# w111liang222/lidar-slam-detection

Hardware: AMD Instinct MI355X
Metric: registered points/sec (120k-pt scan vs 1e7-pt map, full iterate-to-converge) (higher is better)
Workload: dtype f32 per-point geometry / f64 transforms and reductions

## Files before the change

include/lio_hip.h:

```cpp
#ifndef LIO_HIP_H_
#define LIO_HIP_H_

#include <stdint.h>

#ifdef __cplusplus
extern "C" {
#endif

#define LIO_OK 0
#define LIO_E_INVALID (-1)
#define LIO_E_CAPACITY (-2)
#define LIO_E_DEVICE (-3)
#define LIO_E_STATE (-4)

typedef struct lio_map lio_map;
typedef struct lio_scan lio_scan;
typedef struct lio_engine lio_engine;

const char* lio_last_error(void);
const char* lio_last_warning(void);
int lio_device_count(void);
#define LIO_ABI_VERSION 24
int lio_abi_version(void);
void* lio_pinned_alloc(uint64_t bytes);
void lio_pinned_free(void* p);
uint64_t lio_map_bytes(const lio_map*);

lio_map* lio_map_create(int device, float resolution, uint64_t max_points, uint64_t max_voxels, int stencil);
void lio_map_destroy(lio_map*);
int lio_map_set_stencil(lio_map*, int stencil);
int lio_map_insert(lio_map*, const float* world_xyzi, uint64_t n, double travel);
int lio_map_insert_device(lio_map*, const void* d_world_xyzi, uint64_t n, double travel);
int lio_map_clear(lio_map*);
int lio_map_set_lru(lio_map*, uint64_t capacity_voxels, double max_distance);
int lio_map_lru_stats(lio_map*, uint64_t* n_evicted, uint64_t* n_interleaved);
int lio_map_lru_exact_stats(lio_map*, uint64_t* n_recreated, uint64_t* n_batches_not_followed);
int lio_map_set_tie_mode(lio_map*, int mode);
int lio_map_tie_stats(lio_map*, uint64_t* n_boundary_ties, uint64_t* n_unresolved);
int lio_map_pool_stats(lio_map*, uint64_t* pool_top, uint64_t* pool_cap);
int lio_map_stats(lio_map*, uint64_t* n_points, uint64_t* n_voxels);
uint64_t lio_map_knn_candidates(lio_map*);
uint64_t lio_map_knn_touched(lio_map*);
uint64_t lio_map_knn_unique(lio_map*);
int64_t lio_map_dump(lio_map*, float* out_xyzi, uint64_t cap_points);
int lio_map_knn(lio_map*, const float* world_xyzi, uint32_t n, float* out_pts, int32_t* out_cnt);

lio_scan* lio_scan_create(int device, uint32_t max_raw, uint32_t max_ds);
void lio_scan_destroy(lio_scan*);
int lio_scan_reset(lio_scan*);
int lio_scan_upload(lio_scan*, const float* body_xyzi, uint32_t n_raw);
int lio_scan_set_device(lio_scan*, const void* d_body_xyzi, uint32_t n_raw);
int lio_scan_undistort_delta(lio_scan*, const uint32_t* stamp_us, int stamps_on_device, const float delta_pose[16], double scan_period);
int lio_scan_download_raw(lio_scan*, float* out_xyzi, uint32_t cap);
int lio_scan_undistort_poses(lio_scan*, const uint32_t* stamp_us, int stamps_on_device, uint64_t header_stamp_us, const uint64_t* pose_stamp_us,
                             const double* pose_T, uint32_t n_poses);
int lio_scan_undistort_imu(lio_scan*, const uint32_t* stamp_us, int stamps_on_device, const double* poses, uint32_t n_poses, const double* end_pos3,
                           const double* end_rot_xyzw, const double* ril_xyzw, const double* til3, double blind, int filter_num, int undistort);
int lio_scan_voxel_downsample(lio_scan*, float leaf, int sync, uint32_t* n_ds);
int lio_scan_voxel_downsample_batch(lio_scan** scans, int n, float leaf, uint32_t* n_ds);
int lio_scan_set_ds(lio_scan*, const float* ds_body_xyzi, uint32_t n_ds);
int lio_scan_num_ds(lio_scan*);
int lio_scan_download_ds(lio_scan*, float* out_xyzi, uint32_t cap);
int lio_scan_download_world(lio_scan*, float* out_xyzi, uint32_t cap);
const void* lio_scan_ds_device(lio_scan*, uint32_t* n);
int lio_scan_download_match(lio_scan*, uint8_t* selected, float* normvec, int32_t* nn_cnt, float* nn_pts);

typedef struct lio_kernel_times {
    double knn_us, linearize_us, finalize_us;
    uint32_t knn_launches, linearize_launches, finalize_launches;
    uint32_t pad;
} lio_kernel_times;
int lio_scan_enable_kernel_timing(lio_scan*, int on);
int lio_scan_kernel_times(lio_scan*, lio_kernel_times* out, int reset);

typedef struct lio_normal_eq {
    double JtJ[36];
    double Jtr[6];
    double nnT[9];
    double eigvec[9];
    double eigval[3];
    double contri[3];
    double strong[3];
    double sum_abs_res;
    uint32_t n_eff;
    uint32_t n_ds;
    uint32_t n_knn_candidates_lo, n_knn_candidates_hi;
    uint32_t n_tie;
    uint32_t seq;
} lio_normal_eq;

int lio_p2plane_linearize(lio_map*, lio_scan*, const double pose_wi[7], const double ext_il[7], int redo_knn,
                          lio_normal_eq* out);
int lio_scan_set_degeneracy_mode(lio_scan*, int mode);
int lio_p2plane_degeneracy(lio_scan*, const double V[9], double contri[3], double strong[3]);
int lio_p2plane_rows(lio_scan*, const double pose_wi[7], const double ext_il[7], double* h_x6, double* h, uint32_t cap_rows);
int lio_map_incremental(lio_map*, lio_scan*, const double pose_wi[7], const double ext_il[7], float map_leaf,
                        int ekf_inited, double travel);
int lio_map_seed(lio_map*, lio_scan*, const double pose_wi[7], const double ext_il[7], double travel);

lio_engine* lio_engine_create(int device, float resolution, int stencil, uint64_t max_points, uint64_t max_voxels,
                              uint32_t max_raw, uint32_t max_ds);
lio_engine* lio_engine_create_shared(lio_map* shared_map, uint32_t max_raw, uint32_t max_ds);
void lio_engine_destroy(lio_engine*);
lio_map* lio_engine_map(lio_engine*);
lio_scan* lio_engine_scan(lio_engine*);
// ... 40 lines not shown
int lio_engine_set_device_loop(lio_engine*, int on);

int lio_fastlio_ins_enqueue(lio_engine*, double stamp, const double vel_imu[3]);
int lio_fastlio_set_wheelspeed(lio_engine*, int enable);
int lio_fastlio_pcl_enqueue(lio_engine*, const float* xyzi, const uint32_t* stamp_us, uint32_t n, double header_stamp);
int lio_fastlio_pcl_stage(lio_engine*, uint32_t n, float** xyzi, uint32_t** stamp_us);
int lio_fastlio_pcl_commit(lio_engine*, uint32_t n, double header_stamp);
int lio_fastlio_pcl_enqueue_device(lio_engine*, const void* d_xyzi, const void* d_stamp_us, uint32_t n, double header_stamp);
int lio_fastlio_main(lio_engine*);
int lio_fastlio_odometry(lio_engine*, double odom_s[16], double odom_e[16]);
int lio_fastlio_state(lio_engine*, double out[20]);
int lio_fastlio_start_state(lio_engine*, double s26[26]);
int lio_fastlio_download_undistorted(lio_engine*, float* out_xyzi, uint32_t cap, uint32_t* n);
typedef int (*lio_meas_fn)(void* ctx, const double* s26, int converge, int* n, double* rows6, double* h, int cap);
int lio_eskf_update_cb(const double s26[26], const double P[529], double R, int max_iter, lio_meas_fn fn, void* ctx, int cap, double s26_out[26],
                       double P_out[529]);
int lio_eskf_update_ws_cb(const double s26[26], const double P[529], double R, int max_iter, lio_meas_fn fn, void* ctx, int cap, const double* ins_vel,
                          int degenerate, double s26_out[26], double P_out[529]);
int lio_state_predict(const double s26[26], const double P[529], double dt, const double Q[12], const double acc[3], const double gyro[3],
                      double s26_out[26], double P_out[529]);
typedef int (*lio_sums_fn)(void* ctx, const double* s26, int converge, double* acc29);
typedef void (*lio_degeneracy_fn)(void* ctx, const double* V9, double* cs6);
int lio_eskf_update_sums_cb(const double s26[26], const double P[529], double R, int max_iter, int degenerate_detect_en, lio_sums_fn fn,
                            lio_degeneracy_fn dfn, void* ctx, double s26_out[26], double P_out[529], lio_pass_log* logs, int cap_logs, int* status);

typedef void (*lio_reduce_fn)(void* ctx, double* buf, int n);
int lio_engine_set_reduce_hook(lio_engine*, lio_reduce_fn fn, void* ctx);
typedef struct lio_comm lio_comm;
int lio_comm_unique_id(uint8_t id[128]);
lio_comm* lio_comm_init(int device, int rank, int world, const uint8_t id[128]);
void lio_comm_destroy(lio_comm*);
int lio_comm_rank(const lio_comm*);
int lio_comm_world(const lio_comm*);
int lio_allgather_normal_eq(lio_comm*, const double* d_local32, double* d_gathered, double* d_sum32, void* stream);
int lio_allgather_records(lio_comm*, const double* d_local, double* d_gathered, uint32_t n_records, void* stream);
int lio_comm_stats(lio_comm*, uint64_t* n_collectives, double* total_us);
int lio_engine_set_joint(lio_engine* e, lio_engine** others, int n_others, lio_comm* comm);
int lio_engine_joint_register(lio_engine* e, const float* raw_body_xyzi, uint32_t n_raw, double lidar_beg_time, double state26[26], double cov[529]);
int lio_engine_joint_register_device(lio_engine* e, const void* d_raw_body_xyzi, uint32_t n_raw, double lidar_beg_time, double state26[26], double cov[529]);
#define LIO_JOB_KEEP_CACHE 1u
#define LIO_JOB_IDLE 2u
#define LIO_JOB_HOST_RAW 4u
#define LIO_JOB_FLAGS_KNOWN 7u
typedef struct lio_scan_job {
    const void* d_raw;
    uint32_t n_raw;
    uint32_t flags;
    double lidar_beg_time;
    const double* state_in;
    const double* cov_in;
    double* state_out;
    int32_t rc;
    int32_t n_ds, n_pass, n_knn_pass;
} lio_scan_job;
int lio_engines_process_batch(lio_engine** engines, int n_engines, lio_scan_job* jobs, int n_jobs);
typedef struct lio_batch lio_batch;
typedef struct lio_batch_result {
    double state[26];
    int32_t status;
    int32_t n_pass, n_knn_pass, n_ds, n_eff, degenerate, radix_passes, err;
    int32_t loop_i, loop_t, loop_converge, pad;
    uint32_t seq, pad2;
} lio_batch_result;
lio_batch* lio_batch_create(lio_map* shared_map, int n_slots, int n_groups, uint32_t max_raw, uint32_t max_ds);
lio_batch* lio_batch_create_joint(lio_map** sub_maps, int n_sub_maps, lio_comm* comm, int n_slots, int n_groups, uint32_t max_raw, uint32_t max_ds);
typedef int (*lio_gather_fn)(void* ctx, const double* d_local, double* d_gathered, uint32_t n_records, void* stream);
int lio_batch_set_gather_hook(lio_batch*, lio_gather_fn fn, void* ctx, int rank, int world);
int lio_batch_exchange_stats(lio_batch*, uint32_t* chunk_points, uint64_t* jobs_rerun, uint64_t* bytes_per_rank_and_round);
lio_batch* lio_batch_create_sequences(int device, float resolution, int stencil, uint64_t max_points, uint64_t max_voxels, int n_slots, int n_groups,
                                      uint32_t max_raw, uint32_t max_ds);
int lio_batch_sequences_step(lio_batch*, lio_scan_job* jobs, int n_jobs, double* cov_out);
int lio_batch_fastlio_main(lio_batch*, int* rc_out);
void lio_batch_destroy(lio_batch*);
int lio_batch_process(lio_batch*, lio_scan_job* jobs, int n_jobs);
typedef struct lio_batch_times {
    double downsample_us, knn_us, linearize_us, step_us;
    uint32_t downsample_launches, knn_launches, linearize_launches, step_launches;
    double insert_us;
    uint32_t insert_launches, pad;
} lio_batch_times;
int lio_batch_enable_kernel_timing(lio_batch*, int on);
int lio_batch_kernel_times(lio_batch*, lio_batch_times* out, int reset);
lio_engine* lio_batch_engine(lio_batch*, int group, int slot);
int lio_engine_set_static_map(lio_engine*, int on);

typedef struct lio_ndt lio_ndt;
lio_ndt* lio_ndt_create(int device, float resolution, int search_method, uint64_t max_points, uint64_t max_voxels, uint32_t max_source_points);
void lio_ndt_destroy(lio_ndt*);
int lio_ndt_set_target(lio_ndt*, const float* xyzi, uint64_t n);
int lio_ndt_set_target_device(lio_ndt*, const void* d_xyzi, uint64_t n);
int lio_ndt_num_voxels(lio_ndt*);
int lio_ndt_voxel_at(lio_ndt*, const float p[3], float mean[3], float cinv[9]);
int lio_ndt_linearize(lio_ndt*, lio_scan* source, const double T[16], int update_corr, int with_derivatives, double H[36], double b[6],
                      double* err, uint32_t* n_corr);
int lio_ndt_fitness_score(lio_ndt*, lio_scan* source, const double T[16], double max_range, double* score, uint32_t* n_inliers);
int lio_ndt_overlap_score(lio_ndt*, lio_scan* source, const double relpose[16], double max_range, double xy_range, double min_z, double* score,
                          double* inlier_ratio);
typedef struct lio_ndt_times {
    double cost_us;
    uint64_t launches, update_launches, pairs, source_points;
} lio_ndt_times;
int lio_ndt_enable_kernel_timing(lio_ndt*, int on);
int lio_ndt_kernel_times(lio_ndt*, lio_ndt_times* out, int reset);
typedef struct lio_ndt_params {
    int32_t max_iterations;
    int32_t lm_max_iterations;
    double rotation_epsilon_deg;
    double transformation_epsilon;
    double lm_init_lambda_factor;
    double max_process_time_ms;
} lio_ndt_params;
void lio_ndt_default_params(lio_ndt_params*);
int lio_ndt_align(lio_ndt*, lio_scan* source, const double guess[16], const lio_ndt_params* params, double out[16], int* iterations,
                  int* converged);

typedef struct lio_align_job {
    lio_ndt* target;
    lio_scan* source;
    const double* guess;
    double out[16];
    int32_t iterations, converged, evaluations, rc;
} lio_align_job;
int lio_ndt_align_batch(lio_ndt*, lio_align_job* jobs, int n_jobs, const lio_ndt_params* params);

typedef struct lio_gicp lio_gicp;
lio_gicp* lio_gicp_create(int device, float grid_resolution, uint32_t max_points, int k_correspondences);
void lio_gicp_destroy(lio_gicp*);
int lio_gicp_set_target(lio_gicp*, const float* xyzi, uint32_t n);
int lio_gicp_set_source(lio_gicp*, const float* xyzi, uint32_t n);
int lio_gicp_set_target_device(lio_gicp*, const void* d_xyzi, uint32_t n);
int lio_gicp_set_source_device(lio_gicp*, const void* d_xyzi, uint32_t n);
int lio_gicp_set_voxel_mode(lio_gicp*, double voxel_resolution, int search_method);
int lio_gicp_voxel_at(lio_gicp*, const float p[3], double mean[3], double cov6[6]);
int lio_gicp_download(lio_gicp*, int which, float* xyzi, double* cov6, uint32_t cap);
int lio_gicp_correspondences(lio_gicp*, int32_t* corr, uint32_t cap);
int lio_gicp_neighbours(lio_gicp*, int which, int32_t* idx, uint32_t cap_points);
int lio_gicp_mahalanobis(lio_gicp*, double* maha6, uint32_t cap);
int lio_gicp_linearize(lio_gicp*, const double T[16], double max_corr_dist, int update_corr, int with_derivatives, double H[36], double b[6], double* err,
                       uint32_t* n_corr);
int lio_gicp_align(lio_gicp*, const double guess[16], const lio_ndt_params* params, double max_corr_dist, double out[16], int* iterations, int* converged);
int lio_gicp_fitness_score(lio_gicp*, const double T[16], double max_range, double* score, uint32_t* nr);

typedef struct lio_pose_estimator lio_pose_estimator;
typedef struct lio_gps_observation {
    double T[16];
    double precision;
    int32_t dimension;
} lio_gps_observation;
lio_pose_estimator* lio_pose_estimator_create(const float imu_ext[16], uint64_t stamp_us, const float pos[3], const float quat_wxyz[4],
                                              double cool_time_duration);
void lio_pose_estimator_destroy(lio_pose_estimator*);
int lio_pose_estimator_predict(lio_pose_estimator*, uint64_t stamp_us, const float acc[3], const float gyro[3]);
int lio_pose_estimator_match(lio_pose_estimator*, lio_ndt* target, lio_scan* source, const lio_ndt_params* params, float observation[7],
                             int* iterations);
int lio_pose_estimator_match_gps(lio_pose_estimator*, lio_ndt* target, lio_scan* source, const lio_ndt_params* params, const lio_gps_observation* gps,
                                 float observation[7], float observation_cov[49], int* iterations);
int lio_pose_estimator_guess(lio_pose_estimator*, const lio_gps_observation* gps, float init_guess[16]);
int lio_pose_estimator_observe(lio_pose_estimator*, const float init_guess[16], const float aligned[16], int converged, const lio_gps_observation* gps,
                               float observation[7], float observation_cov[49]);
int lio_pose_estimator_match_gps_only(lio_pose_estimator*, const lio_gps_observation* gps, float observation[7], float observation_cov[49]);
int lio_pose_estimator_get_timed_pose(lio_pose_estimator*, uint64_t stamp_us, const double acc_g[3], const double gyro_dps[3], double pose[16]);
int lio_pose_estimator_predict_nostate(lio_pose_estimator*, uint64_t stamp_us, double pose[16]);
int lio_pose_estimator_correct(lio_pose_estimator*, uint64_t stamp_us, const float observation[7]);
uint64_t lio_pose_estimator_get_dt(lio_pose_estimator*);
int lio_pose_estimator_get(lio_pose_estimator*, float mean23[23], float cov529[529]);
int lio_pose_estimator_set(lio_pose_estimator*, const float mean23[23], const float cov529[529]);
// ... 532 lines not shown
```

lidar-slam-detection_amd/csrc/batch.hip:

```cpp
#include <sched.h>
#include <stdlib.h>

#include <chrono>
#include <deque>
#include <vector>

#include "eskf.h"
#include "lio_common.h"

using namespace lio;

int engine_resume_update(lio_engine* e, const double* x_now26, const double* x_prop26, const double* P_prop, int i, int converge, int t);
void engine_count_passes(lio_engine* e, int* n_pass, int* n_knn);
int engine_joint_register_device(lio_engine* e, const void* d_raw, uint32_t n_raw, double lidar_beg_time, double state26[26], double cov[529]);
struct lio_comm;
extern "C" int lio_comm_world(const lio_comm*);
extern "C" {
int engine_seq_prepare(lio_engine* e, uint32_t n_raw, double lidar_beg_time, int* ekf_inited);
void engine_seq_params(lio_engine* e, double* laser_cov, int* maximum_iter, int* degenerate_detect_en, float* leaf_surf, float* leaf_map, int* static_map,
                       double* travel, double last_pos_lid[3]);
int engine_seq_finish(lio_engine* e, const double x26[26], const double P529[529], int n_ds, int n_pass, int n_knn, int n_eff, int degenerate, int inserted,
                      uint32_t n_add, uint32_t map_err, uint32_t bound);
int engine_seq_resume(lio_engine* e, const double* x_now26, const double* x_prop26, const double* P_prop, int i, int converge, int t);
int engine_seq_has_lru(lio_engine* e);
int engine_fastlio_front(lio_engine* e, const void** d_raw, uint32_t* n_raw, double* beg, double state26[26], double cov529[529]);
void engine_fastlio_back(lio_engine* e);
}

namespace {

struct Group {
    hipStream_t stream = nullptr;
    std::vector<lio_engine*> eng;
    std::vector<lio_engine*> sub_eng;
    double* d_local32 = nullptr;
    double* d_gathered = nullptr;
    char* d_ds_send = nullptr;
    char* d_ds_all = nullptr;
    int ds_world = 0;
    MapRef* d_rowmaps = nullptr;
    std::vector<MapRef> rowmap_rows;
    char* d_block = nullptr;
    char* h_block = nullptr;
    size_t block_bytes = 0;
    SlotDesc* d_desc = nullptr;
    SlotDesc* h_desc = nullptr;
    EskfDev* d_ctrl = nullptr;
    EskfDev* h_ctrl = nullptr;
    hipGraphExec_t exec[5] = {nullptr, nullptr, nullptr, nullptr, nullptr};
    const void* graph_table = nullptr;
    int graph_stencil = 0;
    lio_batch_result* h_res = nullptr;
    lio_batch_result* h_res_dev = nullptr;
    std::vector<int> job_of_slot;
    float4* d_rawbuf = nullptr;
    MapRef* d_maps = nullptr;
    MapRef* h_maps = nullptr;
    SeqDev* d_seq = nullptr;
    SeqDev* h_seq = nullptr;
    std::vector<int> seq_path;
    int any_lru = 0;
    int n_active = 0;
    int launched_passes = 4;
    uint32_t seq = 0;
    uint32_t max_n_raw = 0;
    BatchTimer* bt = nullptr;
};

}

struct lio_batch {
    lio_map* map = nullptr;
    int device = 0;
    int n_slots = 0;
    uint32_t max_raw = 0, max_ds = 0;
    int pred_passes = 4;
    bool broken = false;
    int use_graph = 1;
    int count_touched = 0;
    std::vector<lio_map*> maps;
    lio_comm* comm = nullptr;
    int world = 1;
    int rank = 0;
    int split_ds = 1;
    uint32_t ds_cap = 0;
    uint32_t ds_seen_max = 0;
    bool ds_cap_full = false;
    uint64_t n_ds_cut = 0;
    int (*gather_hook)(void*, const double*, double*, uint32_t, void*) = nullptr;
    void* gather_ctx = nullptr;
    bool joint = false;
    bool sequences = false;
    std::vector<lio_scan_job> fl_jobs;
    std::vector<double> fl_state, fl_cov;
    std::vector<Group> groups;
    double t_submit = 0, t_wait = 0, t_collect = 0;
    uint64_t n_rounds = 0;
};

static void fill_mapref(MapRef& r, const lio_map* m);

namespace {

const MapRef* joint_rowmaps(lio_batch* b, Group& g) {
    const int M = (int)b->maps.size(), B = b->n_slots;
    if (M < 2) return nullptr;
    for (int m = 1; m < M; m++)
        if (b->maps[m]->stencil_id != b->maps[0]->stencil_id || b->maps[m]->stencil.n != b->maps[0]->stencil.n) return nullptr;
    std::vector<MapRef> now((size_t)M);
    for (int m = 0; m < M; m++) {
        memset(&now[m], 0, sizeof(MapRef));
        fill_mapref(now[m], b->maps[m]);
    }
    bool fresh = g.d_rowmaps != nullptr && (int)g.rowmap_rows.size() == M;
    for (int m = 0; m < M && fresh; m++) fresh = memcmp(&g.rowmap_rows[m], &now[m], sizeof(MapRef)) == 0;
    if (fresh) return g.d_rowmaps;
    std::vector<MapRef> rows((size_t)M * B);
    for (int m = 0; m < M; m++)
        for (int s = 0; s < B; s++) rows[(size_t)m * B + s] = now[m];
    if (!g.d_rowmaps && hipMalloc(reinterpret_cast<void**>(&g.d_rowmaps), sizeof(MapRef) * rows.size()) != hipSuccess) { g.d_rowmaps = nullptr; return nullptr; }
    if (hipMemcpyAsync(g.d_rowmaps, rows.data(), sizeof(MapRef) * rows.size(), hipMemcpyHostToDevice, g.stream) != hipSuccess) return nullptr;
    if (hipStreamSynchronize(g.stream) != hipSuccess) return nullptr;
    g.rowmap_rows = now;
    return g.d_rowmaps;
}

void fill_desc(SlotDesc& d, lio_scan* sc, EskfDev* d_ctrl, lio_batch_result* d_res) {
    d.max_ds = sc->max_ds;
    d.partial_blocks = sc->partial_blocks;
    d.sd = sc->dev;
    d.keys_a = sc->keys_a; d.keys_b = sc->keys_b; d.vals_a = sc->vals_a; d.vals_b = sc->vals_b;
// ... 60 lines not shown
    return dst;
}

int submit(lio_batch* b, Group& g, lio_scan_job* jobs, int first, int n, int passes) {
    const int B = b->n_slots;
    g.seq++;
    g.n_active = 0;
    g.max_n_raw = 0;
    g.launched_passes = passes;
    for (int s = 0; s < B; s++) {
        SlotDesc& d = g.h_desc[s];
        d.active = 0;
        g.job_of_slot[s] = -1;
        if (s >= n) continue;
        lio_scan_job& job = jobs[first + s];
        g.job_of_slot[s] = first + s;
        job.rc = LIO_E_INVALID;
        job.n_ds = job.n_pass = job.n_knn_pass = 0;
        if (job.flags & ~LIO_JOB_FLAGS_KNOWN) { set_error("lio_scan_job.flags = 0x%x: unknown bits (a job array that was not zero-initialised?)", job.flags); continue; }
        if (job.flags & LIO_JOB_IDLE) { job.rc = 0; g.job_of_slot[s] = -1; continue; }
        if (!job.state_in || !job.cov_in || (!job.d_raw && job.n_raw)) continue;
        if (job.n_raw > b->max_raw) { set_error("scan of %u points exceeds max_raw %u", job.n_raw, b->max_raw); job.rc = LIO_E_CAPACITY; continue; }
        if (job.n_raw == 0) { job.rc = 2; continue; }
        d.raw = static_cast<const float4*>(job.d_raw);
        if (job.flags & LIO_JOB_HOST_RAW) {
            int src = LIO_OK;
            d.raw = stage_host_raw(b, g, s, job, &src);
            if (src != LIO_OK) { job.rc = src; continue; }
        }
        d.n_raw = job.n_raw;
        d.nblocks = (job.n_raw + 2047u) / 2048u;
        d.active = 1;
        d.seq = g.seq;
        d.min_ds = 5;
        d.reset_cache = (job.flags & LIO_JOB_KEEP_CACHE) ? 0u : 1u;
        fill_ctrl(g.h_ctrl[s], job.state_in, job.cov_in, 0.001 , 4, 1, b->joint ? 1 : 0);
        g.h_res[s].seq = g.seq - 1;
        g.n_active++;
        if (job.n_raw > g.max_n_raw) g.max_n_raw = job.n_raw;
    }
    const int M = (int)b->maps.size();
    for (int m = 1; m < M; m++)
        for (int s = 0; s < B; s++) {
            SlotDesc& d = g.h_desc[(size_t)m * B + s];
            const SlotDesc& p = g.h_desc[s];
            d.raw = p.raw; d.n_raw = p.n_raw; d.nblocks = p.nblocks; d.active = p.active; d.seq = p.seq; d.min_ds = p.min_ds; d.reset_cache = p.reset_cache;
        }
    if (g.n_active == 0) return LIO_OK;
    const bool timed = g.bt && g.bt->on;
    const MapRef* rowmaps = b->joint ? joint_rowmaps(b, g) : nullptr;
    auto enqueue = [&](BatchTimer* bt) -> int {
        LIO_HIP_TRY(hipMemcpyAsync(g.d_block, g.h_block, g.block_bytes, hipMemcpyHostToDevice, g.stream));
        const uint32_t ds_bound = b->max_raw < b->max_ds ? b->max_raw : b->max_ds;
        int rc = LIO_OK;
        if (b->joint && b->world > 1 && b->split_ds) {
            const int per = (B + b->world - 1) / b->world;
            const int s0 = std::min(B, b->rank * per), s1 = std::min(B, s0 + per);
            if (g.ds_world != b->world) {
                if (g.d_ds_send) hipFree(g.d_ds_send);
                if (g.d_ds_all) hipFree(g.d_ds_all);
                g.d_ds_send = g.d_ds_all = nullptr;
                g.ds_world = 0;
                const size_t chunk = (size_t)per * ds_exchange_slot_bytes(ds_bound);
                LIO_HIP_TRY(hipMalloc(reinterpret_cast<void**>(&g.d_ds_send), chunk));
                LIO_HIP_TRY(hipMalloc(reinterpret_cast<void**>(&g.d_ds_all), chunk * (size_t)b->world));
                g.ds_world = b->world;
            }
            if (bt) bt->begin(0);
            if (s1 > s0) rc = vg_downsample_batch(g.stream, g.d_desc + s0, s1 - s0, b->max_raw, b->max_ds, 0.5f, passes);
            if (bt) bt->end(0);
            if (rc != LIO_OK) return rc;
            if (b->ds_cap == 0) {
                const char* k = getenv("LIO_JOINT_DS_CAP");
                const uint32_t want = k ? (uint32_t)strtoul(k, nullptr, 10) : ((ds_bound / 4u + 1023u) & ~1023u);
                b->ds_cap = std::min(ds_bound, std::max(k ? 1u : 4096u, want));
            }
            const uint32_t cap = b->ds_cap_full ? ds_bound : b->ds_cap;
            rc = p2plane_batch_exchange_ds(b->comm, b->world, b->gather_hook, b->gather_ctx, g.stream, g.d_desc, B, per, s0, s1, cap, g.d_ds_send, g.d_ds_all);
            if (rc == LIO_OK && s0 > 0) rc = scan_begin_rows(g.stream, g.d_desc, s0);
            if (rc == LIO_OK && s1 < B) rc = scan_begin_rows(g.stream, g.d_desc + s1, B - s1);
            if (rc != LIO_OK) return rc;
        } else {
            if (bt) bt->begin(0);
            rc = vg_downsample_batch(g.stream, g.d_desc, B, b->max_raw, b->max_ds, 0.5f, passes);
            if (bt) bt->end(0);
            if (rc != LIO_OK) return rc;
        }
        if (b->joint) {
            rc = p2plane_batch_share(g.stream, g.d_desc, B, M, ds_bound);
            if (rc == LIO_OK) rc = scan_begin_rows(g.stream, g.d_desc + B, B * (M - 1));
            if (rc != LIO_OK) return rc;
            return p2plane_batch_update_joint(b->maps.data(), M, b->comm, b->world, b->gather_hook, b->gather_ctx, g.stream, g.d_desc, B, ds_bound, 5, g.d_local32, g.d_gathered, bt,
                                              rowmaps);
        }
        return p2plane_batch_update(b->map, g.stream, g.d_desc, B, ds_bound, 5, bt, bt ? b->count_touched : 0);
    };
    if (!b->use_graph || timed || b->joint) return enqueue(timed ? g.bt : nullptr);
    if (g.graph_table != b->map->table || g.graph_stencil != b->map->stencil.n) {
        for (int k = 0; k < 5; k++)
            if (g.exec[k]) { hipGraphExecDestroy(g.exec[k]); g.exec[k] = nullptr; }
        g.graph_table = b->map->table;
        g.graph_stencil = b->map->stencil.n;
    }
    if (!g.exec[passes]) {
        hipGraph_t graph = nullptr;
        LIO_HIP_TRY(hipStreamBeginCapture(g.stream, hipStreamCaptureModeThreadLocal));
        const int rc = enqueue(nullptr);
        const hipError_t e2 = hipStreamEndCapture(g.stream, &graph);
        if (rc != LIO_OK) { if (graph) hipGraphDestroy(graph); return rc; }
        LIO_HIP_TRY(e2);
        LIO_HIP_TRY(hipGraphInstantiate(&g.exec[passes], graph, nullptr, nullptr, 0));
        hipGraphDestroy(graph);
    }
    LIO_HIP_TRY(hipGraphLaunch(g.exec[passes], g.stream));
    return LIO_OK;
}

int wait_group(Group& g, int B) {
    for (int s = 0; s < B; s++) {
        if (!g.h_desc[s].active) continue;
        volatile uint32_t* seq = &g.h_res[s].seq;
        for (uint64_t spin = 0; *seq != g.seq; spin++) {
            __builtin_ia32_pause();
            if (spin > 2000 && (spin & 31) == 0) sched_yield();
            if (spin > 40000000ull) {
                LIO_HIP_TRY(hipStreamSynchronize(g.stream));
                if (*seq != g.seq) { set_error("batch slot %d did not report (seq %u, expected %u)", s, *seq, g.seq); return LIO_E_DEVICE; }
                break;
            }
        }
    }
    __atomic_thread_fence(__ATOMIC_ACQUIRE);
    return LIO_OK;
}

}


extern "C" {

static lio_batch* batch_create_impl(lio_map** maps, int n_maps, lio_comm* comm, int n_slots, int n_groups, uint32_t max_raw, uint32_t max_ds) {
    lio_map* map = n_maps > 0 && maps ? maps[0] : nullptr;
    if (!map || n_maps > 64 || n_slots < 1 || n_slots > 256 || n_groups < 1 || n_groups > 8 || max_raw == 0 || max_ds == 0) { set_error("lio_batch_create: bad argument"); return nullptr; }
    for (int m = 1; m < n_maps; m++)
        if (!maps[m] || maps[m]->device != map->device) { set_error("lio_batch_create_joint: the sub-maps of a batch live on one device"); return nullptr; }
    if (hipSetDevice(map->device) != hipSuccess) { set_error("lio_batch_create: no HIP device %d", map->device); return nullptr; }
    lio_batch* b = new lio_batch();
    b->map = map;
    b->device = map->device;
    b->n_slots = n_slots;
    b->max_raw = max_raw;
    b->max_ds = max_ds;
    b->maps.assign(maps, maps + n_maps);
    b->comm = comm;
    b->world = comm ? lio_comm_world(comm) : 1;
    b->rank = comm ? lio_comm_rank(comm) : 0;
    { const char* k = getenv("LIO_JOINT_SPLIT_DS"); b->split_ds = (k && k[0] == '0') ? 0 : 1; }
    b->joint = n_maps > 1 || comm != nullptr;
    b->groups.resize(n_groups);
    { const char* k = getenv("LIO_BATCH_GRAPH"); b->use_graph = (k && k[0] == '0') ? 0 : 1; }
    bool ok = true;
    const int M = n_maps;
    for (Group& g : b->groups) ok = ok && hipStreamCreateWithFlags(&g.stream, hipStreamNonBlocking) == hipSuccess;
    for (Group& g : b->groups) {
        g.job_of_slot.assign(n_slots, -1);
        const size_t desc_bytes = sizeof(SlotDesc) * (size_t)n_slots * (size_t)M;
        g.block_bytes = desc_bytes + sizeof(EskfDev) * (size_t)n_slots;
        ok = ok && hipMalloc(reinterpret_cast<void**>(&g.d_block), g.block_bytes) == hipSuccess;
        ok = ok && hipHostMalloc(reinterpret_cast<void**>(&g.h_block), g.block_bytes, hipHostMallocDefault) == hipSuccess;
        if (ok) {
            g.d_desc = reinterpret_cast<SlotDesc*>(g.d_block);
            g.h_desc = reinterpret_cast<SlotDesc*>(g.h_block);
            g.d_ctrl = reinterpret_cast<EskfDev*>(g.d_block + desc_bytes);
            g.h_ctrl = reinterpret_cast<EskfDev*>(g.h_block + desc_bytes);
        }
        ok = ok && hipHostMalloc(reinterpret_cast<void**>(&g.h_res), sizeof(lio_batch_result) * n_slots, hipHostMallocMapped) == hipSuccess;
        ok = ok && hipHostGetDevicePointer(reinterpret_cast<void**>(&g.h_res_dev), g.h_res, 0) == hipSuccess;
        if (b->joint) {
            ok = ok && hipMalloc(reinterpret_cast<void**>(&g.d_local32), sizeof(double) * 32 * n_slots) == hipSuccess;
            ok = ok && hipMalloc(reinterpret_cast<void**>(&g.d_gathered), sizeof(double) * 32 * n_slots * (size_t)b->world) == hipSuccess;
        }
        if (!ok) break;
        memset(g.h_block, 0, g.block_bytes);
        memset(g.h_res, 0, sizeof(lio_batch_result) * n_slots);
        ok = hipMemset(g.d_block, 0, g.block_bytes) == hipSuccess;
        for (int s = 0; s < n_slots && ok; s++) {
            lio_engine* e = lio_engine_create_shared(map, max_raw, max_ds);
            if (!e) { ok = false; break; }
            lio_engine_set_flags(e, 1, 0, 0.0, -10.0);
            g.eng.push_back(e);
            fill_desc(g.h_desc[s], lio_engine_scan(e), &g.d_ctrl[s], &g.h_res_dev[s]);
        }
        for (int m = 1; m < M && ok; m++)
            for (int s = 0; s < n_slots && ok; s++) {
                lio_engine* e = lio_engine_create_shared(maps[m], max_raw, max_ds);
                if (!e) { ok = false; break; }
                lio_engine_set_flags(e, 1, 0, 0.0, -10.0);
                g.sub_eng.push_back(e);
                fill_desc(g.h_desc[(size_t)m * n_slots + s], lio_engine_scan(e), &g.d_ctrl[s], nullptr);
            }
        for (int s = 0; s < n_slots && ok && b->joint; s++) {
            std::vector<lio_engine*> others;
            for (int m = 1; m < M; m++) others.push_back(g.sub_eng[(size_t)(m - 1) * n_slots + s]);
            ok = lio_engine_set_joint(g.eng[s], others.empty() ? nullptr : others.data(), (int)others.size(), comm) == LIO_OK;
        }
    }
    if (!ok) {
        set_error("lio_batch_create: device setup failed: %s", hipGetErrorString(hipGetLastError()));
        lio_batch_destroy(b);
        return nullptr;
    }
    {
        const char* q = getenv("GPU_MAX_HW_QUEUES");
        if (n_groups > 1 && (!q || atoi(q) < 8))
            set_warning("lio_batch_create: GPU_MAX_HW_QUEUES=%s -- with fewer than 8 hardware queues the %d rounds in flight mostly serialise (~20 %% slower); "
                        "export GPU_MAX_HW_QUEUES=8 before the process's first HIP call", q ? q : "(unset: 4)", n_groups);
    }
    return b;
}

lio_batch* lio_batch_create(lio_map* map, int n_slots, int n_groups, uint32_t max_raw, uint32_t max_ds) {
    return batch_create_impl(&map, map ? 1 : 0, nullptr, n_slots, n_groups, max_raw, max_ds);
}

lio_batch* lio_batch_create_joint(lio_map** sub_maps, int n_sub_maps, lio_comm* comm, int n_slots, int n_groups, uint32_t max_raw, uint32_t max_ds) {
    return batch_create_impl(sub_maps, n_sub_maps, comm, n_slots, n_groups, max_raw, max_ds);
}

int lio_batch_set_gather_hook(lio_batch* b, lio_gather_fn fn, void* ctx, int rank, int world) {
    if (!b || !fn || world < 1 || rank < 0 || rank >= world) return LIO_E_INVALID;
    if (!b->joint || b->comm) { set_error("lio_batch_set_gather_hook: for a batch made by lio_batch_create_joint without a communicator"); return LIO_E_STATE; }
    hipSetDevice(b->map->device);
    for (auto& g : b->groups) {
        LIO_HIP_TRY(hipStreamSynchronize(g.stream));
        if (g.d_gathered) hipFree(g.d_gathered);
        g.d_gathered = nullptr;
        LIO_HIP_TRY(hipMalloc(reinterpret_cast<void**>(&g.d_gathered), sizeof(double) * 32 * b->n_slots * (size_t)world));
    }
    b->gather_hook = fn;
    b->gather_ctx = ctx;
    b->world = world;
    b->rank = rank;
    return LIO_OK;
}

int lio_batch_exchange_stats(lio_batch* b, uint32_t* chunk_points, uint64_t* jobs_rerun, uint64_t* bytes_per_rank_and_round) {
    if (!b) return LIO_E_INVALID;
    const bool on = b->joint && b->world > 1 && b->split_ds;
    if (chunk_points) *chunk_points = on ? b->ds_cap : 0u;
    if (jobs_rerun) *jobs_rerun = b->n_ds_cut;
    if (bytes_per_rank_and_round) {
        const int per = (b->n_slots + b->world - 1) / b->world;
        *bytes_per_rank_and_round = on && b->ds_cap ? (uint64_t)per * ds_exchange_slot_bytes(b->ds_cap) : 0u;
    }
    return LIO_OK;
}

void lio_batch_destroy(lio_batch* b) {
    if (!b) return;
    hipSetDevice(b->device);
    if (getenv("LIO_BATCH_PROFILE") && b->n_rounds)
        fprintf(stderr, "lio_batch: %llu rounds of %d slots; host per round: submit %.1f us, wait %.1f us, collect %.1f us\n", (unsigned long long)b->n_rounds,
                b->n_slots, 1e6 * b->t_submit / b->n_rounds, 1e6 * b->t_wait / b->n_rounds, 1e6 * b->t_collect / b->n_rounds);
    for (Group& g : b->groups) {
        if (g.stream) hipStreamSynchronize(g.stream);
        group_free(g);
    }
    delete b;
}

int lio_batch_enable_kernel_timing(lio_batch* b, int on) {
    if (!b) return LIO_E_INVALID;
    hipSetDevice(b->device);
    for (Group& g : b->groups) {
        if (!g.bt) { g.bt = new BatchTimer(); g.bt->stream = g.stream; }
        if (on && !g.bt->created) {
            for (int c = 0; c < BatchTimer::kClasses; c++)
                for (int i = 0; i < BatchTimer::kPool; i++) {
                    LIO_HIP_TRY(hipEventCreate(&g.bt->ev[c][i][0]));
                    LIO_HIP_TRY(hipEventCreate(&g.bt->ev[c][i][1]));
                }
            g.bt->created = true;
        }
        g.bt->on = on != 0;
    }
    b->count_touched = (on & 2) ? 1 : 0;
    if (b->count_touched && b->map) { const int rc = map_enable_touch_bits(b->map); if (rc != LIO_OK) return rc; }
    return LIO_OK;
}

int lio_batch_kernel_times(lio_batch* b, lio_batch_times* out, int reset) {
    if (!b || !out) return LIO_E_INVALID;
    memset(out, 0, sizeof(*out));
    for (Group& g : b->groups) {
        if (!g.bt) continue;
        out->downsample_us += g.bt->us[0]; out->knn_us += g.bt->us[1]; out->linearize_us += g.bt->us[2]; out->step_us += g.bt->us[3];
        out->downsample_launches += g.bt->launches[0]; out->knn_launches += g.bt->launches[1]; out->linearize_launches += g.bt->launches[2];
        out->step_launches += g.bt->launches[3];
        out->insert_us += g.bt->us[4];
        out->insert_launches += g.bt->launches[4];
        if (reset)
            for (int c = 0; c < BatchTimer::kClasses; c++) { g.bt->us[c] = 0; g.bt->launches[c] = 0; }
    }
    return LIO_OK;
}

lio_engine* lio_batch_engine(lio_batch* b, int group, int slot) {
    if (!b || group < 0 || group >= (int)b->groups.size() || slot < 0 || slot >= b->n_slots) return nullptr;
    return b->groups[group].eng[slot];
}

int lio_batch_process(lio_batch* b, lio_scan_job* jobs, int n_jobs) {
    if (!b || (!jobs && n_jobs) || n_jobs < 0) return LIO_E_INVALID;
    if (b->sequences) { set_error("lio_batch_process: a sequence batch is driven by lio_batch_sequences_step"); return LIO_E_STATE; }
    hipSetDevice(b->device);
    const int B = b->n_slots;
    int next = 0, first_err = 0;
    std::deque<int> inflight;
    std::vector<int> retry;
    auto note = [&](int rc) { if (rc < 0 && !first_err) first_err = rc; };
    auto collect = [&](Group& g) {
        int need_max = 1;
        for (int s = 0; s < B; s++) {
            const int j = g.job_of_slot[s];
            if (j < 0) continue;
            if (!g.h_desc[s].active) { note(jobs[j].rc); continue; }
            lio_scan_job& job = jobs[j];
            const lio_batch_result& r = g.h_res[s];
            if (r.radix_passes > need_max) need_max = r.radix_passes;
            if (r.radix_passes > g.launched_passes) { retry.push_back(j); continue; }
            lio_engine* e = g.eng[s];
            lio_scan* sc = lio_engine_scan(e);
            sc->have_ds = r.n_ds;
            sc->n_raw = g.h_desc[s].n_raw;
            job.n_ds = r.n_ds;
            job.n_pass = r.n_pass;
            job.n_knn_pass = r.n_knn_pass;
            if (r.err & 4) {
                hipMemsetAsync(&sc->dev->err, 0, 4, g.stream);
                b->n_ds_cut++;
                retry.push_back(j);
                continue;
            }
            if (r.err & 1) {
                set_error("downsampled scan exceeds max_ds %u", b->max_ds);
                hipMemsetAsync(&sc->dev->err, 0, 4, g.stream);
                job.rc = LIO_E_CAPACITY;
                note(job.rc);
                continue;
            }
            if ((uint32_t)r.n_ds > b->ds_seen_max) b->ds_seen_max = (uint32_t)r.n_ds;
            if (r.status == EK_SKIPPED) { job.rc = 2; continue; }
            if (r.status == EK_NEEDS_HOST && b->joint && b->gather_hook) {
                set_error("lio_batch (gather hook mode): a scan needs the host-driven joint path, which only exists over a lio_comm");
                job.rc = LIO_E_STATE;
                note(job.rc);
                continue;
            }
            if (r.status == EK_NEEDS_HOST && b->joint) {
                if (!(job.flags & LIO_JOB_KEEP_CACHE)) {
                    scan_forget_cache(sc);
                    for (int m = 1; m < (int)b->maps.size(); m++) scan_forget_cache(lio_engine_scan(g.sub_eng[(size_t)(m - 1) * B + s]));
                }
                double st26[26], cov[529];
                memcpy(st26, job.state_in, sizeof(st26));
                memcpy(cov, job.cov_in, sizeof(cov));
                const void* d_cloud = (job.flags & LIO_JOB_HOST_RAW) ? static_cast<const void*>(g.d_rawbuf + (size_t)s * b->max_raw) : job.d_raw;
                const int rc = engine_joint_register_device(e, d_cloud, job.n_raw, job.lidar_beg_time, st26, cov);
                if (rc < 0) { job.rc = rc; note(rc); continue; }
                engine_count_passes(e, &job.n_pass, &job.n_knn_pass);
                if (job.state_out) memcpy(job.state_out, st26, sizeof(st26));
                job.rc = rc;
                continue;
            }
            if (r.status == EK_NEEDS_HOST) {
                const int rc = engine_resume_update(e, r.state, job.state_in, job.cov_in, r.loop_i, r.loop_converge, r.loop_t);
                if (rc != LIO_OK) { job.rc = rc; note(rc); continue; }
                int np = 0, nk = 0;
                engine_count_passes(e, &np, &nk);
                job.n_pass += np;
                job.n_knn_pass += nk;
                if (job.state_out) lio_engine_get_state(e, job.state_out);
                job.rc = 3;
                continue;
            }
// ... 497 lines not shown
```

lidar-slam-detection_amd/csrc/knn.hip:

```cpp
#include "hashgrid.h"
#include "knn_dev.h"
#include "lio_common.h"
#include "refsel.h"

namespace lio {

#ifndef LIO_KNN_G
#define LIO_KNN_G 16
#endif
#ifndef LIO_KNN_U
#define LIO_KNN_U 4
#endif
#ifndef LIO_KNN_WAVES
#define LIO_KNN_WAVES 6
#endif
#ifndef LIO_KNN_PRUNE
#define LIO_KNN_PRUNE 1
#endif
#ifndef LIO_KNN_STAT
#define LIO_KNN_STAT 1
#endif
#ifndef LIO_KNN_WAVES_BATCH
#define LIO_KNN_WAVES_BATCH 7
#endif
#ifdef LIO_KNN_MAXWAVES
#define LIO_KNN_OCC __attribute__((amdgpu_waves_per_eu(LIO_KNN_MAXWAVES, LIO_KNN_MAXWAVES)))
#else
#define LIO_KNN_OCC
#endif
constexpr int kG = LIO_KNN_G;
constexpr int kU = LIO_KNN_U;
constexpr int kGPB = 256 / kG;

template <int CTRL>
__device__ inline uint32_t dpp_row(uint32_t v) {
    return (uint32_t)__builtin_amdgcn_update_dpp(0, (int)v, CTRL, 0xF, 0xF, true);
}
__device__ inline uint32_t group_min32(uint32_t v) {
    if constexpr (kG == 8) {
        v = min(v, dpp_row<0xB1>(v));
        v = min(v, dpp_row<0x4E>(v));
        v = min(v, dpp_row<0x141>(v));
    } else if constexpr (kG == 16) {
        v = min(v, dpp_row<0x128>(v));
        v = min(v, dpp_row<0x124>(v));
        v = min(v, dpp_row<0x122>(v));
        v = min(v, dpp_row<0x121>(v));
    } else {
#pragma unroll
        for (int off = kG / 2; off > 0; off >>= 1) v = min(v, __shfl_xor(v, off, kG));
    }
    return v;
}
__device__ inline uint32_t group_ballot(bool p, int lane) {
    const unsigned long long b = __ballot(p);
    if constexpr (kG == 16 || kG == 8) {
        const uint32_t half = (lane & 32) ? (uint32_t)(b >> 32) : (uint32_t)b;
        return (half >> (lane & (32 - kG) & 31)) & ((1u << kG) - 1u);
    } else {
        return (uint32_t)((b >> (lane & ~(kG - 1))) & ((1ull << kG) - 1ull));
    }
}
__device__ inline uint32_t group_max32(uint32_t v) {
    if constexpr (kG == 8) {
        v = max(v, dpp_row<0xB1>(v));
        v = max(v, dpp_row<0x4E>(v));
        v = max(v, dpp_row<0x141>(v));
    } else if constexpr (kG == 16) {
        v = max(v, dpp_row<0x128>(v));
        v = max(v, dpp_row<0x124>(v));
        v = max(v, dpp_row<0x122>(v));
        v = max(v, dpp_row<0x121>(v));
    } else {
#pragma unroll
        for (int off = kG / 2; off > 0; off >>= 1) v = max(v, __shfl_xor(v, off, kG));
    }
    return v;
}
__device__ inline uint32_t group_sum32(uint32_t v) {
    if constexpr (kG == 8) {
        v += dpp_row<0xB1>(v);
        v += dpp_row<0x4E>(v);
        v += dpp_row<0x141>(v);
    } else if constexpr (kG == 16) {
// ... 132 lines not shown
    for (int k = 0; k < KM; k++) {
        uint32_t ptr = 0, cnt = 0;
        if (want[k] != kEmptyKey) {
            uint4 r = raw[k];
            for (uint32_t probe = 0; probe <= (mask >> 6); probe++) {
                const unsigned long long kk = ((unsigned long long)r.y << 32) | r.x;
                if (kk == want[k]) { ptr = r.z; cnt = r.w; break; }
                if (kk == kEmptyKey) break;
                brick_next(bp[k]);
                r = *reinterpret_cast<const uint4*>(&table[brick_slot(bp[k], mask)]);
            }
        }
        const bool hit = cnt > 0;
        const uint32_t m = group_ballot(hit, lane);
        if (hit) {
            const uint32_t at = nhit + __popc(m & below);
            g.v_ptr[at] = ptr;
            g.v_cnt[at] = cnt;
        }
        nhit += __popc(m);
        total += cnt;
    }
    if (gl < kU) { g.v_ptr[nhit + gl] = 0; g.v_cnt[nhit + gl] = 0; }
    nhit_out = nhit;
    return total;
}

__device__ inline void group_lds_sync() {
    __builtin_amdgcn_fence(__ATOMIC_RELEASE, "wavefront");
    __builtin_amdgcn_wave_barrier();
    __builtin_amdgcn_fence(__ATOMIC_ACQUIRE, "wavefront");
}

__device__ inline uint32_t med3_u32(uint32_t a, uint32_t b, uint32_t c) {
    uint32_t r;
    asm("v_med3_u32 %0, %1, %2, %3" : "=v"(r) : "v"(a), "v"(b), "v"(c));
    return r;
}
#ifndef LIO_KNN_BOUND
#define LIO_KNN_BOUND 5
#endif
__device__ inline uint32_t fifth_bound(uint32_t d0, uint32_t d2, uint32_t d4) {
    uint32_t t = group_min32(d4);
#if LIO_KNN_BOUND == 2
    (void)d0;
    const uint32_t m1 = group_min32(d2);
    return min(t, group_min32(d2 == m1 ? 0xFFFFFFFFu : d2));
#endif
    (void)d2;
    uint32_t v = d0, m = 0xFFFFFFFFu;
#pragma unroll
    for (int r = 0; r < 5; r++) {
        m = group_min32(v);
        if (v == m) v = 0xFFFFFFFFu;
    }
    return min(t, m);
}

struct Cand {
    float d2;
    uint32_t id;
};

__device__ __noinline__ bool cand_tie_less(const Cand& a, const Cand& b, const float4* __restrict__ pool) {
    if (a.id == b.id) return false;
    if (a.id == kNoIdx || b.id == kNoIdx) return a.id < b.id;
    const float4 pa = pool[a.id], pb = pool[b.id];
    if (pa.x != pb.x) return pa.x < pb.x;
    if (pa.y != pb.y) return pa.y < pb.y;
    if (pa.z != pb.z) return pa.z < pb.z;
    return a.id < b.id;
}
__device__ inline bool cand_less(const Cand& a, const Cand& b, const float4* __restrict__ pool) {
    if (a.d2 != b.d2) return a.d2 < b.d2;
    return cand_tie_less(a, b, pool);
}


template <int KM, int MODE, bool COUNT = false, class PoseFill>
__device__ __forceinline__ void knn_body(const Slot* __restrict__ table, uint32_t mask, const float4* __restrict__ pool,
                                         float inv_res, const StencilArgs& st, PoseFill fill, const float4* __restrict__ queries,
                                         uint32_t n_host, const ScanDev* __restrict__ sd, float4* __restrict__ world_out,
                                         float4* __restrict__ nn_pts, uint32_t nn_stride, int32_t* __restrict__ nn_cnt,
                                         MapDev* md, uint32_t* __restrict__ n_tie, uint32_t* __restrict__ tie_list) {
    __shared__ GroupLds lds[kGPB];
    const int tid = threadIdx.x;
    const int grp = tid / kG, gl = tid % kG;
    const int lane = tid & 63;
    GroupLds& g = lds[grp];
    const uint32_t n = sd ? sd->n_ds : n_host;
    const unsigned long long gmask = ((1ull << kG) - 1ull) << (lane - gl);
    __shared__ uint32_t stat_s[256 / 64];
    if (tid < 256 / 64) stat_s[tid] = 0;
    uint32_t touched = 0;
    uint32_t fresh = 0;
    uint32_t* const bits = COUNT ? md->touch_bits : nullptr;
    const float res = 1.0f / inv_res;
    const uint32_t b1_bits = __float_as_uint(0.0625f * res * res), b2_bits = __float_as_uint(0.25f * res * res);
    (void)b1_bits; (void)b2_bits;

    const uint32_t nblk = (n + kGPB - 1) / kGPB;
    const uint32_t per_xcd = (nblk + 7u) >> 3;
    const uint32_t wg_per_xcd = gridDim.x >> 3;
    constexpr uint32_t kAhead = 64 / kGPB;
    __shared__ float4 pw_s[64];
    __shared__ PoseArgs pose_s;
    if constexpr (MODE == 0) fill(pose_s);
    uint32_t ahead = kAhead;
    for (uint32_t j = blockIdx.x >> 3; j < per_xcd; j += wg_per_xcd) {
        const uint32_t q0 = ((blockIdx.x & 7u) * per_xcd + j) * kGPB;
        const uint32_t q = q0 + grp;
        const bool active = q < n;
        float4 pw = make_float4(0.f, 0.f, 0.f, 0.f);
        if constexpr (MODE == 0) {
            if (ahead == kAhead) {
                __syncthreads();
                if (tid < 64) {
                    const uint32_t j2 = j + (uint32_t)(tid / kGPB) * wg_per_xcd;
                    const uint32_t q2 = ((blockIdx.x & 7u) * per_xcd + j2) * kGPB + (uint32_t)(tid % kGPB);
                    if (j2 < per_xcd && q2 < n) {
                        float4 w2;
                        body_to_world(pose_s, queries[q2], w2);
                        world_out[q2] = w2;
                        uint32_t t2 = (uint32_t)tid;
                        asm volatile("" : "+v"(t2));
                        pw_s[t2] = w2;
                    }
                }
                __syncthreads();
                ahead = 0;
            }
            if (active) pw = pw_s[ahead * kGPB + grp];
            ahead++;
        } else {
            if (active) pw = queries[q];
        }
        int kx = 0, ky = 0, kz = 0;
        pos2grid(pw.x, pw.y, pw.z, inv_res, kx, ky, kz);
        uint32_t nhit = 0;
        constexpr bool kPrune = LIO_KNN_PRUNE && KM * kG <= 32;
        uint32_t n0 = 0, n01 = 0, total;
        const uint32_t limit = 0xFFFFFFFFu;
        if constexpr (kPrune) total = probe_stencil_bucketed<KM>(table, mask, st, active, pw, res, kx, ky, kz, gl, lane, gmask, g, nhit, n0, n01, limit);
        else total = probe_stencil<KM>(table, mask, st, active, kx, ky, kz, gl, lane, gmask, g, nhit);
        if constexpr (LIO_KNN_STAT || COUNT) {
            const uint32_t gs = group_sum32(total);
            const uint32_t ws = (uint32_t)__builtin_amdgcn_readlane((int)gs, 0) + (uint32_t)__builtin_amdgcn_readlane((int)gs, 16) +
                                (uint32_t)__builtin_amdgcn_readlane((int)gs, 32) + (uint32_t)__builtin_amdgcn_readlane((int)gs, 48);
            if (lane == 0) stat_s[tid >> 6] += ws;
        }
        group_lds_sync();
        uint32_t d0 = 0xFFFFFFFFu, d1 = 0xFFFFFFFFu, dd2 = 0xFFFFFFFFu, d3 = 0xFFFFFFFFu, d4 = 0xFFFFFFFFu;
        uint32_t i0d = 0xFFFFFFFFu, i1d = 0xFFFFFFFFu, i2d = 0xFFFFFFFFu, i3d = 0xFFFFFFFFu, i4d = 0xFFFFFFFFu;
        uint32_t inrange = 0;
        bool drop_tie = false;
        uint32_t bound5 = 0xFFFFFFFFu;
        const uint32_t ptr_first = g.v_ptr[0];
        bool need_bound = true;
#ifndef LIO_KNN_HOME_FIRST
#define LIO_KNN_HOME_FIRST 0
#endif
        int phase = (kPrune && LIO_KNN_HOME_FIRST) ? 0 : 2;
        for (uint32_t s0 = 0; s0 < nhit; s0 += (phase >= 1 ? kU : 0u), phase = (phase < 2 ? phase + 1 : 2)) {
            uint32_t ptr4[kU], cnt4[kU];
            uint32_t cmax = 0;
            bool ins = false;
            if constexpr (kPrune) {
                if (s0 > 0 || phase == 1) {
                    if (need_bound) bound5 = fifth_bound(d0, dd2, d4);
                    const uint32_t floor_bits = s0 < n0 ? 0u : (s0 < n01 ? b1_bits : b2_bits);
                    if (bound5 < floor_bits) break;
                    const uint32_t r0 = s0 + gl, r1 = r0 + kG, r2 = r1 + kG, r3 = r2 + kG;
                    const bool mine = (r0 < nhit && g.v_dmin[r0] <= bound5) || (r1 < nhit && g.v_dmin[r1] <= bound5) ||
                                      (kG < 16 && ((r2 < nhit && g.v_dmin[r2] <= bound5) || (r3 < nhit && g.v_dmin[r3] <= bound5)));
                    if (!group_ballot(mine, lane)) break;
                }
            }
#pragma unroll
            for (int u = 0; u < kU; u += 4) {
                const uint4 vp = *reinterpret_cast<const uint4*>(&g.v_ptr[s0 + u]);
                uint4 vc = *reinterpret_cast<const uint4*>(&g.v_cnt[s0 + u]);
                if constexpr (kPrune) {
                    const uint4 vd = *reinterpret_cast<const uint4*>(&g.v_dmin[s0 + u]);
                    if (vd.x > bound5) vc.x = 0;
                    if (vd.y > bound5) vc.y = 0;
                    if (vd.z > bound5) vc.z = 0;
                    if (vd.w > bound5) vc.w = 0;
                    if (LIO_KNN_HOME_FIRST && u == 0) {
                        if (phase == 0) { vc.y = 0; vc.z = 0; vc.w = 0; }
                        else if (phase == 1) vc.x = 0;
                    }
                }
                ptr4[u] = vp.x; ptr4[u + 1] = vp.y; ptr4[u + 2] = vp.z; ptr4[u + 3] = vp.w;
                cnt4[u] = vc.x; cnt4[u + 1] = vc.y; cnt4[u + 2] = vc.z; cnt4[u + 3] = vc.w;
                cmax = max(cmax, max(max(vc.x, vc.y), max(vc.z, vc.w)));
                if constexpr (COUNT) { if (gl == 0) touched += (vc.x + vc.y) + (vc.z + vc.w); }
            }
            for (uint32_t i0 = gl; i0 < cmax + gl; i0 += kG) {
                float4 p[kU];
#pragma unroll
                for (int u = 0; u < kU; u++) p[u] = pool[i0 < cnt4[u] ? ptr4[u] + i0 : ptr_first];
#pragma unroll
// ... 27 lines not shown
                        dd2 = med3_u32(d1, dd2, kd);
                        d1 = med3_u32(d0, d1, kd);
                        d0 = min(d0, kd);
                    }
                }
            }
            if constexpr (kPrune) need_bound = group_ballot(ins, lane) != 0;
        }
        inrange = group_sum32(inrange);
        uint32_t win = 0xFFFFFFFFu, prev_d = 0xFFFFFFFFu;
        bool tie = false;
        int pops = 0;
#pragma unroll
        for (int r = 0; r < 6; r++) {
            const uint32_t bd = group_min32(d0);
            const uint32_t bi = group_min32(d0 == bd ? i0d : 0xFFFFFFFFu);
            const bool some = bi != 0xFFFFFFFFu;
            if (r > 0 && some && bd == prev_d) tie = true;
            prev_d = some ? bd : 0xFFFFFFFFu;
            if (gl == r) win = bi;
            if (some && d0 == bd && i0d == bi) {
                d0 = d1; d1 = dd2; dd2 = d3; d3 = d4; d4 = 0xFFFFFFFFu;
                i0d = i1d; i1d = i2d; i2d = i3d; i3d = i4d; i4d = 0xFFFFFFFFu;
                pops++;
            }
        }
        if (group_ballot(pops >= 5 && drop_tie, lane)) tie = true;
        if (active && inrange > 0) {
            if (gl < 5) {
                uint32_t g2 = (uint32_t)gl;
                asm volatile("" : "+v"(g2));
                nn_pts[g2 * nn_stride + q] = (win != 0xFFFFFFFFu) ? pool[win] : make_float4(0.f, 0.f, 0.f, 0.f);
            }
            if (gl == 0) {
                nn_cnt[q] = inrange < 5 ? (int32_t)inrange : 5;
                if (tie) tie_list[atomicAdd(n_tie, 1u)] = q;
            }
        }
        group_lds_sync();
    }
    __shared__ unsigned long long vred[256 / 64];
    if constexpr (LIO_KNN_STAT || COUNT) {
        __syncthreads();
        uint32_t te = threadIdx.x;
        asm volatile("" : "+v"(te));
        if (te < 256 / 64) vred[te] = stat_s[te];
        __syncthreads();
        if (tid == 0) {
            const unsigned long long v = (vred[0] + vred[1]) + (vred[2] + vred[3]);
            if (v) atomicAdd(&md->knn_cand[(blockIdx.x & 63) * 16], v);
        }
    }
    if constexpr (COUNT) {
        __syncthreads();
        unsigned long long tsum = touched;
#pragma unroll
        for (int off = 32; off > 0; off >>= 1) tsum += __shfl_xor(tsum, off);
        if (lane == 0) vred[tid >> 6] = tsum;
        __syncthreads();
        if (tid == 0) {
            const unsigned long long v = (vred[0] + vred[1]) + (vred[2] + vred[3]);
            if (v) atomicAdd(&md->knn_cand[(blockIdx.x & 63) * 16 + 1], v);
        }
        __syncthreads();
        unsigned long long fsum = fresh;
#pragma unroll
        for (int off = 32; off > 0; off >>= 1) fsum += __shfl_xor(fsum, off);
        if (lane == 0) vred[tid >> 6] = fsum;
        __syncthreads();
        if (tid == 0) {
            const unsigned long long v = (vred[0] + vred[1]) + (vred[2] + vred[3]);
            if (v) atomicAdd(&md->knn_cand[(blockIdx.x & 63) * 16 + 2], v);
        }
    }
}

template <int KM, int MODE>
__global__ void __launch_bounds__(256, LIO_KNN_WAVES) knn_kernel(const Slot* __restrict__ table, uint32_t mask, const float4* __restrict__ pool,
                                                  float inv_res, StencilArgs st, PoseArgs pose, const float4* __restrict__ queries,
                                                  uint32_t n_host, const ScanDev* __restrict__ sd, float4* __restrict__ world_out,
                                                  float4* __restrict__ nn_pts, uint32_t nn_stride, int32_t* __restrict__ nn_cnt,
                                                  MapDev* md, uint32_t* __restrict__ n_tie, uint32_t* __restrict__ tie_list) {
    knn_body<KM, MODE>(table, mask, pool, inv_res, st, [&](PoseArgs& P) { if (threadIdx.x == 0) P = pose; }, queries, n_host, sd, world_out, nn_pts, nn_stride, nn_cnt, md,
                       n_tie, tie_list);
}
template <int KM, bool COUNT>
__global__ void LIO_KNN_OCC __launch_bounds__(256, COUNT ? LIO_KNN_WAVES : LIO_KNN_WAVES_BATCH) knn_batch_kernel(const Slot* __restrict__ table, uint32_t mask, const float4* __restrict__ pool,
                                                                       float inv_res, StencilArgs st, const SlotDesc* __restrict__ slots, MapDev* md) {
    const SlotDesc& d = slots[blockIdx.y];
    if (!d.active) return;
    const SlotGateLite sg = slot_gate_lite(d);
    if ((sg.status != EK_RUNNING) | (sg.converge == 0) | (sg.n_ds < d.min_ds)) return;
    const double* __restrict__ x = d.ctrl->x;
    knn_body<KM, 0, COUNT>(table, mask, pool, inv_res, st, [x](PoseArgs& P) { pose_fill_from_state(P, x); }, d.ds_body, sg.n_ds, nullptr, d.ds_world, d.nn_pts,
                                  d.max_ds, d.nn_cnt, md, &d.sd->n_tie, d.tie_list);
}

constexpr int kSelCap = 2560;
struct SelLds {
    uint32_t a_d[kSelCap], a_id[kSelCap], a_seq[kSelCap];
    refsel::Rec list[kSelCap];
    refsel::Rec fin[5 * kMaxStencil + 8];
    uint32_t v_ptr[kMaxStencil], v_cnt[kMaxStencil];
    uint32_t v_first[kMaxStencil + 1];
    uint32_t seg_m[kMaxStencil], seg_base[kMaxStencil + 1], seg_keep[kMaxStencil];
    uint32_t wsum[4];
    uint32_t out_d[8], out_id[8];
    int size;
};

template <int MODE>
__device__ __forceinline__ void refsel_query(const Slot* __restrict__ table, uint32_t mask, const float4* __restrict__ pool, const uint32_t* __restrict__ seq,
                                          float inv_res, const StencilArgs& st, const PoseArgs& pose, const float4* __restrict__ queries, uint32_t q,
                                          float4* __restrict__ nn_pts, uint32_t nn_stride, MapDev* md, SelLds& S, bool keep_order) {
    const int tid = threadIdx.x, lane = tid & 63, wave = tid >> 6;
    float4 pw;
    {
        const float4 pq = queries[q];
        if (MODE == 0) body_to_world(pose, pq, pw);
        else pw = pq;
    }
    int kx = 0, ky = 0, kz = 0;
    pos2grid(pw.x, pw.y, pw.z, inv_res, kx, ky, kz);
    if (tid < st.n) {
        uint32_t ptr = 0, cnt = 0;
        grid_find(table, mask, kx + st.off[tid][0], ky + st.off[tid][1], kz + st.off[tid][2], ptr, cnt);
        S.v_ptr[tid] = ptr;
        S.v_cnt[tid] = cnt;
        S.seg_m[tid] = 0;
    }
    __syncthreads();
    if (tid == 0) {
        uint32_t acc = 0;
        for (int v = 0; v < st.n; v++) { S.v_first[v] = acc; acc += S.v_cnt[v]; }
        S.v_first[st.n] = acc;
    }
    __syncthreads();
    if (tid == 0) S.size = 0;
    bool overflow = false;
    int g0 = 0;
    while (g0 < st.n) {
        int g1 = g0;
        uint32_t total = 0;
        while (g1 < st.n && total + S.v_cnt[g1] <= (uint32_t)kSelCap) { total += S.v_cnt[g1]; g1++; }
        if (g1 == g0) { overflow = true; break; }
        const uint32_t f0 = S.v_first[g0];
        uint32_t m_all = 0;
        for (uint32_t base = 0; base < total; base += 256) {
            const uint32_t f = f0 + base + (uint32_t)tid;
            const bool have = base + (uint32_t)tid < total;
            int v = g0;
            if (have)
                while (v + 1 < g1 && S.v_first[v + 1] <= f) v++;
            const uint32_t idx = have ? S.v_ptr[v] + (f - S.v_first[v]) : 0u;
            const float4 p = pool[idx];
            const float dx = p.x - pw.x, dy = p.y - pw.y, dz = p.z - pw.z;
            const float d2 = dx * dx + (dy * dy + dz * dz);
            const bool in = have && d2 < 5.0f;
            const unsigned long long bal = __ballot(in);
            if (lane == 0) S.wsum[wave] = (uint32_t)__popcll(bal);
            __syncthreads();
            uint32_t at = m_all + (uint32_t)__popcll(bal & ((1ull << lane) - 1ull));
            for (int w = 0; w < wave; w++) at += S.wsum[w];
            const uint32_t tot = (S.wsum[0] + S.wsum[1]) + (S.wsum[2] + S.wsum[3]);
            if (in) {
                S.a_d[at] = __float_as_uint(d2);
                S.a_id[at] = idx;
                S.a_seq[at] = seq[idx];
                atomicAdd(&S.seg_m[v], 1u);
            }
            m_all += tot;
            __syncthreads();
        }
        if (tid == 0) {
            uint32_t acc = 0;
            for (int v = g0; v < g1; v++) { S.seg_base[v] = acc; acc += S.seg_m[v]; }
            S.seg_base[g1] = acc;
        }
// ... 127 lines not shown
        uint32_t win = kNoIdx;
        float d_fifth = -1.f, d_sixth = -2.f;
        for (int r = 0; r < 6; r++) {
            Cand best = e[0];
            for (int off = kG / 2; off > 0; off >>= 1) {
                Cand o;
                o.d2 = __shfl_xor(best.d2, off, kG);
                o.id = __shfl_xor(best.id, off, kG);
                if (cand_less(o, best, pool)) best = o;
            }
            if (r < 5 && gl == r) win = best.id;
            if (best.id != kNoIdx) {
                if (r == 4) d_fifth = best.d2;
                if (r == 5) d_sixth = best.d2;
            }
            if (best.id != kNoIdx && e[0].id == best.id) {
                for (int k = 0; k < 5; k++) e[k] = e[k + 1];
                e[5] = {INFINITY, kNoIdx};
            }
        }
        if (active && gl < 5 && win != kNoIdx) nn_pts[(size_t)gl * nn_stride + q] = pool[win];
        if (tie_mode != 0 && active && gl == 0 && d_fifth == d_sixth) tie_list[w] = q | 0x80000000u;
        __syncthreads();
    }
}

template <int KM, int MODE>
__global__ void __launch_bounds__(256) knn_exact_kernel(const Slot* __restrict__ table, uint32_t mask, const float4* __restrict__ pool,
                                                        float inv_res, StencilArgs st, PoseArgs pose, const float4* __restrict__ queries,
                                                        float4* __restrict__ nn_pts, uint32_t nn_stride, const uint32_t* __restrict__ n_tie,
                                                        uint32_t* __restrict__ tie_list, int tie_mode) {
    knn_exact_body<KM, MODE>(table, mask, pool, inv_res, st, pose, queries, nn_pts, nn_stride, n_tie, tie_list, tie_mode);
}
template <int MODE>
__device__ __forceinline__ void knn_refsel_body(const Slot* __restrict__ table, uint32_t mask, const float4* __restrict__ pool, const uint32_t* __restrict__ seq,
                                                float inv_res, const StencilArgs& st, const PoseArgs& pose, const float4* __restrict__ queries,
                                                float4* __restrict__ nn_pts, uint32_t nn_stride, const uint32_t* __restrict__ n_tie,
                                                const uint32_t* __restrict__ tie_list, MapDev* md, int tie_mode, uint32_t n_all) {
    __shared__ SelLds sel;
    const bool all = tie_mode == 2;
    const uint32_t n = all ? n_all : *n_tie;
    for (uint32_t w = blockIdx.x; w < n; w += gridDim.x) {
        const uint32_t ent = all ? (w | 0x80000000u) : tie_list[w];
        if (!(ent >> 31)) continue;
        refsel_query<MODE>(table, mask, pool, seq, inv_res, st, pose, queries, ent & 0x7FFFFFFFu, nn_pts, nn_stride, md, sel, all);
    }
}
template <int MODE>
__global__ void __launch_bounds__(256) knn_refsel_kernel(const Slot* __restrict__ table, uint32_t mask, const float4* __restrict__ pool, const uint32_t* __restrict__ seq,
                                                         float inv_res, StencilArgs st, PoseArgs pose, const float4* __restrict__ queries, float4* __restrict__ nn_pts,
                                                         uint32_t nn_stride, const uint32_t* __restrict__ n_tie, const uint32_t* __restrict__ tie_list, MapDev* md,
                                                         int tie_mode, uint32_t n_all) {
    knn_refsel_body<MODE>(table, mask, pool, seq, inv_res, st, pose, queries, nn_pts, nn_stride, n_tie, tie_list, md, tie_mode, n_all);
}
__global__ void __launch_bounds__(256) knn_refsel_batch_kernel(const Slot* __restrict__ table, uint32_t mask, const float4* __restrict__ pool,
                                                               const uint32_t* __restrict__ seq, float inv_res, StencilArgs st, const SlotDesc* __restrict__ slots,
                                                               MapDev* md, int tie_mode) {
    const SlotDesc& d = slots[blockIdx.y];
    if (!d.active || (d.sd->n_tie == 0 && tie_mode != 2)) return;
    const SlotGate sg = slot_gate(d);
    if ((sg.status != EK_RUNNING) | (sg.converge == 0) | (sg.n_ds < d.min_ds)) return;
    knn_refsel_body<0>(table, mask, pool, seq, inv_res, st, sg.pose, d.ds_body, d.nn_pts, d.max_ds, &d.sd->n_tie, d.tie_list, md, tie_mode, sg.n_ds);
}
__global__ void __launch_bounds__(256) knn_refsel_seq_kernel(const MapRef* __restrict__ maps, StencilArgs st, int stencil_id, const SlotDesc* __restrict__ slots) {
    const SlotDesc& d = slots[blockIdx.y];
    if (!d.active) return;
    const MapRef& r = maps[blockIdx.y];
    if (r.stencil_id != stencil_id || r.tie_mode == 0 || !r.pool_seq || (d.sd->n_tie == 0 && r.tie_mode != 2)) return;
    const SlotGate sg = slot_gate(d);
    if ((sg.status != EK_RUNNING) | (sg.converge == 0) | (sg.n_ds < d.min_ds)) return;
    knn_refsel_body<0>(r.table, r.mask, r.pool, r.pool_seq, r.inv_res, st, sg.pose, d.ds_body, d.nn_pts, d.max_ds, &d.sd->n_tie, d.tie_list, r.md, r.tie_mode, sg.n_ds);
}
template <int KM>
__global__ void __launch_bounds__(256) knn_exact_batch_kernel(const Slot* __restrict__ table, uint32_t mask, const float4* __restrict__ pool,
                                                              float inv_res, StencilArgs st, const SlotDesc* __restrict__ slots, int tie_mode) {
    const SlotDesc& d = slots[blockIdx.y];
    if (!d.active || d.sd->n_tie == 0) return;
    const SlotGate sg = slot_gate(d);
    if ((sg.status != EK_RUNNING) | (sg.converge == 0) | (sg.n_ds < d.min_ds)) return;
    const PoseArgs& pose = sg.pose;
    knn_exact_body<KM, 0>(table, mask, pool, inv_res, st, pose, d.ds_body, d.nn_pts, d.max_ds, &d.sd->n_tie, d.tie_list, tie_mode);
}

int knn_batch_launch(lio_map* m, hipStream_t st, const SlotDesc* d_slots, int n_slots, uint32_t grid_x, int count_touched) {
    static const uint32_t forced = [] { const char* e = getenv("LIO_KNN_GRID"); const int v = e ? atoi(e) : 0; return v >= 8 ? (uint32_t)v : 0u; }();
    uint32_t cap = forced ? forced : (12288u / (uint32_t)(n_slots > 0 ? n_slots : 1));
    if (cap > 2048u) cap = 2048u;
    if (cap < 128u) cap = 128u;
    if (grid_x > cap) grid_x = cap;
    if (grid_x == 0) grid_x = 8;
    const dim3 grid((grid_x + 7u) & ~7u, (uint32_t)n_slots);
    const dim3 gridx(n_slots > 8 ? 8 : 64, (uint32_t)n_slots);
    const int tmode = m->pool_seq ? m->tie_mode : 0;
    const int km = (m->stencil.n + kG - 1) / kG;
    if (count_touched && m->touch_bits) LIO_HIP_TRY(hipMemsetAsync(m->touch_bits, 0, (size_t)((m->pool_cap + 31) / 32) * 4, st));
#define KNNB_LAUNCH(KM)                                                                                                                              \
    do {                                                                                                                                             \
        if (count_touched) hipLaunchKernelGGL((knn_batch_kernel<KM, true>), grid, 256, 0, st, m->table, m->table_mask, m->pool, m->inv_res, m->stencil, d_slots, m->dev); \
        else hipLaunchKernelGGL((knn_batch_kernel<KM, false>), grid, 256, 0, st, m->table, m->table_mask, m->pool, m->inv_res, m->stencil, d_slots, m->dev); \
        hipLaunchKernelGGL((knn_exact_batch_kernel<KM>), gridx, 256, 0, st, m->table, m->table_mask, m->pool, m->inv_res, m->stencil, d_slots, tmode); \
    } while (0)
    if (km <= 1) KNNB_LAUNCH(1);
    else if (km <= 2) KNNB_LAUNCH(2);
    else if (km <= 3) KNNB_LAUNCH(3);
    else KNNB_LAUNCH((kMaxStencil + kG - 1) / kG);
#undef KNNB_LAUNCH
    if (tmode != 0)
        hipLaunchKernelGGL(knn_refsel_batch_kernel, dim3(tmode == 2 ? 256 : 4, (uint32_t)n_slots), 256, 0, st, m->table, m->table_mask, m->pool, m->pool_seq, m->inv_res,
                           m->stencil, d_slots, m->dev, tmode);
    LIO_HIP_TRY(hipGetLastError());
    return LIO_OK;
}

template <int KM>
__global__ void __launch_bounds__(256, KM <= 3 ? LIO_KNN_WAVES_BATCH : LIO_KNN_WAVES) knn_seq_kernel(const MapRef* __restrict__ maps, StencilArgs st, int stencil_id,
                                                                     const SlotDesc* __restrict__ slots) {
    const SlotDesc& d = slots[blockIdx.y];
    if (!d.active) return;
    const MapRef& r = maps[blockIdx.y];
    if (r.stencil_id != stencil_id) return;
    const SlotGateLite sg = slot_gate_lite(d);
    if ((sg.status != EK_RUNNING) | (sg.converge == 0) | (sg.n_ds < d.min_ds)) return;
    const double* __restrict__ x = d.ctrl->x;
    knn_body<KM, 0, false>(r.table, r.mask, r.pool, r.inv_res, st, [x](PoseArgs& P) { pose_fill_from_state(P, x); }, d.ds_body, sg.n_ds, nullptr, d.ds_world, d.nn_pts,
                                  d.max_ds, d.nn_cnt, r.md, &d.sd->n_tie, d.tie_list);
}
template <int KM>
__global__ void __launch_bounds__(256) knn_exact_seq_kernel(const MapRef* __restrict__ maps, StencilArgs st, int stencil_id, const SlotDesc* __restrict__ slots) {
    const SlotDesc& d = slots[blockIdx.y];
    if (!d.active) return;
    const MapRef& r = maps[blockIdx.y];
    if (r.stencil_id != stencil_id || d.sd->n_tie == 0) return;
    const SlotGate sg = slot_gate(d);
    if ((sg.status != EK_RUNNING) | (sg.converge == 0) | (sg.n_ds < d.min_ds)) return;
    const PoseArgs& pose = sg.pose;
    knn_exact_body<KM, 0>(r.table, r.mask, r.pool, r.inv_res, st, pose, d.ds_body, d.nn_pts, d.max_ds, &d.sd->n_tie, d.tie_list, r.pool_seq ? r.tie_mode : 0);
}

int knn_seq_launch(hipStream_t st, const MapRef* d_maps, const SlotDesc* d_slots, int n_slots, uint32_t grid_x, const StencilArgs* stencils, const int* stencil_ids,
                   int n_stencils) {
    static const uint32_t forced = [] { const char* e = getenv("LIO_KNN_GRID"); const int v = e ? atoi(e) : 0; return v >= 8 ? (uint32_t)v : 0u; }();
    uint32_t cap = forced ? forced : (12288u / (uint32_t)(n_slots > 0 ? n_slots : 1));
    if (cap > 2048u) cap = 2048u;
    if (cap < 128u) cap = 128u;
    if (grid_x > cap) grid_x = cap;
    if (grid_x == 0) grid_x = 8;
    const dim3 grid((grid_x + 7u) & ~7u, (uint32_t)n_slots);
    const dim3 gridx(n_slots > 8 ? 8 : 64, (uint32_t)n_slots);
    for (int k = 0; k < n_stencils; k++) {
        const StencilArgs& sa = stencils[k];
        const int km = (sa.n + kG - 1) / kG;
#define KNNS_LAUNCH(KM)                                                                                                  \
    do {                                                                                                                 \
        hipLaunchKernelGGL((knn_seq_kernel<KM>), grid, 256, 0, st, d_maps, sa, stencil_ids[k], d_slots);                 \
        hipLaunchKernelGGL((knn_exact_seq_kernel<KM>), gridx, 256, 0, st, d_maps, sa, stencil_ids[k], d_slots);          \
    } while (0)
        if (km <= 1) KNNS_LAUNCH(1);
        else if (km <= 2) KNNS_LAUNCH(2);
        else if (km <= 3) KNNS_LAUNCH(3);
        else KNNS_LAUNCH((kMaxStencil + kG - 1) / kG);
#undef KNNS_LAUNCH
        hipLaunchKernelGGL(knn_refsel_seq_kernel, dim3(4, (uint32_t)n_slots), 256, 0, st, d_maps, sa, stencil_ids[k], d_slots);
    }
    LIO_HIP_TRY(hipGetLastError());
    return LIO_OK;
}

template <int MODE>
static int launch_knn(lio_map* m, hipStream_t st, const PoseArgs& pose, const float4* q, uint32_t n_host, const ScanDev* sd,
                      float4* world_out, float4* nn_pts, uint32_t nn_stride, int32_t* nn_cnt, uint32_t n_bound, uint32_t* n_tie,
                      uint32_t* tie_list) {
    uint32_t blocks = (n_bound + kGPB - 1) / kGPB;
    if (blocks > 16384) blocks = 16384;
    if (blocks == 0) return LIO_OK;
    blocks = (blocks + 7u) & ~7u;
#define KNN_LAUNCH(KM)                                                                                                                  \
    hipLaunchKernelGGL((knn_kernel<KM, MODE>), blocks, 256, 0, st, m->table, m->table_mask, m->pool, m->inv_res, m->stencil, pose, q, n_host, \
                       sd, world_out, nn_pts, nn_stride, nn_cnt, m->dev, n_tie, tie_list)
    const int km = (m->stencil.n + kG - 1) / kG;
    if (km <= 1) KNN_LAUNCH(1);
    else if (km <= 2) KNN_LAUNCH(2);
    else if (km <= 3) KNN_LAUNCH(3);
    else KNN_LAUNCH((kMaxStencil + kG - 1) / kG);
#undef KNN_LAUNCH
    LIO_HIP_TRY(hipGetLastError());
    return LIO_OK;
}

template <int MODE>
static int launch_knn_exact(lio_map* m, hipStream_t st, const PoseArgs& pose, const float4* q, float4* nn_pts, uint32_t nn_stride,
                            uint32_t n_tie_host, const uint32_t* n_tie, uint32_t* tie_list, uint32_t n_all = 0) {
    const int tmode = m->pool_seq ? m->tie_mode : 0;
    if (tmode == 2 && n_all) {
        hipLaunchKernelGGL((knn_refsel_kernel<MODE>), n_all < 4096u ? n_all : 4096u, 256, 0, st, m->table, m->table_mask, m->pool, m->pool_seq, m->inv_res, m->stencil, pose,
                           q, nn_pts, nn_stride, n_tie, tie_list, m->dev, tmode, n_all);
        LIO_HIP_TRY(hipGetLastError());
        return LIO_OK;
    }
    uint32_t blocks = (n_tie_host + kGPB - 1) / kGPB;
    if (blocks == 0) return LIO_OK;
    if (blocks > 4096) blocks = 4096;
#define KNNX_LAUNCH(KM)                                                                                                                      \
    hipLaunchKernelGGL((knn_exact_kernel<KM, MODE>), blocks, 256, 0, st, m->table, m->table_mask, m->pool, m->inv_res, m->stencil, pose, q, nn_pts, \
                       nn_stride, n_tie, tie_list, tmode)
    const int km = (m->stencil.n + kG - 1) / kG;
    if (km <= 1) KNNX_LAUNCH(1);
    else if (km <= 2) KNNX_LAUNCH(2);
    else if (km <= 3) KNNX_LAUNCH(3);
// ... 42 lines not shown
```

lidar-slam-detection_amd/csrc/lio_common.h:

```cpp
#pragma once
#include <hip/hip_runtime.h>
#include <stdint.h>
#include <stdio.h>
#include <string.h>

#include "../../include/lio_hip.h"
#include "eskf_dev.h"

struct LruEntry;

namespace lio {

#if defined(__HIP_DEVICE_COMPILE__)
#define LIO_PIN4(r) asm volatile("" : "+v"((r).x), "+v"((r).y), "+v"((r).z), "+v"((r).w))
#define LIO_PIN1(r) asm volatile("" : "+v"(r))
#else
#define LIO_PIN4(r) ((void)(r))
#define LIO_PIN1(r) ((void)(r))
#endif
__host__ __device__ __forceinline__ void pin_loaded(float4& r) { LIO_PIN4(r); }
__host__ __device__ __forceinline__ void pin_loaded(uint4& r) { LIO_PIN4(r); }
__host__ __device__ __forceinline__ void pin_loaded(uint32_t& r) { LIO_PIN1(r); }
__host__ __device__ __forceinline__ void pin_loaded(float& r) { LIO_PIN1(r); }

// ... 206 lines not shown
    lio::StencilArgs stencil;
    int stencil_id;
    int own_stream;
    uint64_t n_batches;
    uint64_t bytes;
};

namespace lio {
struct KernelTimer;
namespace ground {
const float4* inliers_view(lio_ground* g, uint32_t* n);
}
}
struct lio_scan {
    lio::KernelTimer* kt;
    int force_degeneracy;
    int device;
    hipStream_t stream;
    uint32_t max_raw, max_ds;
    uint32_t n_raw;
    const float4* raw;
    float4* raw_own;
    float4* ds_body;
    float4* ds_world;
    float4* nn_pts;
    int32_t* nn_cnt;
    uint8_t* selected;
    float4* normvec;
    uint32_t *keys_a, *keys_b, *vals_a, *vals_b;
    uint32_t* hist;
    uint32_t* blockcnt;
    uint32_t* hpos;
    uint32_t* longlist;
    uint32_t* tie_list;
    float4* sorted;
    double* partial;
    uint32_t partial_blocks;
    lio::ScanDev* dev;
    lio::ScanDev* host_dev;
    lio_normal_eq* d_result;
    uint32_t* host_nds;
    int pred_passes;
    lio::SlotDesc* d_batch_desc = nullptr;
    lio::SlotDesc* h_batch_desc = nullptr;
    uint32_t batch_desc_cap = 0;
    uint32_t* host_nds_dev;
    lio_normal_eq* h_result;
    lio_normal_eq* h_result_dev;
    uint32_t seq_expected;
    int have_ds;
    uint32_t resize_min;
    uint64_t bytes;
};

namespace lio {
constexpr int kMaxImuPoses = 128;
struct ImuPoseDev {
    double off;
    double acc[3], gyr[3], vel[3], pos[3], R[9];
};
struct UndistortArgs {
    double pos_e[3], rot_e[4], ril[4], til[3];
    double blind2;
    int n_poses, filter_num, undistort;
};
struct DeltaArgs {
    float t[3];
    float aa[3];
    double scan_period;
};
constexpr int kMaxPoseList = 64;
struct PoseListArgs {
    int n_poses;
    unsigned long long limit[kMaxPoseList];
    DeltaArgs d[kMaxPoseList];
};
int undistort_poses_launch(hipStream_t stream, const float4* d_in, const uint32_t* d_stamp_us, uint32_t n, float4* d_out, const PoseListArgs& args,
                           uint32_t* d_tile_max);
int undistort_delta_launch(hipStream_t stream, const float4* d_in, const uint32_t* d_stamp_us, uint32_t n, float4* d_out, const DeltaArgs& args);
int undistort_launch(hipStream_t stream, const float4* d_in, const uint32_t* d_stamp_us, uint32_t n, float4* d_out, const ImuPoseDev* d_poses,
                     const UndistortArgs& args, unsigned long long* d_block_min );

int vg_downsample(lio_scan* s, float leaf, int passes );
int vg_downsample_batch(hipStream_t st, const SlotDesc* d_slots, int n_slots, uint32_t max_raw, uint32_t max_ds, float leaf, int passes);
int knn_batch_launch(lio_map* m, hipStream_t st, const SlotDesc* d_slots, int n_slots, uint32_t grid_x, int count_touched);
struct BatchTimer {
    static constexpr int kClasses = 5;
    static constexpr int kPool = 256;
    hipEvent_t ev[kClasses][kPool][2];
    int used[kClasses] = {0, 0, 0, 0, 0};
    double us[kClasses] = {0, 0, 0, 0, 0};
    uint32_t launches[kClasses] = {0, 0, 0, 0, 0};
    bool on = false, created = false;
    hipStream_t stream = nullptr;
    void begin(int c) { if (on && used[c] < kPool) hipEventRecord(ev[c][used[c]][0], stream); }
    void end(int c) { if (on && used[c] < kPool) { hipEventRecord(ev[c][used[c]][1], stream); used[c]++; } }
    void resolve() {
        for (int c = 0; c < kClasses; c++) {
            for (int i = 0; i < used[c]; i++) {
                float ms = 0.f;
                if (hipEventElapsedTime(&ms, ev[c][i][0], ev[c][i][1]) == hipSuccess) { us[c] += (double)ms * 1000.0; launches[c]++; }
            }
            used[c] = 0;
        }
    }
};
int p2plane_batch_update(lio_map* m, hipStream_t st, const SlotDesc* d_slots, int n_slots, uint32_t ds_bound, int n_passes, BatchTimer* bt, int count_touched);
int knn_seq_launch(hipStream_t st, const MapRef* d_maps, const SlotDesc* d_slots, int n_slots, uint32_t grid_x, const StencilArgs* stencils, const int* stencil_ids,
                   int n_stencils);
int p2plane_seq_update(hipStream_t st, const MapRef* d_maps, const SlotDesc* d_slots, int n_slots, uint32_t ds_bound, int n_passes, const StencilArgs* stencils,
                       const int* stencil_ids, int n_stencils, BatchTimer* bt);
int p2plane_seq_insert(hipStream_t st, const MapRef* d_maps, const SlotDesc* d_slots, SeqDev* d_seq, int n_slots, uint32_t ds_bound, int any_lru);
int map_insert_seq(hipStream_t st, const MapRef* d_maps, const SeqDev* d_seq, int n_slots, uint32_t bound, int any_lru);
int map_rebuild(lio_map* m, hipStream_t stream);
}
struct lio_comm;
namespace lio {
int p2plane_batch_share(hipStream_t st, const SlotDesc* d_descs, int n_slots, int n_maps, uint32_t ds_bound);
int p2plane_batch_update_joint(lio_map** maps, int n_maps, ::lio_comm* comm, int world, int (*gather_hook)(void*, const double*, double*, uint32_t, void*), void* gather_ctx, hipStream_t st, const SlotDesc* d_descs, int n_slots, uint32_t ds_bound,
                               int n_passes, double* d_local32, double* d_gathered, BatchTimer* bt, const MapRef* d_rowmaps = nullptr);
int scan_begin_rows(hipStream_t st, const SlotDesc* d_descs, int n_rows);
size_t ds_exchange_slot_bytes(uint32_t cap);
int p2plane_batch_exchange_ds(::lio_comm* comm, int world, int (*gather_hook)(void*, const double*, double*, uint32_t, void*), void* gather_ctx, hipStream_t st,
                              const SlotDesc* d_descs, int n_slots, int per, int s0, int s1, uint32_t cap, char* d_send, char* d_all);
int scan_begin(lio_scan* s);
int scan_set_nds(lio_scan* s, uint32_t n);
void kt_begin(lio_scan* s, int which);
void kt_end(lio_scan* s, int which);
int map_enable_touch_bits(lio_map* m);
lio_map* map_create_mode(int device, float resolution, uint64_t max_points, uint64_t max_voxels, int stencil, int key_mode);
int map_insert_dev(lio_map* m, hipStream_t stream, const float4* d_pts, uint64_t n, const uint32_t* d_n, double travel);
int map_knn_plane(lio_map* m, lio_scan* s, const PoseArgs& pose, int redo_knn);
int knn_batch(lio_map* m, const float4* d_q, uint32_t n, float4* d_out, int32_t* d_cnt, uint32_t* d_tie);
int map_knn_exact(lio_map* m, lio_scan* s, const PoseArgs& pose, uint32_t n_tie_host);
int p2plane_reduce(lio_map* m, lio_scan* s, const PoseArgs& pose, int redo_knn);
int p2plane_degeneracy(lio_scan* s);
int incremental_classify(lio_map* m, lio_scan* s, const PoseArgs& pose, float map_leaf, int ekf_inited, int seed_all);
PoseArgs make_pose(const double pose_wi[7], const double ext_il[7]);
}

extern "C" {
int p2plane_linearize_begin(lio_map* m, lio_scan* s, const double pose_wi[7], const double ext_il[7], int redo_knn);
int p2plane_linearize_end(lio_map* m, lio_scan* s, const double pose_wi[7], const double ext_il[7], int redo_knn, lio_normal_eq* out);
int scan_share_ds(lio_scan* dst, lio_scan* src, uint32_t n);
int scan_forget_cache(lio_scan* s);
int map_clear(lio_map* m);
int map_incremental_async(lio_map* m, lio_scan* s, const double pose_wi[7], const double ext_il[7], float map_leaf, int ekf_inited, double travel);
int map_settle(lio_map* m);
int map_settle_if_done(lio_map* m);
}
```

lidar-slam-detection_amd/csrc/p2plane.hip:

```cpp
#include "knn_dev.h"
#include "lio_common.h"

namespace lio {


__device__ inline void body_to_world_d(const PoseArgs& P, const float4 pb, double pi[3], float4& pw) {
    const double vx = (double)pb.x, vy = (double)pb.y, vz = (double)pb.z;
    double ux = P.ql[1] * vz - P.ql[2] * vy, uy = P.ql[2] * vx - P.ql[0] * vz, uz = P.ql[0] * vy - P.ql[1] * vx;
    ux += ux; uy += uy; uz += uz;
    double cx = P.ql[1] * uz - P.ql[2] * uy, cy = P.ql[2] * ux - P.ql[0] * uz, cz = P.ql[0] * uy - P.ql[1] * ux;
    pi[0] = ((vx + P.ql[3] * ux) + cx) + P.tl[0];
    pi[1] = ((vy + P.ql[3] * uy) + cy) + P.tl[1];
    pi[2] = ((vz + P.ql[3] * uz) + cz) + P.tl[2];
    ux = P.qw[1] * pi[2] - P.qw[2] * pi[1]; uy = P.qw[2] * pi[0] - P.qw[0] * pi[2]; uz = P.qw[0] * pi[1] - P.qw[1] * pi[0];
    ux += ux; uy += uy; uz += uz;
    cx = P.qw[1] * uz - P.qw[2] * uy; cy = P.qw[2] * ux - P.qw[0] * uz; cz = P.qw[0] * uy - P.qw[1] * ux;
    pw.x = (float)(((pi[0] + P.qw[3] * ux) + cx) + P.tw[0]);
    pw.y = (float)(((pi[1] + P.qw[3] * uy) + cy) + P.tw[1]);
    pw.z = (float)(((pi[2] + P.qw[3] * uz) + cz) + P.tw[2]);
    pw.w = pb.w;
}

__device__ inline bool esti_plane_dev(const float4 pt[5], float threshold, float pabcd[4]) {
    float A[5][3], b[5];
// ... 326 lines not shown
        if (c < kAcc && l == 0) acc[c] = s;
    }
    __syncthreads();
    if (tid < 64) {
        if (tid < 36) {
            int a = tid / 6, c = tid % 6;
            if (a > c) { const int u = a; a = c; c = u; }
            const int t = a * 6 - a * (a - 1) / 2 + (c - a);
            out->JtJ[tid] = acc[t];
        } else if (tid < 42) {
            out->Jtr[tid - 36] = acc[21 + (tid - 36)];
        } else if (tid < 51) {
            const int k = tid - 42;
            int a = k / 3, c = k % 3;
            if (a > c) { const int u = a; a = c; c = u; }
            out->nnT[k] = acc[a * 6 - a * (a - 1) / 2 + (c - a)];
        } else if (tid < 54) {
            out->contri[tid - 51] = 0.0;
        } else if (tid < 57) {
            out->strong[tid - 54] = 0.0;
        } else if (tid == 57) {
            out->sum_abs_res = acc[27];
            out->n_eff = (uint32_t)(acc[28] + 0.5);
            out->n_ds = n;
            out->n_tie = sd->n_tie;
            sd->n_tie_done = sd->n_tie;
            sd->n_tie = 0;
        } else if (tid == 58) {
            unsigned long long kc = 0ull;
            if (md)
                for (int k = 0; k < 64; k++) kc += md->knn_cand[k * 16];
            out->n_knn_candidates_lo = (uint32_t)kc;
            out->n_knn_candidates_hi = (uint32_t)(kc >> 32);
        }
        __threadfence_system();
    }
    __syncthreads();
    if (tid == 0) {
        const uint32_t seq = sd->seq + 1u;
        sd->seq = seq;
        *reinterpret_cast<volatile uint32_t*>(&out->seq) = seq;
    }
}

__global__ void __launch_bounds__(256) degeneracy_kernel(const ScanDev* __restrict__ sd, const uint8_t* __restrict__ selected,
                                                         const float4* __restrict__ normvec, lio_normal_eq* __restrict__ out) {
    const uint32_t n = sd->n_ds;
    if (blockIdx.x * 256u >= n) return;
    __shared__ double red[4][6];
    __shared__ double V[9];
    const int tid = threadIdx.x, wave = tid >> 6, lane = tid & 63;
    if (tid < 9) V[tid] = out->eigvec[tid];
    __syncthreads();
    double s[6] = {0, 0, 0, 0, 0, 0};
    const uint32_t i = blockIdx.x * 256u + tid;
    if (i < n && selected[i]) {
        const float4 nv = normvec[i];
        double f0 = (double)nv.x, f1 = (double)nv.y, f2 = (double)nv.z;
        const double nn = sqrt(f0 * f0 + f1 * f1 + f2 * f2);
        if (nn > 0) { f0 /= nn; f1 /= nn; f2 /= nn; }
#pragma unroll
        for (int e = 0; e < 3; e++) {
            const float dotp = (float)fabs(f0 * V[0 * 3 + e] + f1 * V[1 * 3 + e] + f2 * V[2 * 3 + e]);
            if (dotp > 0.1736f) s[e] += (double)dotp;
            if (dotp > 0.7070f) s[3 + e] += (double)dotp;
        }
    }
#pragma unroll
    for (int e = 0; e < 6; e++) {
        const double v = wave_sum(s[e]);
        if (lane == 0) red[wave][e] = v;
    }
    __syncthreads();
    if (tid < 6) {
        const double v = (red[0][tid] + red[1][tid]) + (red[2][tid] + red[3][tid]);
        if (v != 0.0) atomicAdd(tid < 3 ? &out->contri[tid] : &out->strong[tid - 3], v);
    }
}

constexpr int kStepThreads = 1024;

template <bool JOINT>
__global__ void __launch_bounds__(kStepThreads) step_batch(const SlotDesc* __restrict__ slots, const double* __restrict__ gathered, int world,
                                                           uint32_t n_slots) {
    const SlotDesc& d = slots[blockIdx.x];
    if (!d.active) return;
    EskfDev& cg = *d.ctrl;
    if (cg.status != EK_RUNNING) return;
    __shared__ __attribute__((aligned(16))) EskfDev c;
    __shared__ EkWork w;
    __shared__ double acc[kAcc];
    __shared__ double red6[kStepThreads / 64][6];
    const int tid = threadIdx.x;
    constexpr int kCoreWords = (int)(offsetof(EskfDev, log) / 8);
    EK_STAMP(0);
    const uint32_t n = d.sd->n_ds;
    const bool skip = (d.sd->err & 1u) || n < d.min_ds;
    const uint32_t nb = (n + kLinThreads - 1) / kLinThreads;
    {
        const double* src = reinterpret_cast<const double*>(&cg);
        double* dst = reinterpret_cast<double*>(&c);
        double v0 = 0, v1 = 0;
        const int k0 = tid, k1 = tid + kStepThreads;
        if (k0 < kCoreWords) v0 = src[k0];
        if (k1 < kCoreWords) v1 = src[k1];
        static_assert(kCoreWords <= 2 * kStepThreads, "filter core: two words per thread");
        double s = 0.0;
        const int comp = tid >> 5, l = tid & 31;
        if constexpr (JOINT) {
            if (!skip && tid < kAcc) {
                s = gathered[(size_t)blockIdx.x * 32 + tid];
                for (int r = 1; r < world; r++) s += gathered[((size_t)r * n_slots + blockIdx.x) * 32 + tid];
            }
        } else {
            if (!skip && comp < kAcc) s = fold_partials(d.partial, (uint32_t)l, nb, comp);
        }
        if (k0 < kCoreWords) dst[k0] = v0;
        if (k1 < kCoreWords) dst[k1] = v1;
        if constexpr (JOINT) {
            if (!skip && tid < kAcc) acc[tid] = s;
        } else if (!skip) {
#pragma unroll
            for (int off = 16; off > 0; off >>= 1) s += __shfl_xor(s, off);
            if (comp < kAcc && l == 0) acc[comp] = s;
        }
    }
    __syncthreads();
    EK_STAMP(1);
    if (tid == 0) d.sd->n_tie = 0;
    const int log0 = c.n_log;
    if (skip) {
        if (tid == 0) c.status = EK_SKIPPED;
    } else if (tid < 64) {
        ek_measure_head(c, w, acc, c.converge);
        EK_STAMP(20);
        if constexpr (JOINT) {
            if (w.flag[1]) {
                if (tid == 0) { c.status = EK_NEEDS_HOST; c.n_pass--; if (c.converge) c.n_knn--; w.flag[0] = 0; w.flag[5] = 1; }
                EK_SYNC();
            } else {
                ek_measure_tail(c, w);
            }
        } else {
            if (!w.flag[1]) ek_measure_tail(c, w);
            EK_STAMP(21);
        }
    } else if (tid < 128) {
        ek_step_prep(c, w);
    }
    __syncthreads();
    EK_STAMP(2);
    if (!JOINT && !skip && w.flag[1]) {
        double s6[6] = {0, 0, 0, 0, 0, 0};
        for (uint32_t i = tid; i < n; i += kStepThreads) {
            if (!d.selected[i]) continue;
            const float4 nv = d.normvec[i];
            double f0 = (double)nv.x, f1 = (double)nv.y, f2 = (double)nv.z;
            const double nn = sqrt(f0 * f0 + f1 * f1 + f2 * f2);
            if (nn > 0) { f0 /= nn; f1 /= nn; f2 /= nn; }
#pragma unroll
            for (int e = 0; e < 3; e++) {
                const float dotp = (float)fabs(f0 * w.eigvec[0 * 3 + e] + f1 * w.eigvec[1 * 3 + e] + f2 * w.eigvec[2 * 3 + e]);
                if (dotp > 0.1736f) s6[e] += (double)dotp;
                if (dotp > 0.7070f) s6[3 + e] += (double)dotp;
            }
        }
#pragma unroll
        for (int e = 0; e < 6; e++) {
            const double v = wave_sum(s6[e]);
            if ((tid & 63) == 0) red6[tid >> 6][e] = v;
        }
        __syncthreads();
        if (tid < 6) {
            double v = 0.0;
            for (int k = 0; k < kStepThreads / 64; k++) v += red6[k][tid];
            w.cs[tid] = v;
        }
        __syncthreads();
        if (tid < 64) ek_measure_tail(c, w);
    }
    if (tid >= 64) return;
    EK_STAMP(3);
    if (!skip && c.status == EK_RUNNING && w.flag[0]) ek_step_solve(c, w);
    EK_SYNC();
    EK_STAMP(5);
    {
        const double* src = reinterpret_cast<const double*>(&c);
        double* dst = reinterpret_cast<double*>(&cg);
        for (int k = tid; k < kCoreWords; k += 64) dst[k] = src[k];
        constexpr int kLogWords = (int)(sizeof(EkPassLog) / 8);
        const int log1 = c.n_log < kEkMaxPass ? c.n_log : kEkMaxPass;
        for (int e = log0; e < log1 + (c.status == EK_NEEDS_HOST ? 1 : 0) && e < kEkMaxPass; e++) {
            const double* ls = reinterpret_cast<const double*>(&c.log[e]);
            double* ld = reinterpret_cast<double*>(&cg.log[e]);
            for (int k = tid; k < kLogWords; k += 64) ld[k] = ls[k];
        }
    }
    EK_STAMP(6);
    if (c.status != EK_RUNNING) {
        lio_batch_result* r = d.result;
        if (tid < 26) r->state[tid] = c.x[tid];
        if (tid == 32) {
            r->status = c.status; r->n_pass = c.n_pass; r->n_knn_pass = c.n_knn; r->n_ds = (int32_t)n;
            r->n_eff = c.n_eff_last; r->degenerate = c.is_degenerate; r->radix_passes = (int32_t)((d.sd->nbits + 7u) >> 3); r->err = (int32_t)d.sd->err;
            r->loop_i = c.i; r->loop_t = c.t; r->loop_converge = c.converge; r->pad = 0;
        }
        __threadfence_system();
        EK_SYNC();
        if (tid == 0) *reinterpret_cast<volatile uint32_t*>(&r->seq) = d.seq;
    }
    EK_STAMP(7);
}

#ifdef LIO_STEP_TRACE
extern "C" int lio_debug_step_trace(unsigned long long* out64, int reset) {
    hipDeviceSynchronize();
    if (hipMemcpyFromSymbol(out64, HIP_SYMBOL(g_ek_trace), 64 * sizeof(unsigned long long)) != hipSuccess) return -1;
    if (reset) { unsigned long long z[64] = {0}; hipMemcpyToSymbol(HIP_SYMBOL(g_ek_trace), z, sizeof(z)); }
    return 0;
}
#endif


__global__ void __launch_bounds__(256) share_ds_batch(const SlotDesc* __restrict__ descs, uint32_t n_slots) {
    const uint32_t slot = blockIdx.y % n_slots, m = 1u + blockIdx.y / n_slots;
    const SlotDesc& src = descs[slot];
    const SlotDesc& dst = descs[(size_t)m * n_slots + slot];
    if (!src.active) return;
    const uint32_t n = src.sd->n_ds;
    for (uint32_t i = blockIdx.x * blockDim.x + threadIdx.x; i < n; i += gridDim.x * blockDim.x) dst.ds_body[i] = src.ds_body[i];
    if (blockIdx.x == 0 && threadIdx.x == 0) {
        dst.sd->n_ds_prev = dst.sd->cache_n;
        dst.sd->n_ds = n;
        dst.sd->err = src.sd->err;
        dst.sd->n_tie = 0;
    }
}

int lio_allgather_records_internal(::lio_comm* c, const double* d_local, double* d_gathered, uint32_t n_records, hipStream_t st);
constexpr uint32_t kDsHdrBytes = 256;

__global__ void __launch_bounds__(256) pack_ds_batch(const SlotDesc* __restrict__ descs, uint32_t s0, char* __restrict__ send, size_t slot_bytes, uint32_t cap) {
    const SlotDesc& d = descs[s0 + blockIdx.y];
    char* chunk = send + (size_t)blockIdx.y * slot_bytes;
    uint32_t* hdr = reinterpret_cast<uint32_t*>(chunk);
    float4* pts = reinterpret_cast<float4*>(chunk + kDsHdrBytes);
    uint32_t n = d.active ? d.sd->n_ds : 0u;
    const bool cut = n > cap;
    if (cut) n = cap;
    if (blockIdx.x == 0 && threadIdx.x == 0) {
        hdr[0] = n;
        hdr[1] = d.active ? (d.sd->err | (cut ? 4u : 0u)) : 0u;
        hdr[2] = d.active ? d.sd->nbits : 0u;
        hdr[3] = d.active;
        if (cut) d.sd->err |= 4u;
    }
    for (uint32_t i = blockIdx.x * blockDim.x + threadIdx.x; i < n; i += gridDim.x * blockDim.x) pts[i] = d.ds_body[i];
}
__global__ void __launch_bounds__(256) unpack_ds_batch(const SlotDesc* __restrict__ descs, uint32_t s0, uint32_t s1, const char* __restrict__ all, size_t slot_bytes) {
    const uint32_t slot = blockIdx.y;
    if (slot >= s0 && slot < s1) return;
    const SlotDesc& d = descs[slot];
    if (!d.active) return;
    const char* chunk = all + (size_t)slot * slot_bytes;
    const uint32_t* hdr = reinterpret_cast<const uint32_t*>(chunk);
    const float4* pts = reinterpret_cast<const float4*>(chunk + kDsHdrBytes);
    const uint32_t n = hdr[0];
    for (uint32_t i = blockIdx.x * blockDim.x + threadIdx.x; i < n; i += gridDim.x * blockDim.x) d.ds_body[i] = pts[i];
    if (blockIdx.x == 0 && threadIdx.x == 0) {
        d.sd->n_ds_prev = d.sd->cache_n;
        d.sd->n_ds = n;
        d.sd->err = hdr[1];
        d.sd->nbits = hdr[2];
        d.sd->n_tie = 0;
    }
}

size_t ds_exchange_slot_bytes(uint32_t cap) { return ((size_t)kDsHdrBytes + (size_t)cap * sizeof(float4) + 255u) & ~(size_t)255u; }

int p2plane_batch_exchange_ds(::lio_comm* comm, int world, int (*gather_hook)(void*, const double*, double*, uint32_t, void*), void* gather_ctx, hipStream_t st,
                              const SlotDesc* d_descs, int n_slots, int per, int s0, int s1, uint32_t cap, char* d_send, char* d_all) {
// ... 16 lines not shown
    LIO_HIP_TRY(hipGetLastError());
    (void)world;
    return LIO_OK;
}

__global__ void __launch_bounds__(1024) joint_fold_batch(const SlotDesc* __restrict__ descs, uint32_t n_slots, int n_maps, double* __restrict__ local32) {
    const uint32_t slot = blockIdx.x;
    const SlotDesc& d0 = descs[slot];
    const int tid = threadIdx.x, comp = tid >> 5, l = tid & 31;
    double total = 0.0;
    bool run = d0.active != 0;
    if (run) {
        const EskfDev* c = d0.ctrl;
        const uint32_t n = d0.sd->n_ds;
        run = c->status == EK_RUNNING && !((d0.sd->err & 1u) || n < d0.min_ds);
        if (run) {
            const uint32_t nb = (n + kLinThreads - 1) / kLinThreads;
            for (int m = 0; m < n_maps; m++) {
                const SlotDesc& d = descs[(size_t)m * n_slots + slot];
                double s = 0.0;
                if (comp < kAcc) s = fold_partials(d.partial, (uint32_t)l, nb, comp);
#pragma unroll
                for (int off = 16; off > 0; off >>= 1) s += __shfl_xor(s, off);
                total = m == 0 ? s : total + s;
                if (m > 0 && tid == 0) d.sd->n_tie = 0;
            }
        }
    }
    if (comp < 32 && l == 0) local32[(size_t)slot * 32 + comp] = (run && comp < kAcc) ? total : 0.0;
}

int p2plane_batch_share(hipStream_t st, const SlotDesc* d_descs, int n_slots, int n_maps, uint32_t ds_bound) {
    if (n_maps <= 1) return LIO_OK;
    uint32_t bx = (ds_bound + 255u) / 256u;
    if (bx > 64u) bx = 64u;
    if (bx == 0) bx = 1;
    hipLaunchKernelGGL(share_ds_batch, dim3(bx, (uint32_t)(n_slots * (n_maps - 1))), 256, 0, st, d_descs, (uint32_t)n_slots);
    LIO_HIP_TRY(hipGetLastError());
    return LIO_OK;
}

int p2plane_batch_update_joint(lio_map** maps, int n_maps, ::lio_comm* comm, int world, int (*gather_hook)(void*, const double*, double*, uint32_t, void*),
                               void* gather_ctx, hipStream_t st, const SlotDesc* d_descs, int n_slots, uint32_t ds_bound,
                               int n_passes, double* d_local32, double* d_gathered, BatchTimer* bt, const MapRef* d_rowmaps) {
    uint32_t lin_blocks = (ds_bound + kLinThreads - 1) / kLinThreads;
    if (lin_blocks > kLinGridCap) lin_blocks = kLinGridCap;
    if (lin_blocks == 0) lin_blocks = 1;
    for (int p = 0; p < n_passes; p++) {
        if (d_rowmaps) {
            const int rows = n_maps * n_slots;
            const StencilArgs& sa = maps[0]->stencil;
            const int sid = maps[0]->stencil_id;
            if (bt) bt->begin(1);
            const int rc = knn_seq_launch(st, d_rowmaps, d_descs, rows, (ds_bound + 15) / 16, &sa, &sid, 1);
            if (bt) bt->end(1);
            if (rc != LIO_OK) return rc;
            if (bt) bt->begin(2);
            hipLaunchKernelGGL(linearize_batch, dim3(lin_blocks, (uint32_t)rows), kLinThreads, 0, st, d_descs);
            if (bt) bt->end(2);
        }
        for (int m = 0; m < n_maps && !d_rowmaps; m++) {
            const SlotDesc* row = d_descs + (size_t)m * n_slots;
            if (bt) bt->begin(1);
            const int rc = knn_batch_launch(maps[m], st, row, n_slots, (ds_bound + 15) / 16, 0);
            if (bt) bt->end(1);
            if (rc != LIO_OK) return rc;
            if (bt) bt->begin(2);
            hipLaunchKernelGGL(linearize_batch, dim3(lin_blocks, (uint32_t)n_slots), kLinThreads, 0, st, row);
            if (bt) bt->end(2);
        }
        if (bt) bt->begin(3);
        hipLaunchKernelGGL(joint_fold_batch, dim3((uint32_t)n_slots), 1024, 0, st, d_descs, (uint32_t)n_slots, n_maps, d_local32);
        LIO_HIP_TRY(hipGetLastError());
        const double* sums = d_local32;
        if (gather_hook && world > 1) {
            const int rc = gather_hook(gather_ctx, d_local32, d_gathered, (uint32_t)n_slots, st);
            if (rc != LIO_OK) { set_error("the gather hook returned %d", rc); return rc < 0 ? rc : LIO_E_DEVICE; }
            sums = d_gathered;
        } else if (comm && world > 1) {
            const int rc = lio_allgather_records_internal(comm, d_local32, d_gathered, (uint32_t)n_slots, st);
            if (rc != LIO_OK) return rc;
            sums = d_gathered;
        }
        hipLaunchKernelGGL((step_batch<true>), dim3((uint32_t)n_slots), kStepThreads, 0, st, d_descs, sums, world, (uint32_t)n_slots);
        if (bt) bt->end(3);
    }
    LIO_HIP_TRY(hipGetLastError());
    return LIO_OK;
}

int p2plane_batch_update(lio_map* m, hipStream_t st, const SlotDesc* d_slots, int n_slots, uint32_t ds_bound, int n_passes, BatchTimer* bt, int count_touched) {
    uint32_t lin_blocks = (ds_bound + kLinThreads - 1) / kLinThreads;
    if (lin_blocks > kLinGridCap) lin_blocks = kLinGridCap;
    if (lin_blocks == 0) lin_blocks = 1;
    for (int p = 0; p < n_passes; p++) {
        if (bt) bt->begin(1);
        const int rc = knn_batch_launch(m, st, d_slots, n_slots, (ds_bound + 15) / 16, count_touched);
        if (bt) bt->end(1);
        if (rc != LIO_OK) return rc;
        if (bt) bt->begin(2);
        hipLaunchKernelGGL(linearize_batch, dim3(lin_blocks, (uint32_t)n_slots), kLinThreads, 0, st, d_slots);
        if (bt) { bt->end(2); bt->begin(3); }
        hipLaunchKernelGGL((step_batch<false>), dim3((uint32_t)n_slots), kStepThreads, 0, st, d_slots, static_cast<const double*>(nullptr), 1, (uint32_t)n_slots);
        if (bt) bt->end(3);
    }
    LIO_HIP_TRY(hipGetLastError());
    return LIO_OK;
}

int p2plane_seq_update(hipStream_t st, const MapRef* d_maps, const SlotDesc* d_slots, int n_slots, uint32_t ds_bound, int n_passes, const StencilArgs* stencils,
                       const int* stencil_ids, int n_stencils, BatchTimer* bt) {
    uint32_t lin_blocks = (ds_bound + kLinThreads - 1) / kLinThreads;
    if (lin_blocks > kLinGridCap) lin_blocks = kLinGridCap;
    if (lin_blocks == 0) lin_blocks = 1;
    for (int p = 0; p < n_passes; p++) {
        if (bt) bt->begin(1);
        const int rc = knn_seq_launch(st, d_maps, d_slots, n_slots, (ds_bound + 15) / 16, stencils, stencil_ids, n_stencils);
        if (bt) bt->end(1);
        if (rc != LIO_OK) return rc;
        if (bt) bt->begin(2);
        hipLaunchKernelGGL(linearize_batch, dim3(lin_blocks, (uint32_t)n_slots), kLinThreads, 0, st, d_slots);
        if (bt) { bt->end(2); bt->begin(3); }
        hipLaunchKernelGGL((step_batch<false>), dim3((uint32_t)n_slots), kStepThreads, 0, st, d_slots, static_cast<const double*>(nullptr), 1, (uint32_t)n_slots);
        if (bt) bt->end(3);
    }
    LIO_HIP_TRY(hipGetLastError());
    return LIO_OK;
}

int p2plane_reduce(lio_map* m, lio_scan* s, const PoseArgs& pose, int redo_knn) {
    const uint32_t bound = s->have_ds > 0 ? (uint32_t)s->have_ds : (s->n_raw && s->n_raw < s->max_ds ? s->n_raw : s->max_ds);
    uint32_t blocks = (bound + kLinThreads - 1) / kLinThreads;
    if (blocks == 0) blocks = 1;
    if (blocks > s->partial_blocks) blocks = s->partial_blocks;
    kt_begin(s, 1);
    hipLaunchKernelGGL(linearize_kernel, blocks, kLinThreads, 0, s->stream, pose, redo_knn, s->dev, s->ds_body, s->ds_world, s->nn_pts,
                       s->max_ds, s->nn_cnt, s->selected, s->normvec, s->partial);
    hipLaunchKernelGGL(finalize_kernel, 1, kFinThreads, 0, s->stream, s->dev, s->partial, m ? m->dev : nullptr, s->h_result_dev);
    kt_end(s, 1);
    s->seq_expected++;
    LIO_HIP_TRY(hipGetLastError());
    return LIO_OK;
}

constexpr int kClsThreads = 256;

__device__ __forceinline__ void classify_body(const PoseArgs& pose, const ScanDev* __restrict__ sd, const float4* __restrict__ ds_body,
                                              float4* __restrict__ ds_world, const float4* __restrict__ nn_pts, uint32_t nn_stride,
                                              const int32_t* __restrict__ nn_cnt, float map_leaf, int ekf_inited, int seed_all,
                                              uint8_t* __restrict__ cls, uint32_t* __restrict__ blk_cnt ,
                                              uint32_t vb = 0xFFFFFFFFu, uint32_t stride = 0u) {
    if (vb == 0xFFFFFFFFu) { vb = blockIdx.x; stride = gridDim.x; }
    const uint32_t n = sd->n_ds;
    const uint32_t i = vb * kClsThreads + threadIdx.x;
    int c = 0;
    if (i < n) {
        double pi[3];
        float4 pw;
        body_to_world_d(pose, ds_body[i], pi, pw);
        ds_world[i] = pw;
        const int cnt = nn_cnt[i];
        c = 1;
        if (!seed_all && cnt > 0 && ekf_inited) {
            const double fs = (double)map_leaf;
            float4 mid;
            mid.x = (float)(floor((double)pw.x / fs) * fs + 0.5 * fs);
            mid.y = (float)(floor((double)pw.y / fs) * fs + 0.5 * fs);
            mid.z = (float)(floor((double)pw.z / fs) * fs + 0.5 * fs);
            const float dist = ((pw.x - mid.x) * (pw.x - mid.x) + (pw.y - mid.y) * (pw.y - mid.y)) + (pw.z - mid.z) * (pw.z - mid.z);
            const double half = 0.5 * fs;
            const float4 n0 = nn_pts[i];
            if (fabs((double)(n0.x - mid.x)) > half && fabs((double)(n0.y - mid.y)) > half && fabs((double)(n0.z - mid.z)) > half) {
                c = 2;
            } else if (cnt >= 5) {
#pragma unroll
                for (int k = 0; k < 5; k++) {
                    const float4 q = nn_pts[(size_t)k * nn_stride + i];
                    const float dq = ((q.x - mid.x) * (q.x - mid.x) + (q.y - mid.y) * (q.y - mid.y)) + (q.z - mid.z) * (q.z - mid.z);
                    if (dq < dist) c = 0;
                }
            }
        }
        cls[i] = (uint8_t)c;
    }
    __shared__ uint32_t wc[kClsThreads / 64][2];
    const unsigned long long m1 = __ballot(c == 1), m2 = __ballot(c == 2);
    if ((threadIdx.x & 63) == 0) { wc[threadIdx.x >> 6][0] = __popcll(m1); wc[threadIdx.x >> 6][1] = __popcll(m2); }
    __syncthreads();
    if (threadIdx.x < 2) {
        uint32_t t = 0;
        for (int w = 0; w < kClsThreads / 64; w++) t += wc[w][threadIdx.x];
        blk_cnt[threadIdx.x * stride + vb] = t;
    }
}

__device__ __forceinline__ void classify_scatter_body(const ScanDev* __restrict__ sd, const float4* __restrict__ ds_world,
                                                      const uint8_t* __restrict__ cls, const uint32_t* __restrict__ blk_cnt,
                                                      float4* __restrict__ stage, MapDev* md, uint32_t vb = 0xFFFFFFFFu, uint32_t nb = 0u,
                                                      uint32_t stride = 0u) {
    if (vb == 0xFFFFFFFFu) { vb = blockIdx.x; nb = gridDim.x; stride = gridDim.x; }
    const uint32_t n = sd->n_ds;
    const int tid = threadIdx.x, wave = tid >> 6, lane = tid & 63;
    __shared__ uint32_t red[kClsThreads / 64][3];
    uint32_t preA = 0, preB = 0, totA = 0;
    for (uint32_t b = tid; b < nb; b += kClsThreads) {
        const uint32_t a = blk_cnt[b], bb = blk_cnt[stride + b];
// ... 155 lines not shown
```

lidar-slam-detection_amd/csrc/voxelgrid.hip:

```cpp
#include "device_prims.h"

namespace lio {

constexpr int kThreads = 256;
constexpr int kItems = 8;
constexpr int kTile = kThreads * kItems;
constexpr int kWaves = kThreads / 64;

__device__ __forceinline__ void vg_bbox_atomic_body(const float4* __restrict__ in, uint32_t n, ScanDev* sd) {
    float mn0 = INFINITY, mn1 = INFINITY, mn2 = INFINITY, mx0 = -INFINITY, mx1 = -INFINITY, mx2 = -INFINITY;
    uint32_t cnt = 0;
    const uint32_t stride = gridDim.x * blockDim.x;
    for (uint32_t i = blockIdx.x * blockDim.x + threadIdx.x; i < n; i += 4u * stride) {
        float4 q[4];
#pragma unroll
        for (int k = 0; k < 4; k++) {
            const uint32_t j = i + (uint32_t)k * stride;
            q[k] = in[j < n ? j : i];
        }
#pragma unroll
        for (int k = 0; k < 4; k++) {
            const float4 p = q[k];
            if (i + (uint32_t)k * stride < n && isfinite(p.x) && isfinite(p.y) && isfinite(p.z)) {
                mn0 = fminf(mn0, p.x); mx0 = fmaxf(mx0, p.x);
// ... 804 lines not shown
    if (!d.active || bx >= d.nblocks) return;
    radix_hist_body(d.keys_a, d.keys_b, d.n_raw, pass, d.hist, d.nblocks, d.sd, bx);
}
__global__ void __launch_bounds__(kThreads) radix_scatter_kernel(uint32_t* __restrict__ ka, uint32_t* __restrict__ va,
                                                                 uint32_t* __restrict__ kb, uint32_t* __restrict__ vb, uint32_t n, int pass,
                                                                 const uint32_t* __restrict__ hist, uint32_t nblocks, const ScanDev* sd) {
    radix_scatter_body<false>(ka, va, kb, vb, n, pass, hist, nblocks, sd);
}
__global__ void __launch_bounds__(kThreads) radix_scatter_batch(const SlotDesc* __restrict__ slots, int pass) {
    uint32_t slot, bx;
    vg_slot_tile(gridDim.y, slot, bx);
    const SlotDesc& d = slots[slot];
    if (!d.active || bx >= d.nblocks) return;
    radix_scatter_body<true>(d.keys_a, d.vals_a, d.keys_b, d.vals_b, d.n_raw, pass, d.hist, d.nblocks, d.sd, bx);
}
__global__ void __launch_bounds__(256) radix_prefix_batch(const SlotDesc* __restrict__ slots, int pass) {
    const SlotDesc& d = slots[blockIdx.x];
    if (!d.active) return;
    if ((uint32_t)pass >= active_passes(d.sd)) return;
    const uint32_t nb = d.nblocks;
    uint32_t* col = d.hist + threadIdx.x;
    uint32_t run = 0;
    for (uint32_t b = 0; b < nb; b += 16) {
        uint32_t hv[16];
#pragma unroll
        for (int k = 0; k < 16; k++) hv[k] = col[(size_t)(b + k < nb ? b + k : b) * 256u];
#pragma unroll
        for (int k = 0; k < 16; k++)
            if (b + k < nb) {
                col[(size_t)(b + k) * 256u] = run;
                run += hv[k];
            }
    }
    col[(size_t)nb * 256u] = run;
}
__global__ void __launch_bounds__(kThreads) vg_count_heads_kernel(const uint32_t* __restrict__ ka, const uint32_t* __restrict__ kb, uint32_t n,
                                                                  const ScanDev* sd, uint32_t* __restrict__ blockcnt) {
    vg_count_heads_body(ka, kb, n, sd, blockcnt);
}
__global__ void __launch_bounds__(kThreads) vg_count_heads_batch(const SlotDesc* __restrict__ slots) {
    uint32_t slot, bx;
    vg_slot_tile(gridDim.y, slot, bx);
    const SlotDesc& d = slots[slot];
    if (!d.active || bx >= d.nblocks) return;
    vg_count_heads_body(d.keys_a, d.keys_b, d.n_raw, d.sd, d.blockcnt, bx);
}
__global__ void __launch_bounds__(kThreads) vg_heads_kernel(const float4* __restrict__ in, const uint32_t* __restrict__ ka,
                                                            const uint32_t* __restrict__ kb, const uint32_t* __restrict__ va,
                                                            const uint32_t* __restrict__ vb, uint32_t n, ScanDev* sd,
                                                            const uint32_t* __restrict__ blockcnt, uint32_t* __restrict__ hpos,
                                                            float4* __restrict__ sorted, float4* __restrict__ out, uint32_t* __restrict__ longlist,
                                                            uint32_t max_ds, uint32_t* __restrict__ host_nds, uint32_t launched_passes) {
    vg_heads_body(in, ka, kb, va, vb, n, sd, blockcnt, hpos, sorted, out, longlist, max_ds, host_nds, launched_passes, gridDim.x - 1);
}
__global__ void __launch_bounds__(kThreads) vg_heads_batch(const SlotDesc* __restrict__ slots, uint32_t launched_passes) {
    uint32_t slot, bx;
    vg_slot_tile(gridDim.y, slot, bx);
    const SlotDesc& d = slots[slot];
    if (!d.active || bx >= d.nblocks) return;
    vg_heads_body(d.raw, d.keys_a, d.keys_b, d.vals_a, d.vals_b, d.n_raw, d.sd, d.blockcnt, d.hpos, d.sorted, d.ds_body, d.longlist, d.max_ds, d.host_nds,
                  launched_passes, d.nblocks - 1, bx);
}
__global__ void __launch_bounds__(kThreads) vg_centroid_long_kernel(const float4* __restrict__ sorted, const uint32_t* __restrict__ hpos,
                                                                    const ScanDev* __restrict__ sd, float4* __restrict__ out,
                                                                    const uint32_t* __restrict__ longlist, uint32_t max_ds, uint32_t n_long_blocks) {
    vg_centroid_long_body<0>(sorted, hpos, sd, out, longlist, max_ds, n_long_blocks);
}
__global__ void __launch_bounds__(kThreads) vg_centroid_long_batch(const SlotDesc* __restrict__ slots) {
    const SlotDesc& d = slots[blockIdx.y];
    if (!d.active) return;
    vg_centroid_long_body<1>(d.sorted, d.hpos, d.sd, d.ds_body, d.longlist, d.max_ds, gridDim.x);
}
__global__ void __launch_bounds__(kThreads) vg_centroid_both_batch(const SlotDesc* __restrict__ slots) {
    const SlotDesc& d = slots[blockIdx.y];
    if (!d.active) return;
    vg_centroid_long_body<0>(d.sorted, d.hpos, d.sd, d.ds_body, d.longlist, d.max_ds, gridDim.x - kMonsterBlocksBatch);
}
__global__ void __launch_bounds__(kThreads) vg_centroid_monster_batch(const SlotDesc* __restrict__ slots) {
    const SlotDesc& d = slots[blockIdx.y];
    if (!d.active || d.sd->n_monster == 0) return;
    vg_centroid_long_body<2>(d.sorted, d.hpos, d.sd, d.ds_body, d.longlist, d.max_ds, 0u);
}
__global__ void scan_begin_kernel(ScanDev* sd, int32_t* __restrict__ nn_cnt, uint32_t min_ds) { scan_begin_body(sd, nn_cnt, min_ds, 0u); }
__global__ void scan_begin_batch(const SlotDesc* __restrict__ slots) {
    const SlotDesc& d = slots[blockIdx.y];
    if (!d.active) return;
    scan_begin_body(d.sd, d.nn_cnt, d.min_ds, d.reset_cache);
}

int vg_downsample(lio_scan* s, float leaf, int passes) {
    const uint32_t n = s->n_raw;
    const float inv = 1.0f / leaf;
    hipStream_t st = s->stream;
    const uint32_t nblocks = (n + kTile - 1) / kTile;
    if (n == 0) {
        hipLaunchKernelGGL(scan_set_nds_kernel, 1, 1, 0, st, s->dev, 0u);
        s->host_nds[0] = 0;
        s->host_nds[1] = 0;
        s->host_nds[2] = 0;
        return LIO_OK;
    }
    uint32_t* parts = reinterpret_cast<uint32_t*>(s->sorted);
    hipLaunchKernelGGL(vg_bbox_kernel, nblocks, kThreads, 0, st, s->raw, n, parts);
    hipLaunchKernelGGL(vg_keys_kernel, nblocks, kThreads, 0, st, s->raw, n, inv, s->dev, s->keys_a, s->hist, nblocks, parts);
    for (int pass = 0; pass < passes; pass++) {
        if (pass > 0) hipLaunchKernelGGL(radix_hist_kernel, nblocks, kThreads, 0, st, s->keys_a, s->keys_b, n, pass, s->hist, nblocks, s->dev);
        hipLaunchKernelGGL(radix_scatter_kernel, nblocks, kThreads, 0, st, s->keys_a, s->vals_a, s->keys_b, s->vals_b, n, pass, s->hist, nblocks,
                           s->dev);
    }
    hipLaunchKernelGGL(vg_count_heads_kernel, nblocks, kThreads, 0, st, s->keys_a, s->keys_b, n, s->dev, s->blockcnt);
    hipLaunchKernelGGL(vg_heads_kernel, nblocks, kThreads, 0, st, s->raw, s->keys_a, s->keys_b, s->vals_a, s->vals_b, n, s->dev, s->blockcnt,
                       s->hpos, s->sorted, s->ds_body, s->longlist, s->max_ds, s->host_nds_dev, (uint32_t)passes);
    hipLaunchKernelGGL(vg_centroid_long_kernel, 256 + kMonsterBlocks, kThreads, 0, st, s->sorted, s->hpos, s->dev, s->ds_body, s->longlist, s->max_ds, 256u);
    LIO_HIP_TRY(hipGetLastError());
    return LIO_OK;
}

int vg_downsample_batch(hipStream_t st, const SlotDesc* d_slots, int n_slots, uint32_t max_raw, uint32_t max_ds, float leaf, int passes) {
    const float inv = 1.0f / leaf;
    const uint32_t nblocks = (max_raw + kTile - 1) / kTile;
    if (nblocks == 0 || n_slots <= 0) return LIO_OK;
    const uint32_t B = (uint32_t)n_slots;
    hipLaunchKernelGGL(vg_bbox_batch, dim3(nblocks < 48 ? nblocks : 48, B), kThreads, 0, st, d_slots);
    hipLaunchKernelGGL(vg_keys_batch, dim3(nblocks, B), kThreads, 0, st, d_slots, inv);
    for (int pass = 0; pass < passes; pass++) {
        if (pass > 0) hipLaunchKernelGGL(radix_hist_batch, dim3(nblocks, B), kThreads, 0, st, d_slots, pass);
        hipLaunchKernelGGL(radix_prefix_batch, dim3(B), 256, 0, st, d_slots, pass);
        hipLaunchKernelGGL(radix_scatter_batch, dim3(nblocks, B), kThreads, 0, st, d_slots, pass);
    }
    hipLaunchKernelGGL(vg_count_heads_batch, dim3(nblocks, B), kThreads, 0, st, d_slots);
    hipLaunchKernelGGL(vg_heads_batch, dim3(nblocks, B), kThreads, 0, st, d_slots, (uint32_t)passes);
    static const bool split = []() { const char* e = getenv("LIO_VG_MONSTER_SPLIT"); return e && e[0] == '1'; }();
    if (split) {
        hipLaunchKernelGGL(vg_centroid_long_batch, dim3(64, B), kThreads, 0, st, d_slots);
        hipLaunchKernelGGL(vg_centroid_monster_batch, dim3(kMonsterBlocksBatch, B), kThreads, 0, st, d_slots);
    } else {
        hipLaunchKernelGGL(vg_centroid_both_batch, dim3(64 + kMonsterBlocksBatch, B), kThreads, 0, st, d_slots);
    }
    hipLaunchKernelGGL(scan_begin_batch, dim3(16, B), 256, 0, st, d_slots);
    LIO_HIP_TRY(hipGetLastError());
    return LIO_OK;
}

int scan_begin_rows(hipStream_t st, const SlotDesc* d_descs, int n_rows) {
    if (n_rows <= 0) return LIO_OK;
    hipLaunchKernelGGL(scan_begin_batch, dim3(16, (uint32_t)n_rows), 256, 0, st, d_descs);
    LIO_HIP_TRY(hipGetLastError());
    return LIO_OK;
}

int scan_begin(lio_scan* s) {
    hipLaunchKernelGGL(scan_begin_kernel, 64, 256, 0, s->stream, s->dev, s->nn_cnt, s->resize_min);
    LIO_HIP_TRY(hipGetLastError());
    return LIO_OK;
}

int scan_set_nds(lio_scan* s, uint32_t n) {
    hipLaunchKernelGGL(scan_set_nds_kernel, 1, 1, 0, s->stream, s->dev, n);
    LIO_HIP_TRY(hipGetLastError());
    return LIO_OK;
}

}
```

lidar-slam-detection_amd/python/lsd_amd/capi.py:

```python
import ctypes as C
import os

import numpy as np

_HERE = os.path.dirname(os.path.abspath(__file__))
os.environ.setdefault("GPU_MAX_HW_QUEUES", "8")
LIB_PATH = os.environ.get("LIO_HIP_LIB") or os.path.join(_HERE, "liblio_hip.so")

LIO_OK, LIO_E_INVALID, LIO_E_CAPACITY, LIO_E_DEVICE, LIO_E_STATE = 0, -1, -2, -3, -4
MAIN_FIRST_SCAN, MAIN_SEEDED, MAIN_SKIPPED, MAIN_UPDATED, MAIN_IMU_INIT, MAIN_IDLE = 0, 1, 2, 3, 4, 5

SYMBOLS = [
    "lio_last_warning",
    "lio_last_error", "lio_device_count", "lio_map_bytes",
    "lio_map_create", "lio_map_destroy", "lio_map_set_lru", "lio_map_lru_stats", "lio_map_lru_exact_stats", "lio_map_set_tie_mode", "lio_map_tie_stats", "lio_map_clear", "lio_map_pool_stats", "lio_map_set_stencil", "lio_map_insert", "lio_map_insert_device", "lio_map_stats",
    "lio_abi_version", "lio_pinned_alloc", "lio_pinned_free",
    "lio_map_dump", "lio_map_knn", "lio_map_knn_candidates", "lio_map_knn_touched", "lio_map_knn_unique",
    "lio_scan_create", "lio_scan_destroy", "lio_scan_reset", "lio_scan_upload", "lio_scan_set_device", "lio_scan_undistort_delta", "lio_scan_undistort_poses", "lio_scan_undistort_imu", "lio_scan_download_raw", "lio_scan_voxel_downsample", "lio_scan_voxel_downsample_batch", "lio_scan_set_ds",
    "lio_scan_num_ds", "lio_scan_download_ds", "lio_scan_download_world", "lio_scan_download_match",
    "lio_p2plane_linearize", "lio_scan_set_degeneracy_mode", "lio_p2plane_degeneracy", "lio_engine_set_reduce_hook", "lio_p2plane_rows", "lio_map_incremental", "lio_map_seed",
    "lio_engine_create", "lio_engine_create_shared", "lio_engine_destroy", "lio_engine_map", "lio_engine_scan", "lio_engine_set_state", "lio_engine_get_state",
    "lio_engine_set_cov", "lio_engine_get_cov", "lio_engine_set_flags", "lio_engine_travel", "lio_engine_is_degenerate",
    "lio_engine_update", "lio_engine_pass_log", "lio_engine_process_scan", "lio_engine_process_scan_device", "lio_engine_timings", "lio_engine_flush",
    "lio_engine_enable_timing", "lio_comm_unique_id", "lio_comm_init", "lio_comm_destroy", "lio_comm_rank", "lio_comm_world", "lio_allgather_normal_eq", "lio_comm_stats", "lio_engine_set_joint", "lio_engine_joint_register", "lio_engine_joint_register_device", "lio_allgather_records", "lio_engines_process_batch", "lio_batch_create", "lio_batch_create_joint", "lio_batch_create_sequences", "lio_batch_sequences_step", "lio_batch_fastlio_main", "lio_batch_set_gather_hook", "lio_batch_exchange_stats", "lio_batch_destroy", "lio_batch_process", "lio_batch_engine", "lio_batch_enable_kernel_timing", "lio_batch_kernel_times", "lio_engine_set_static_map", "lio_scan_enable_kernel_timing", "lio_scan_kernel_times",
    "lio_state_boxplus", "lio_state_boxminus",
    "lio_localmap_create", "lio_localmap_destroy", "lio_localmap_add_keyframe", "lio_localmap_num_keyframes", "lio_localmap_update",
    "lio_localmap_download",
    "lio_localmap_nearest", "lio_localmap_gather", "lio_localmap_z_mean", "lio_localmap_download_gather", "lio_localmap_gather_device", "lio_localmap_store_frame",
    "lio_localmap_frame", "lio_estimate_matcher_params", "lio_localmap_estimate_pose", "lio_scan_ds_device", "lio_gicp_set_target_device", "lio_gicp_set_source_device",
    "lio_cloud_create", "lio_cloud_destroy", "lio_cloud_clear", "lio_cloud_size", "lio_cloud_append_scan", "lio_cloud_append_host",
    "lio_cloud_voxel_downsample", "lio_cloud_download", "lio_cloud_scratch_bytes", "lio_cloud_last_times",
    "lio_knn_index_create", "lio_knn_index_destroy", "lio_knn_index_build", "lio_knn_index_query", "lio_knn_index_colour", "lio_knn_index_last_times",
    "lio_ground_default_params", "lio_ground_draw", "lio_ground_create", "lio_ground_destroy", "lio_ground_detect_scan", "lio_ground_detect_host",
    "lio_ground_download_indices", "lio_ground_download_normals", "lio_ground_download_inliers", "lio_ground_download_draws", "lio_ground_last_run",
    "lio_ground_last_times",
    "lio_bev_create", "lio_bev_destroy", "lio_bev_preprocess_host", "lio_bev_preprocess_cloud", "lio_bev_upload_pixels", "lio_bev_convert", "lio_bev_get_info",
    "lio_bev_download_pixel_coords", "lio_bev_download_kept", "lio_bev_download_pixels", "lio_bev_download_nodes", "lio_bev_download_equalised",
    "lio_bev_download_image", "lio_bev_grey_table", "lio_bev_last_times",
    "lio_keyframe_decide", "lio_keyframer_default_params", "lio_keyframer_create", "lio_keyframer_destroy", "lio_keyframer_reset", "lio_keyframer_push_host",
    "lio_keyframer_pending", "lio_keyframer_pop", "lio_radius_outlier_host", "lio_keyframe_filter_host", "lio_keyframer_fitness_host",
    "lio_keyframer_append_local_map_host", "lio_keyframer_download_local_map", "lio_keyframer_last_times",
    "lio_pose_estimator_create", "lio_pose_estimator_destroy", "lio_pose_estimator_predict", "lio_pose_estimator_match", "lio_pose_estimator_match_gps", "lio_pose_estimator_guess", "lio_pose_estimator_observe",
    "lio_pose_estimator_match_gps_only", "lio_pose_estimator_get_timed_pose", "lio_pose_estimator_predict_nostate",
    "lio_pose_estimator_correct", "lio_pose_estimator_get_dt", "lio_pose_estimator_get", "lio_pose_estimator_set", "lio_pose_estimator_matrix",
    "lio_fastlio_init", "lio_fastlio_is_init", "lio_fastlio_imu_enqueue", "lio_engine_set_device_loop", "lio_fastlio_ins_enqueue", "lio_fastlio_set_wheelspeed", "lio_fastlio_pcl_enqueue", "lio_fastlio_pcl_enqueue_device", "lio_fastlio_pcl_stage", "lio_fastlio_pcl_commit",
    "lio_fastlio_main", "lio_fastlio_odometry", "lio_fastlio_state", "lio_fastlio_start_state", "lio_fastlio_download_undistorted",
    "lio_state_predict", "lio_eskf_update_cb", "lio_eskf_update_ws_cb", "lio_eskf_update_sums_cb",
    "lio_ndt_create", "lio_ndt_destroy", "lio_ndt_set_target", "lio_ndt_set_target_device", "lio_ndt_num_voxels", "lio_ndt_fitness_score", "lio_ndt_overlap_score", "lio_ndt_voxel_at",
    "lio_ndt_linearize", "lio_ndt_default_params", "lio_ndt_align", "lio_ndt_align_batch", "lio_ndt_enable_kernel_timing", "lio_ndt_kernel_times",
    "lio_gicp_create", "lio_gicp_destroy", "lio_gicp_set_target", "lio_gicp_set_source", "lio_gicp_set_voxel_mode", "lio_gicp_voxel_at", "lio_gicp_download", "lio_gicp_correspondences", "lio_gicp_neighbours", "lio_gicp_mahalanobis", "lio_gicp_linearize", "lio_gicp_align", "lio_gicp_fitness_score",
    "lio_loop_default_params", "lio_loop_find_candidates", "lio_loop_information_matrix", "lio_loop_create", "lio_loop_destroy", "lio_loop_reset",
    "lio_loop_add_keyframe_host", "lio_loop_set_pose", "lio_loop_num_keyframes", "lio_loop_download_keyframe", "lio_loop_detect", "lio_loop_edges",
    "lio_loop_last_report", "lio_loop_last_times", "lio_loop_align_candidates", "lio_loop_align_fine", "lio_loop_pair_information",
    "lio_overlap_default_params", "lio_overlap_connection_count", "lio_overlap_find_candidates", "lio_overlap_create", "lio_overlap_destroy",
    "lio_overlap_gate_batch", "lio_overlap_align_pairs", "lio_overlap_accumulate", "lio_overlap_download_accum", "lio_overlap_detect",
    "lio_overlap_last_report", "lio_overlap_last_times",
    "lio_sc_create", "lio_sc_destroy", "lio_sc_reset", "lio_sc_num_frames", "lio_sc_add_frames_host", "lio_sc_download_frame", "lio_sc_describe_host", "lio_sc_set_active",
    "lio_sc_distance", "lio_sc_search", "lio_sc_global_search_host", "lio_sc_shift_to_yaw", "lio_sc_last_dropped", "lio_sc_last_times",
    "lio_sc_set_positions", "lio_sc_local_search", "lio_sc_last_local", "lio_update_origin",
    "lio_graph_default_params", "lio_graph_create", "lio_graph_destroy", "lio_graph_reset", "lio_graph_add_node", "lio_graph_set_fixed", "lio_graph_set_estimate",
    "lio_graph_num_nodes", "lio_graph_get_fixed", "lio_graph_add_edge", "lio_graph_remove_edge", "lio_graph_optimize", "lio_graph_estimates", "lio_graph_edges",
    "lio_graph_chi2", "lio_graph_linearize", "lio_graph_last_times", "lio_se3_from_mqt", "lio_se3_to_mqt", "lio_graph_edge_error",
    "lio_graph_add_prior", "lio_graph_set_kernel", "lio_graph_priors", "lio_graph_prior_error", "lio_graph_remove_gnss_outliers",
    "lio_graph_remove_node", "lio_graph_node_live", "lio_graph_edge_records", "lio_loop_retire",
    "lio_render_create", "lio_render_destroy", "lio_render_clear", "lio_render_set_cameras", "lio_render_set_active", "lio_render_frame", "lio_render_size",
    "lio_render_download", "lio_render_download_voxels", "lio_render_download_points", "lio_render_download_last_image", "lio_render_last_times",
    "lio_utm_create", "lio_utm_destroy", "lio_utm_zone", "lio_utm_forward", "lio_utm_inverse", "lio_utm_longitude0", "lio_grid_convergence",
    "lio_transform_from_rpyt", "lio_quat_of_transform", "lio_interpolate_transform", "lio_rtk_transform_utm", "lio_rtk_transform_origin",
    "lio_rtk_track_create", "lio_rtk_track_destroy", "lio_rtk_track_set_origin", "lio_rtk_track_origin", "lio_rtk_track_feed", "lio_rtk_track_size",
    "lio_rtk_track_interpolate",
    "lio_gnss_queue_create", "lio_gnss_queue_destroy", "lio_gnss_queue_set_origin", "lio_gnss_queue_push", "lio_gnss_queue_size", "lio_gnss_queue_stamps",
    "lio_gnss_queue_flush",
    "lio_scan_merge_create", "lio_scan_merge_destroy", "lio_scan_merge_set_transform", "lio_scan_merge_run_host", "lio_scan_merge_download",
    "lio_scan_merge_device", "lio_scan_merge_last_times",
    "lio_calib_subsample", "lio_se3f_exp", "lio_se3f_log", "lio_se3f_mul", "lio_se3f_inverse", "lio_se3f_matrix", "lio_se3f_from_matrix",
    "lio_calib_interpolate", "lio_dfo_default_params", "lio_dfo_direct_l", "lio_dfo_nelder_mead", "lio_calib_default_params",
    "lio_calib_ins_create", "lio_calib_ins_destroy", "lio_calib_ins_reset", "lio_calib_ins_add_scan", "lio_calib_ins_add_odom", "lio_calib_ins_counts",
    "lio_calib_ins_set_transform", "lio_calib_ins_scan_matrices", "lio_calib_ins_combined", "lio_calib_ins_error", "lio_calib_ins_error_terms",
    "lio_calib_ins_calibrate", "lio_calib_ins_progress", "lio_calib_ins_result", "lio_calib_ins_last_times",
]
ABI_VERSION = 22
ABI_REQUIRED = 23
RTK_INTERPOLATED, RTK_EXACT, RTK_NO_ORIGIN, RTK_TOO_FEW, RTK_EARLY, RTK_LATE = 0, 1, 2, 3, 4, 5


class NormalEq(C.Structure):
    _fields_ = [("JtJ", C.c_double * 36), ("Jtr", C.c_double * 6), ("nnT", C.c_double * 9), ("eigvec", C.c_double * 9),
                ("eigval", C.c_double * 3), ("contri", C.c_double * 3), ("strong", C.c_double * 3), ("sum_abs_res", C.c_double),
                ("n_eff", C.c_uint32), ("n_ds", C.c_uint32), ("n_knn_candidates_lo", C.c_uint32), ("n_knn_candidates_hi", C.c_uint32),
                ("n_tie", C.c_uint32), ("seq", C.c_uint32)]


class BatchTimes(C.Structure):
    _fields_ = [("downsample_us", C.c_double), ("knn_us", C.c_double), ("linearize_us", C.c_double), ("step_us", C.c_double),
                ("downsample_launches", C.c_uint32), ("knn_launches", C.c_uint32), ("linearize_launches", C.c_uint32), ("step_launches", C.c_uint32),
                ("insert_us", C.c_double), ("insert_launches", C.c_uint32), ("pad", C.c_uint32)]


class PassLog(C.Structure):
    _fields_ = [("knn", C.c_int32), ("n_eff", C.c_int32), ("valid", C.c_int32), ("degenerate", C.c_int32), ("sum_abs_res", C.c_double),
                ("JtJ", C.c_double * 36), ("Jtr", C.c_double * 6), ("dx", C.c_double * 23)]


SUMS_FN = C.CFUNCTYPE(C.c_int, C.c_void_p, C.POINTER(C.c_double), C.c_int, C.POINTER(C.c_double))
DEG_FN = C.CFUNCTYPE(None, C.c_void_p, C.POINTER(C.c_double), C.POINTER(C.c_double))
MEAS_FN = C.CFUNCTYPE(C.c_int, C.c_void_p, C.POINTER(C.c_double), C.c_int, C.POINTER(C.c_int), C.POINTER(C.c_double), C.POINTER(C.c_double), C.c_int)

# ... 200 lines not shown
    sig("lio_map_bytes", u64, vp)
    sig("lio_map_create", vp, cint, flt, u64, u64, cint)
    sig("lio_map_destroy", None, vp)
    sig("lio_map_set_stencil", cint, vp, cint)
    sig("lio_map_insert", cint, vp, f32p, u64, dbl)
    sig("lio_map_insert_device", cint, vp, vp, u64, dbl)
    sig("lio_map_stats", cint, vp, C.POINTER(u64), C.POINTER(u64))
    sig("lio_map_dump", C.c_int64, vp, f32p, u64)
    sig("lio_map_set_lru", cint, vp, u64, dbl)
    sig("lio_map_lru_stats", cint, vp, C.POINTER(u64), C.POINTER(u64))
    sig("lio_map_lru_exact_stats", cint, vp, C.POINTER(u64), C.POINTER(u64))
    sig("lio_map_clear", cint, vp)
    sig("lio_map_set_tie_mode", cint, vp, cint)
    sig("lio_map_tie_stats", cint, vp, C.POINTER(u64), C.POINTER(u64))
    sig("lio_map_pool_stats", cint, vp, C.POINTER(u64), C.POINTER(u64))
    sig("lio_map_knn_candidates", u64, vp)
    sig("lio_map_knn_touched", u64, vp)
    sig("lio_map_knn_unique", u64, vp)
    sig("lio_map_knn", cint, vp, f32p, u32, f32p, i32p)
    sig("lio_scan_create", vp, cint, u32, u32)
    sig("lio_scan_destroy", None, vp)
    sig("lio_scan_reset", cint, vp)
    sig("lio_scan_upload", cint, vp, f32p, u32)
    sig("lio_scan_set_device", cint, vp, vp, u32)
    sig("lio_scan_undistort_delta", cint, vp, vp, cint, f32p, C.c_double)
    sig("lio_scan_undistort_poses", cint, vp, vp, cint, u64, C.POINTER(u64), f64p, u32)
    sig("lio_scan_undistort_imu", cint, vp, vp, cint, f64p, u32, f64p, f64p, f64p, f64p, dbl, cint, cint)
    sig("lio_scan_download_raw", cint, vp, f32p, u32)
    sig("lio_scan_voxel_downsample", cint, vp, flt, cint, C.POINTER(u32))
    sig("lio_scan_voxel_downsample_batch", cint, C.POINTER(vp), cint, flt, C.POINTER(u32))
    sig("lio_scan_set_ds", cint, vp, f32p, u32)
    sig("lio_scan_num_ds", cint, vp)
    sig("lio_scan_download_ds", cint, vp, f32p, u32)
    sig("lio_scan_download_world", cint, vp, f32p, u32)
    sig("lio_scan_download_match", cint, vp, u8p, f32p, i32p, f32p)
    sig("lio_p2plane_linearize", cint, vp, vp, f64p, f64p, cint, C.POINTER(NormalEq))
    sig("lio_scan_set_degeneracy_mode", cint, vp, cint)
    sig("lio_p2plane_degeneracy", cint, vp, f64p, f64p, f64p)
    sig("lio_engine_set_reduce_hook", cint, vp, REDUCE_FN, vp)
    sig("lio_p2plane_rows", cint, vp, f64p, f64p, f64p, f64p, u32)
    sig("lio_map_incremental", cint, vp, vp, f64p, f64p, flt, cint, dbl)
    sig("lio_map_seed", cint, vp, vp, f64p, f64p, dbl)
    sig("lio_engine_create", vp, cint, flt, cint, u64, u64, u32, u32)
    sig("lio_engine_create_shared", vp, vp, u32, u32)
    sig("lio_engine_destroy", None, vp)
    sig("lio_engine_map", vp, vp)
    sig("lio_engine_scan", vp, vp)
    sig("lio_engine_set_state", cint, vp, f64p)
    sig("lio_engine_get_state", cint, vp, f64p)
    sig("lio_engine_set_cov", cint, vp, f64p)
    sig("lio_engine_get_cov", cint, vp, f64p)
    sig("lio_engine_set_flags", cint, vp, cint, cint, dbl, dbl)
    sig("lio_engine_travel", dbl, vp)
    sig("lio_engine_is_degenerate", cint, vp)
    sig("lio_engine_update", cint, vp)
    sig("lio_engine_pass_log", cint, vp, cint, C.POINTER(PassLog))
    sig("lio_engine_process_scan", cint, vp, f32p, u32, dbl)
    sig("lio_engine_process_scan_device", cint, vp, vp, u32, dbl)
    sig("lio_engine_timings", cint, vp, C.POINTER(Timings))
    sig("lio_engine_flush", cint, vp)
    sig("lio_engine_enable_timing", cint, vp, cint)
    sig("lio_engines_process_batch", cint, C.POINTER(vp), cint, C.POINTER(ScanJob), cint)
    sig("lio_comm_unique_id", cint, C.POINTER(C.c_uint8))
    sig("lio_comm_init", vp, cint, cint, cint, C.POINTER(C.c_uint8))
    sig("lio_comm_destroy", None, vp)
    sig("lio_comm_rank", cint, vp)
    sig("lio_comm_world", cint, vp)
    sig("lio_allgather_normal_eq", cint, vp, vp, vp, vp, vp)
    sig("lio_comm_stats", cint, vp, C.POINTER(u64), f64p)
    sig("lio_engine_set_joint", cint, vp, C.POINTER(vp), cint, vp)
    sig("lio_engine_joint_register", cint, vp, f32p, u32, dbl, f64p, f64p)
    sig("lio_engine_joint_register_device", cint, vp, vp, u32, dbl, f64p, f64p)
    sig("lio_allgather_records", cint, vp, vp, vp, u32, vp)
    sig("lio_batch_create_joint", vp, C.POINTER(vp), cint, vp, cint, cint, u32, u32)
    sig("lio_batch_set_gather_hook", cint, vp, GATHER_FN, vp, cint, cint)
    sig("lio_batch_exchange_stats", cint, vp, C.POINTER(C.c_uint32), C.POINTER(C.c_uint64), C.POINTER(C.c_uint64))
    sig("lio_batch_create", vp, vp, cint, cint, u32, u32)
    sig("lio_batch_create_sequences", vp, cint, C.c_float, cint, u64, u64, cint, cint, u32, u32)
    sig("lio_batch_sequences_step", cint, vp, C.POINTER(ScanJob), cint, C.POINTER(C.c_double))
    sig("lio_batch_fastlio_main", cint, vp, C.POINTER(cint))
    sig("lio_batch_destroy", None, vp)
    sig("lio_batch_process", cint, vp, C.POINTER(ScanJob), cint)
    sig("lio_batch_engine", vp, vp, cint, cint)
    sig("lio_batch_enable_kernel_timing", cint, vp, cint)
    sig("lio_batch_kernel_times", cint, vp, C.POINTER(BatchTimes), cint)
    sig("lio_engine_set_static_map", cint, vp, cint)
    sig("lio_localmap_create", vp, cint, u64, u32, u32)
    sig("lio_localmap_destroy", None, vp)
    sig("lio_localmap_add_keyframe", cint, vp, f32p, u32, f32p)
    sig("lio_localmap_num_keyframes", cint, vp)
    sig("lio_localmap_update", cint, vp, vp, f64p, dbl, dbl, dbl, flt, C.POINTER(cint), C.POINTER(u32))
    sig("lio_localmap_download", cint, vp, f32p, u32)
    sig("lio_localmap_nearest", cint, vp, f64p, u32, i32p, f32p)
    sig("lio_localmap_gather", cint, vp, i32p, u32, C.POINTER(u32), f64p)
    sig("lio_localmap_z_mean", cint, vp, vp, u32, f64p)
    sig("lio_localmap_download_gather", cint, vp, f32p, u32)
    sig("lio_localmap_gather_device", vp, vp, C.POINTER(u32))
    sig("lio_localmap_store_frame", cint, vp, cint, vp, u32)
    sig("lio_localmap_frame", vp, vp, cint, C.POINTER(u32))
    sig("lio_estimate_matcher_params", None, C.POINTER(NdtParams))
    sig("lio_localmap_estimate_pose", cint, vp, vp, vp, u32, f64p, C.POINTER(EstimateReport), f64p)
    sig("lio_scan_ds_device", vp, vp, C.POINTER(u32))
    sig("lio_cloud_create", vp, cint, u64)
    sig("lio_cloud_destroy", None, vp)
    sig("lio_cloud_clear", cint, vp)
    sig("lio_cloud_size", cint, vp, C.POINTER(u64))
    sig("lio_cloud_append_scan", cint, vp, vp, f64p, flt, cint, dbl, dbl)
    sig("lio_cloud_append_host", cint, vp, f32p, u64, f64p, flt, cint, dbl, dbl)
    sig("lio_cloud_voxel_downsample", cint, vp, flt, C.POINTER(u64))
    sig("lio_cloud_download", C.c_int64, vp, f32p, u64)
    sig("lio_cloud_scratch_bytes", cint, vp, C.POINTER(u64))
    sig("lio_cloud_last_times", cint, vp, f64p, f64p)
    sig("lio_knn_index_create", vp, cint)
    sig("lio_knn_index_destroy", None, vp)
    sig("lio_knn_index_build", cint, vp, f32p, C.POINTER(C.c_uint32), u64, C.POINTER(u64))
    sig("lio_knn_index_query", cint, vp, f32p, u64, cint, i32p, f32p)
    sig("lio_knn_index_colour", cint, vp, f32p, u64, cint, u8p)
    sig("lio_knn_index_last_times", cint, vp, f64p, f64p)
    gp, u32p = C.POINTER(GroundParams), C.POINTER(u32)
    sig("lio_ground_default_params", None, gp, cint)
    sig("lio_ground_draw", None, u32, u32, u32, u32p)
    sig("lio_ground_create", vp, cint)
    sig("lio_ground_destroy", None, vp)
    sig("lio_ground_detect_scan", cint, vp, vp, gp, cint, C.POINTER(cint), f32p, u32p, u32p, u32p)
    sig("lio_ground_detect_host", cint, vp, f32p, u64, gp, C.POINTER(cint), f32p, u32p, u32p, u32p)
    sig("lio_ground_download_indices", C.c_int64, vp, cint, u32p, u64)
    sig("lio_ground_download_normals", C.c_int64, vp, f32p, u64)
    sig("lio_ground_download_inliers", C.c_int64, vp, f32p, u64)
    sig("lio_ground_download_draws", C.c_int64, vp, u32p, u32p, f32p, u64)
    sig("lio_ground_last_run", cint, vp, C.POINTER(cint), C.POINTER(cint), C.POINTER(cint), C.POINTER(cint))
    sig("lio_ground_last_times", cint, vp, f64p, f64p)
    kp, kr, u64p = C.POINTER(KeyframerParams), C.POINTER(KeyframeReport), C.POINTER(u64)
    sig("lio_keyframe_decide", cint, f64p, f64p, dbl, dbl, C.POINTER(cint), C.POINTER(cint), f64p, f64p)
    sig("lio_keyframer_default_params", None, kp)
    sig("lio_keyframer_create", vp, cint, kp)
    sig("lio_keyframer_destroy", None, vp)
    sig("lio_keyframer_reset", cint, vp)
    sig("lio_keyframer_push_host", cint, vp, f32p, u32p, u32, u64, f64p, f64p, u64p, f64p, u32, kr)
    sig("lio_keyframer_pending", cint, vp)
    sig("lio_keyframer_pop", C.c_int64, vp, f32p, u64, f64p, u64p, f64p, u32p, u32p)
    sig("lio_radius_outlier_host", C.c_int64, vp, f32p, u64, dbl, cint, u32p, u64, u32p)
    sig("lio_keyframe_filter_host", C.c_int64, vp, f32p, u64, dbl, cint, dbl, u32p, u64, u32p, u32p)
    sig("lio_keyframer_fitness_host", cint, vp, f32p, u32, f64p, f64p, u32p)
    sig("lio_keyframer_append_local_map_host", cint, vp, f32p, u32, f64p)
    sig("lio_keyframer_download_local_map", C.c_int64, vp, f32p, u64)
    sig("lio_keyframer_last_times", cint, vp, f64p, f64p, f64p, f64p)
    u16p = C.POINTER(C.c_uint16)
    sig("lio_bev_create", vp, cint)
    sig("lio_bev_destroy", None, vp)
    sig("lio_bev_preprocess_host", cint, vp, f32p, u64, dbl)
    sig("lio_bev_preprocess_cloud", cint, vp, vp, dbl)
    sig("lio_bev_upload_pixels", cint, vp, u32p, f32p, f32p, u64, u32, u32)
    sig("lio_bev_convert", cint, vp, dbl, dbl)
    sig("lio_bev_get_info", cint, vp, C.POINTER(BevInfo))
    sig("lio_bev_download_pixel_coords", C.c_int64, vp, i32p, u64)
    sig("lio_bev_download_kept", C.c_int64, vp, u32p, u64)
    sig("lio_bev_download_pixels", C.c_int64, vp, u32p, f32p, f32p, u64)
    sig("lio_bev_download_nodes", C.c_int64, vp, u32p, i32p, f64p, u64)
    sig("lio_bev_download_equalised", C.c_int64, vp, f32p, u64)
    sig("lio_bev_download_image", C.c_int64, vp, u16p, u64)
    sig("lio_bev_grey_table", None, u16p)
    sig("lio_bev_last_times", cint, vp, f64p, f64p)
    sig("lio_pose_estimator_create", vp, f32p, u64, f32p, f32p, dbl)
    sig("lio_pose_estimator_destroy", None, vp)
    sig("lio_pose_estimator_predict", cint, vp, u64, f32p, f32p)
    sig("lio_pose_estimator_match", cint, vp, vp, vp, C.POINTER(NdtParams), f32p, C.POINTER(cint))
# ... 243 lines not shown
```

lidar-slam-detection_amd/python/lsd_amd/lio.py:

```python
import ctypes as C

import numpy as np

from . import capi
from .capi import check, f32, f64, lib, ptr

STATE_DIM = 26
DOF = 23
G_LEN = 9.809


def default_state():
    s = np.zeros(STATE_DIM)
    s[6] = 1.0
    s[10] = 1.0
    s[23] = G_LEN
    return s


def init_cov():
    P = np.eye(23)
    for i in (6, 7, 8, 9, 10, 11):
        P[i, i] = 0.00001
    for i in (15, 16, 17):
# ... 1647 lines not shown

    @staticmethod
    def unique_id():
        u = (C.c_uint8 * 128)()
        check(lib().lio_comm_unique_id(u), "comm unique id")
        return bytes(u)

    def allgather(self, d_local, d_gathered, d_sum=None, stream=None):
        check(lib().lio_allgather_normal_eq(self.h, d_local, d_gathered, d_sum, stream), "allgather")

    def stats(self):
        n, t = C.c_uint64(), C.c_double()
        check(lib().lio_comm_stats(self.h, C.byref(n), C.byref(t)))
        return n.value, t.value

    def close(self):
        if getattr(self, "h", None) and lib is not None:
            lib().lio_comm_destroy(self.h)
        self.h = None

    __del__ = close


class Batch:

    def __init__(self, shared_map, n_slots=8, n_groups=3, max_raw=262144, max_ds=100000, sub_maps=None, comm=None):
        self.map = shared_map
        self.n_slots, self.n_groups = n_slots, n_groups
        self._keep = (list(sub_maps or []), comm)
        if sub_maps or comm is not None:
            ms = [shared_map] + list(sub_maps or [])
            hs = (C.c_void_p * len(ms))(*[m.h for m in ms])
            self.h = lib().lio_batch_create_joint(hs, len(ms), comm.h if comm is not None else None, n_slots, n_groups, max_raw, max_ds)
        else:
            self.h = lib().lio_batch_create(shared_map.h, n_slots, n_groups, max_raw, max_ds)
        if not self.h:
            raise capi.LioError("lio_batch_create failed: " + lib().lio_last_error().decode())

    def close(self):
        if getattr(self, "h", None) and lib is not None:
            lib().lio_batch_destroy(self.h)
        self.h = None

    __del__ = close

    def set_gather_hook(self, fn, rank, world):

        def _cb(_ctx, d_local, d_gathered, n, stream):
            try:
                return int(fn(int(d_local or 0), int(d_gathered or 0), int(n), int(stream or 0)) or 0)
            except Exception:
                import traceback

                traceback.print_exc()
                return -1

        self._gather = capi.GATHER_FN(_cb)
        check(lib().lio_batch_set_gather_hook(self.h, self._gather, None, int(rank), int(world)), "set_gather_hook")

    def exchange_stats(self):
        cap, again, nbytes = C.c_uint32(0), C.c_uint64(0), C.c_uint64(0)
        check(lib().lio_batch_exchange_stats(self.h, C.byref(cap), C.byref(again), C.byref(nbytes)))
        return {"chunk_points": cap.value, "jobs_rerun": again.value, "bytes_per_rank_and_round": nbytes.value}

    def enable_kernel_timing(self, on=True):
        check(lib().lio_batch_enable_kernel_timing(self.h, int(on)))

    def kernel_times(self, reset=True):
        t = capi.BatchTimes()
        check(lib().lio_batch_kernel_times(self.h, C.byref(t), int(reset)))
        return {k: getattr(t, k) for k, _ in t._fields_}

    def engine(self, group, slot):
        h = lib().lio_batch_engine(self.h, group, slot)
        if not h:
            raise capi.LioError("no such slot")
        e = Engine.__new__(Engine)
        e.h = h
        e._own = False
        e.map = self.map
        e.scan = Scan(max_ds=100000, _borrow=lib().lio_engine_scan(h))
        return e

    def process(self, jobs):
        return process_batch(None, jobs, batch=self)


JOB_KEEP_CACHE = 1
JOB_IDLE = 2
JOB_HOST_RAW = 4


class PinnedCloud:

    def __init__(self, pts):
        pts = np.ascontiguousarray(pts, dtype=np.float32).reshape(-1, 4)
        self.n = len(pts)
        self.nbytes = max(pts.nbytes, 16)
        self.ptr = lib().lio_pinned_alloc(self.nbytes)
        if not self.ptr:
            raise MemoryError((lib().lio_last_error() or b'').decode())
        self.array = np.ctypeslib.as_array(C.cast(self.ptr, C.POINTER(C.c_float)), shape=(max(self.n, 1), 4))[: self.n]
        self.array[...] = pts

    def __del__(self):
        try:
            if getattr(self, "ptr", None):
                self.array = None
                lib().lio_pinned_free(self.ptr)
                self.ptr = None
        except Exception:
            pass


class SequenceBatch:

    def __init__(self, n_slots=8, n_groups=1, resolution=0.5, stencil=19, max_points=2_000_000, max_voxels=1_000_000, max_raw=262144, max_ds=100000, device=0):
        self.n_slots, self.n_groups = n_slots, n_groups
        self.n = n_slots * n_groups
        self.h = lib().lio_batch_create_sequences(device, resolution, stencil, max_points, max_voxels, n_slots, n_groups, max_raw, max_ds)
        if not self.h:
            raise capi.LioError("lio_batch_create_sequences failed: " + lib().lio_last_error().decode())
        self.arr = (capi.ScanJob * self.n)()
        self.states_in = np.zeros((self.n, STATE_DIM))
        self.covs_in = np.zeros((self.n, 23 * 23))
        self.states_out = np.zeros((self.n, STATE_DIM))
        self.covs_out = np.zeros((self.n, 23 * 23))
        for i in range(self.n):
            a = self.arr[i]
            a.state_in = self.states_in[i].ctypes.data_as(C.POINTER(C.c_double))
            a.cov_in = self.covs_in[i].ctypes.data_as(C.POINTER(C.c_double))
            a.state_out = self.states_out[i].ctypes.data_as(C.POINTER(C.c_double))

    def close(self):
        if getattr(self, "h", None) and lib is not None:
            lib().lio_batch_destroy(self.h)
        self.h = None

    __del__ = close

    def engine(self, session):
        h = lib().lio_batch_engine(self.h, session // self.n_slots, session % self.n_slots)
        if not h:
            raise capi.LioError("no such session")
        e = Engine.__new__(Engine)
        e.h = h
        e._own = False
        e.map = Map(_borrow=lib().lio_engine_map(h))
        e.scan = Scan(max_ds=100000, _borrow=lib().lio_engine_scan(h))
        return e

    def enable_kernel_timing(self, on=True):
        check(lib().lio_batch_enable_kernel_timing(self.h, int(on)))

    def kernel_times(self, reset=True):
        t = capi.BatchTimes()
        check(lib().lio_batch_kernel_times(self.h, C.byref(t), int(reset)))
        return {k: getattr(t, k) for k, _ in t._fields_}

    def fastlio_main(self):
        if not hasattr(self, "_fl_rc"):
            self._fl_rc = (C.c_int * self.n)()
        rc = lib().lio_batch_fastlio_main(self.h, self._fl_rc)
        return rc, list(self._fl_rc)

    def load(self, jobs):
# ... 744 lines not shown
```

Before: 6.199 billion.

## Compact KNN batch grid to only still-iterating slots via device-side search list

Scan begin and each step kernel now record on the device which slots are still running and unconverged, and the batched KNN kernel launches a flattened 1D grid that spreads workgroups only across those listed slots. The aim is to stop launching and early-exiting blocks for slots that have already converged, so later iterate passes use the whole GPU for the remaining slots. The cost is an extra indirection and a readfirstlane load per block. A new posterior query API is added for inspection.

```diff
diff --git a/include/lio_hip.h b/include/lio_hip.h
--- a/include/lio_hip.h
+++ b/include/lio_hip.h
@@ -20,7 +20,7 @@
 const char* lio_last_error(void);
 const char* lio_last_warning(void);
 int lio_device_count(void);
-#define LIO_ABI_VERSION 24
+#define LIO_ABI_VERSION 25
 int lio_abi_version(void);
 void* lio_pinned_alloc(uint64_t bytes);
 void lio_pinned_free(void* p);
@@ -227,6 +227,7 @@
 int lio_batch_enable_kernel_timing(lio_batch*, int on);
 int lio_batch_kernel_times(lio_batch*, lio_batch_times* out, int reset);
 lio_engine* lio_batch_engine(lio_batch*, int group, int slot);
+int lio_batch_slot_posterior(lio_batch*, int group, int slot, double* cov529, int32_t* n_eff, int32_t* degenerate, uint32_t* search_n8);
 int lio_engine_set_static_map(lio_engine*, int on);
 
 typedef struct lio_ndt lio_ndt;
diff --git a/lidar-slam-detection_amd/csrc/batch.hip b/lidar-slam-detection_amd/csrc/batch.hip
--- a/lidar-slam-detection_amd/csrc/batch.hip
+++ b/lidar-slam-detection_amd/csrc/batch.hip
@@ -47,6 +47,7 @@
     SlotDesc* h_desc = nullptr;
     EskfDev* d_ctrl = nullptr;
     EskfDev* h_ctrl = nullptr;
+    uint32_t* d_search = nullptr;
     hipGraphExec_t exec[5] = {nullptr, nullptr, nullptr, nullptr, nullptr};
     const void* graph_table = nullptr;
     int graph_stencil = 0;
@@ -273,7 +274,7 @@
             if (rc != LIO_OK) return rc;
         } else {
             if (bt) bt->begin(0);
-            rc = vg_downsample_batch(g.stream, g.d_desc, B, b->max_raw, b->max_ds, 0.5f, passes);
+            rc = vg_downsample_batch(g.stream, g.d_desc, B, b->max_raw, b->max_ds, 0.5f, passes, g.d_search);
             if (bt) bt->end(0);
             if (rc != LIO_OK) return rc;
         }
@@ -284,7 +285,7 @@
             return p2plane_batch_update_joint(b->maps.data(), M, b->comm, b->world, b->gather_hook, b->gather_ctx, g.stream, g.d_desc, B, ds_bound, 5, g.d_local32, g.d_gathered, bt,
                                               rowmaps);
         }
-        return p2plane_batch_update(b->map, g.stream, g.d_desc, B, ds_bound, 5, bt, bt ? b->count_touched : 0);
+        return p2plane_batch_update(b->map, g.stream, g.d_desc, B, ds_bound, 5, bt, bt ? b->count_touched : 0, g.d_search);
     };
     if (!b->use_graph || timed || b->joint) return enqueue(timed ? g.bt : nullptr);
     if (g.graph_table != b->map->table || g.graph_stencil != b->map->stencil.n) {
@@ -356,7 +357,8 @@
     for (Group& g : b->groups) {
         g.job_of_slot.assign(n_slots, -1);
         const size_t desc_bytes = sizeof(SlotDesc) * (size_t)n_slots * (size_t)M;
-        g.block_bytes = desc_bytes + sizeof(EskfDev) * (size_t)n_slots;
+        const size_t search_at = (desc_bytes + sizeof(EskfDev) * (size_t)n_slots + 15u) & ~(size_t)15u;
+        g.block_bytes = search_at + sizeof(uint32_t) * knn_search_words(n_slots);
         ok = ok && hipMalloc(reinterpret_cast<void**>(&g.d_block), g.block_bytes) == hipSuccess;
         ok = ok && hipHostMalloc(reinterpret_cast<void**>(&g.h_block), g.block_bytes, hipHostMallocDefault) == hipSuccess;
         if (ok) {
@@ -364,6 +366,7 @@
             g.h_desc = reinterpret_cast<SlotDesc*>(g.h_block);
             g.d_ctrl = reinterpret_cast<EskfDev*>(g.d_block + desc_bytes);
             g.h_ctrl = reinterpret_cast<EskfDev*>(g.h_block + desc_bytes);
+            g.d_search = b->joint ? nullptr : reinterpret_cast<uint32_t*>(g.d_block + search_at);
         }
         ok = ok && hipHostMalloc(reinterpret_cast<void**>(&g.h_res), sizeof(lio_batch_result) * n_slots, hipHostMallocMapped) == hipSuccess;
         ok = ok && hipHostGetDevicePointer(reinterpret_cast<void**>(&g.h_res_dev), g.h_res, 0) == hipSuccess;
@@ -492,6 +495,21 @@
         out->insert_launches += g.bt->launches[4];
         if (reset)
             for (int c = 0; c < BatchTimer::kClasses; c++) { g.bt->us[c] = 0; g.bt->launches[c] = 0; }
+    }
+    return LIO_OK;
+}
+
+int lio_batch_slot_posterior(lio_batch* b, int group, int slot, double* cov529, int32_t* n_eff, int32_t* degenerate, uint32_t* search_n8) {
+    if (!b || group < 0 || group >= (int)b->groups.size() || slot < 0 || slot >= b->n_slots) return LIO_E_INVALID;
+    hipSetDevice(b->device);
+    Group& g = b->groups[group];
+    LIO_HIP_TRY(hipStreamSynchronize(g.stream));
+    if (cov529) LIO_HIP_TRY(hipMemcpy(cov529, g.d_ctrl[slot].P, sizeof(double) * 529, hipMemcpyDeviceToHost));
+    if (n_eff) *n_eff = g.h_res[slot].n_eff;
+    if (degenerate) *degenerate = g.h_res[slot].degenerate;
+    if (search_n8) {
+        memset(search_n8, 0, sizeof(uint32_t) * kKnnSearchHead);
+        if (g.d_search) LIO_HIP_TRY(hipMemcpy(search_n8, g.d_search, sizeof(uint32_t) * kKnnSearchHead, hipMemcpyDeviceToHost));
     }
     return LIO_OK;
 }
diff --git a/lidar-slam-detection_amd/csrc/knn.hip b/lidar-slam-detection_amd/csrc/knn.hip
--- a/lidar-slam-detection_amd/csrc/knn.hip
+++ b/lidar-slam-detection_amd/csrc/knn.hip
@@ -1,5 +1,6 @@
 #include "hashgrid.h"
 #include "knn_dev.h"
+#include "knn_spread.h"
 #include "lio_common.h"
 #include "refsel.h"
 
@@ -298,7 +299,7 @@
                                          float inv_res, const StencilArgs& st, PoseFill fill, const float4* __restrict__ queries,
                                          uint32_t n_host, const ScanDev* __restrict__ sd, float4* __restrict__ world_out,
                                          float4* __restrict__ nn_pts, uint32_t nn_stride, int32_t* __restrict__ nn_cnt,
-                                         MapDev* md, uint32_t* __restrict__ n_tie, uint32_t* __restrict__ tie_list) {
+                                         MapDev* md, uint32_t* __restrict__ n_tie, uint32_t* __restrict__ tie_list, const uint32_t bx, const uint32_t nwg) {
     __shared__ GroupLds lds[kGPB];
     const int tid = threadIdx.x;
     const int grp = tid / kG, gl = tid % kG;
@@ -317,14 +318,14 @@
 
     const uint32_t nblk = (n + kGPB - 1) / kGPB;
     const uint32_t per_xcd = (nblk + 7u) >> 3;
-    const uint32_t wg_per_xcd = gridDim.x >> 3;
+    const uint32_t wg_per_xcd = nwg >> 3;
     constexpr uint32_t kAhead = 64 / kGPB;
     __shared__ float4 pw_s[64];
     __shared__ PoseArgs pose_s;
     if constexpr (MODE == 0) fill(pose_s);
     uint32_t ahead = kAhead;
-    for (uint32_t j = blockIdx.x >> 3; j < per_xcd; j += wg_per_xcd) {
-        const uint32_t q0 = ((blockIdx.x & 7u) * per_xcd + j) * kGPB;
+    for (uint32_t j = bx >> 3; j < per_xcd; j += wg_per_xcd) {
+        const uint32_t q0 = ((bx & 7u) * per_xcd + j) * kGPB;
         const uint32_t q = q0 + grp;
         const bool active = q < n;
         float4 pw = make_float4(0.f, 0.f, 0.f, 0.f);
@@ -333,7 +334,7 @@
                 __syncthreads();
                 if (tid < 64) {
                     const uint32_t j2 = j + (uint32_t)(tid / kGPB) * wg_per_xcd;
-                    const uint32_t q2 = ((blockIdx.x & 7u) * per_xcd + j2) * kGPB + (uint32_t)(tid % kGPB);
+                    const uint32_t q2 = ((bx & 7u) * per_xcd + j2) * kGPB + (uint32_t)(tid % kGPB);
                     if (j2 < per_xcd && q2 < n) {
                         float4 w2;
                         body_to_world(pose_s, queries[q2], w2);
@@ -527,18 +528,29 @@
                                                   float4* __restrict__ nn_pts, uint32_t nn_stride, int32_t* __restrict__ nn_cnt,
                                                   MapDev* md, uint32_t* __restrict__ n_tie, uint32_t* __restrict__ tie_list) {
     knn_body<KM, MODE>(table, mask, pool, inv_res, st, [&](PoseArgs& P) { if (threadIdx.x == 0) P = pose; }, queries, n_host, sd, world_out, nn_pts, nn_stride, nn_cnt, md,
-                       n_tie, tie_list);
+                       n_tie, tie_list, blockIdx.x, gridDim.x);
 }
 template <int KM, bool COUNT>
 __global__ void LIO_KNN_OCC __launch_bounds__(256, COUNT ? LIO_KNN_WAVES : LIO_KNN_WAVES_BATCH) knn_batch_kernel(const Slot* __restrict__ table, uint32_t mask, const float4* __restrict__ pool,
-                                                                       float inv_res, StencilArgs st, const SlotDesc* __restrict__ slots, MapDev* md) {
-    const SlotDesc& d = slots[blockIdx.y];
+                                                                       float inv_res, StencilArgs st, const SlotDesc* __restrict__ slots, MapDev* md,
+                                                                       const uint32_t* __restrict__ search, uint32_t n_slots, uint32_t pass) {
+    uint32_t slot = blockIdx.y, bx = blockIdx.x, nwg = gridDim.x;
+    if (search) {
+        uint32_t S = (uint32_t)__builtin_amdgcn_readfirstlane((int)search[pass]);
+        if (S > n_slots) S = n_slots;
+        const KnnSpreadRow r = knn_spread_row(gridDim.x, S, blockIdx.x);
+        if (r.row >= S) return;
+        slot = (uint32_t)__builtin_amdgcn_readfirstlane((int)search[kKnnSearchHead + pass * n_slots + r.row]);
+        if (slot >= n_slots) return;
+        bx = r.bx; nwg = r.nwg;
+    }
+    const SlotDesc& d = slots[slot];
     if (!d.active) return;
     const SlotGateLite sg = slot_gate_lite(d);
     if ((sg.status != EK_RUNNING) | (sg.converge == 0) | (sg.n_ds < d.min_ds)) return;
     const double* __restrict__ x = d.ctrl->x;
     knn_body<KM, 0, COUNT>(table, mask, pool, inv_res, st, [x](PoseArgs& P) { pose_fill_from_state(P, x); }, d.ds_body, sg.n_ds, nullptr, d.ds_world, d.nn_pts,
-                                  d.max_ds, d.nn_cnt, md, &d.sd->n_tie, d.tie_list);
+                                  d.max_ds, d.nn_cnt, md, &d.sd->n_tie, d.tie_list, bx, nwg);
 }
 
 constexpr int kSelCap = 2560;
@@ -832,22 +844,25 @@
     knn_exact_body<KM, 0>(table, mask, pool, inv_res, st, pose, d.ds_body, d.nn_pts, d.max_ds, &d.sd->n_tie, d.tie_list, tie_mode);
 }
 
-int knn_batch_launch(lio_map* m, hipStream_t st, const SlotDesc* d_slots, int n_slots, uint32_t grid_x, int count_touched) {
+int knn_batch_launch(lio_map* m, hipStream_t st, const SlotDesc* d_slots, int n_slots, uint32_t grid_x, int count_touched, const uint32_t* d_search, int pass) {
     static const uint32_t forced = [] { const char* e = getenv("LIO_KNN_GRID"); const int v = e ? atoi(e) : 0; return v >= 8 ? (uint32_t)v : 0u; }();
     uint32_t cap = forced ? forced : (12288u / (uint32_t)(n_slots > 0 ? n_slots : 1));
     if (cap > 2048u) cap = 2048u;
     if (cap < 128u) cap = 128u;
+    const uint32_t blocks_bound = grid_x;
     if (grid_x > cap) grid_x = cap;
     if (grid_x == 0) grid_x = 8;
-    const dim3 grid((grid_x + 7u) & ~7u, (uint32_t)n_slots);
+    dim3 grid((grid_x + 7u) & ~7u, (uint32_t)n_slots);
+    if (d_search) grid = dim3(knn_spread_launch_size((uint32_t)n_slots, blocks_bound, forced), 1u);
     const dim3 gridx(n_slots > 8 ? 8 : 64, (uint32_t)n_slots);
     const int tmode = m->pool_seq ? m->tie_mode : 0;
     const int km = (m->stencil.n + kG - 1) / kG;
+    const uint32_t ns = (uint32_t)n_slots, ps = (uint32_t)pass;
     if (count_touched && m->touch_bits) LIO_HIP_TRY(hipMemsetAsync(m->touch_bits, 0, (size_t)((m->pool_cap + 31) / 32) * 4, st));
 #define KNNB_LAUNCH(KM)                                                                                                                              \
     do {                                                                                                                                             \
-        if (count_touched) hipLaunchKernelGGL((knn_batch_kernel<KM, true>), grid, 256, 0, st, m->table, m->table_mask, m->pool, m->inv_res, m->stencil, d_slots, m->dev); \
-        else hipLaunchKernelGGL((knn_batch_kernel<KM, false>), grid, 256, 0, st, m->table, m->table_mask, m->pool, m->inv_res, m->stencil, d_slots, m->dev); \
+        if (count_touched) hipLaunchKernelGGL((knn_batch_kernel<KM, true>), grid, 256, 0, st, m->table, m->table_mask, m->pool, m->inv_res, m->stencil, d_slots, m->dev, d_search, ns, ps); \
+        else hipLaunchKernelGGL((knn_batch_kernel<KM, false>), grid, 256, 0, st, m->table, m->table_mask, m->pool, m->inv_res, m->stencil, d_slots, m->dev, d_search, ns, ps); \
         hipLaunchKernelGGL((knn_exact_batch_kernel<KM>), gridx, 256, 0, st, m->table, m->table_mask, m->pool, m->inv_res, m->stencil, d_slots, tmode); \
     } while (0)
     if (km <= 1) KNNB_LAUNCH(1);
@@ -873,7 +888,7 @@
     if ((sg.status != EK_RUNNING) | (sg.converge == 0) | (sg.n_ds < d.min_ds)) return;
     const double* __restrict__ x = d.ctrl->x;
     knn_body<KM, 0, false>(r.table, r.mask, r.pool, r.inv_res, st, [x](PoseArgs& P) { pose_fill_from_state(P, x); }, d.ds_body, sg.n_ds, nullptr, d.ds_world, d.nn_pts,
-                                  d.max_ds, d.nn_cnt, r.md, &d.sd->n_tie, d.tie_list);
+                                  d.max_ds, d.nn_cnt, r.md, &d.sd->n_tie, d.tie_list, blockIdx.x, gridDim.x);
 }
 template <int KM>
 __global__ void __launch_bounds__(256) knn_exact_seq_kernel(const MapRef* __restrict__ maps, StencilArgs st, int stencil_id, const SlotDesc* __restrict__ slots) {
diff --git a/lidar-slam-detection_amd/csrc/knn_spread.h b/lidar-slam-detection_amd/csrc/knn_spread.h
--- /dev/null
+++ b/lidar-slam-detection_amd/csrc/knn_spread.h
@@ -0,0 +1,69 @@
+#pragma once
+#include <stdint.h>
+
+#if defined(__HIPCC__)
+#define LIO_SPREAD_FN __host__ __device__ __forceinline__
+#else
+#define LIO_SPREAD_FN inline
+#endif
+
+namespace lio {
+
+constexpr uint32_t kKnnSpreadTotal = 12288;
+constexpr uint32_t kKnnSpreadPerSlot = 2048;
+
+LIO_SPREAD_FN uint32_t knn_spread_per_slot(uint32_t G, uint32_t S) {
+    if (S == 0u || G < 8u) return 0u;
+    uint32_t W = (G / S) & ~7u;
+    if (W > kKnnSpreadPerSlot) W = kKnnSpreadPerSlot;
+    if (W < 8u) W = 8u;
+    return W;
+}
+
+struct KnnSpreadRow {
+    uint32_t row, rows;
+    uint32_t bx, nwg;
+};
+LIO_SPREAD_FN KnnSpreadRow knn_spread_row(uint32_t G, uint32_t S, uint32_t w) {
+    KnnSpreadRow r;
+    const uint32_t W = knn_spread_per_slot(G, S);
+    r.nwg = W;
+    r.rows = W ? G / W : 0u;
+    r.row = W ? w / W : 0u;
+    r.bx = W ? w - r.row * W : 0u;
+    return r;
+}
+
+struct KnnSpreadBlocks {
+    uint32_t xcd, per_xcd;
+    uint32_t first, stride, end;
+};
+LIO_SPREAD_FN KnnSpreadBlocks knn_spread_blocks(uint32_t nblk, uint32_t bx, uint32_t nwg) {
+    KnnSpreadBlocks b;
+    b.xcd = bx & 7u;
+    b.per_xcd = (nblk + 7u) >> 3;
+    b.stride = nwg >> 3;
+    const uint32_t lo = b.xcd * b.per_xcd, hi = lo + b.per_xcd;
+    b.first = lo + (bx >> 3);
+    b.end = hi < nblk ? hi : nblk;
+    if (b.end < lo) b.end = lo;
+    return b;
+}
+
+LIO_SPREAD_FN uint32_t knn_spread_launch_size(uint32_t n_slots, uint32_t per_slot_bound, uint32_t forced) {
+    if (n_slots == 0u) n_slots = 1u;
+    if (forced) {
+        const uint32_t G = (forced + 7u) & ~7u;
+        return G > 8u * n_slots ? G : 8u * n_slots;
+    }
+    uint32_t cap = kKnnSpreadTotal / n_slots;
+    if (cap > kKnnSpreadPerSlot) cap = kKnnSpreadPerSlot;
+    if (cap < 128u) cap = 128u;
+    uint32_t bound = (per_slot_bound + 7u) & ~7u;
+    if (bound == 0u) bound = 8u;
+    if (cap > bound) cap = bound;
+    cap = (cap + 7u) & ~7u;
+    return cap * n_slots;
+}
+
+}
diff --git a/lidar-slam-detection_amd/csrc/lio_common.h b/lidar-slam-detection_amd/csrc/lio_common.h
--- a/lidar-slam-detection_amd/csrc/lio_common.h
+++ b/lidar-slam-detection_amd/csrc/lio_common.h
@@ -312,8 +312,11 @@
                      const UndistortArgs& args, unsigned long long* d_block_min );
 
 int vg_downsample(lio_scan* s, float leaf, int passes );
-int vg_downsample_batch(hipStream_t st, const SlotDesc* d_slots, int n_slots, uint32_t max_raw, uint32_t max_ds, float leaf, int passes);
-int knn_batch_launch(lio_map* m, hipStream_t st, const SlotDesc* d_slots, int n_slots, uint32_t grid_x, int count_touched);
+constexpr uint32_t kKnnSearchHead = 8;
+inline size_t knn_search_words(int n_slots) { return (size_t)kKnnSearchHead * (size_t)(1 + n_slots); }
+int vg_downsample_batch(hipStream_t st, const SlotDesc* d_slots, int n_slots, uint32_t max_raw, uint32_t max_ds, float leaf, int passes, uint32_t* d_search = nullptr);
+int knn_batch_launch(lio_map* m, hipStream_t st, const SlotDesc* d_slots, int n_slots, uint32_t grid_x, int count_touched, const uint32_t* d_search = nullptr,
+                     int pass = 0);
 struct BatchTimer {
     static constexpr int kClasses = 5;
     static constexpr int kPool = 256;
@@ -335,7 +338,8 @@
         }
     }
 };
-int p2plane_batch_update(lio_map* m, hipStream_t st, const SlotDesc* d_slots, int n_slots, uint32_t ds_bound, int n_passes, BatchTimer* bt, int count_touched);
+int p2plane_batch_update(lio_map* m, hipStream_t st, const SlotDesc* d_slots, int n_slots, uint32_t ds_bound, int n_passes, BatchTimer* bt, int count_touched,
+                         uint32_t* d_search = nullptr);
 int knn_seq_launch(hipStream_t st, const MapRef* d_maps, const SlotDesc* d_slots, int n_slots, uint32_t grid_x, const StencilArgs* stencils, const int* stencil_ids,
                    int n_stencils);
 int p2plane_seq_update(hipStream_t st, const MapRef* d_maps, const SlotDesc* d_slots, int n_slots, uint32_t ds_bound, int n_passes, const StencilArgs* stencils,
diff --git a/lidar-slam-detection_amd/csrc/p2plane.hip b/lidar-slam-detection_amd/csrc/p2plane.hip
--- a/lidar-slam-detection_amd/csrc/p2plane.hip
+++ b/lidar-slam-detection_amd/csrc/p2plane.hip
@@ -432,7 +432,7 @@
 
 template <bool JOINT>
 __global__ void __launch_bounds__(kStepThreads) step_batch(const SlotDesc* __restrict__ slots, const double* __restrict__ gathered, int world,
-                                                           uint32_t n_slots) {
+                                                           uint32_t n_slots, uint32_t* __restrict__ search, uint32_t next_pass) {
     const SlotDesc& d = slots[blockIdx.x];
     if (!d.active) return;
     EskfDev& cg = *d.ctrl;
@@ -547,6 +547,10 @@
         }
     }
     EK_STAMP(6);
+    if (search && tid == 0 && next_pass < kKnnSearchHead && c.status == EK_RUNNING && c.converge != 0) {
+        const uint32_t at = atomicAdd(&search[next_pass], 1u);
+        if (at < n_slots) search[kKnnSearchHead + next_pass * n_slots + at] = blockIdx.x;
+    }
     if (c.status != EK_RUNNING) {
         lio_batch_result* r = d.result;
         if (tid < 26) r->state[tid] = c.x[tid];
@@ -729,26 +733,28 @@
             if (rc != LIO_OK) return rc;
             sums = d_gathered;
         }
-        hipLaunchKernelGGL((step_batch<true>), dim3((uint32_t)n_slots), kStepThreads, 0, st, d_descs, sums, world, (uint32_t)n_slots);
+        hipLaunchKernelGGL((step_batch<true>), dim3((uint32_t)n_slots), kStepThreads, 0, st, d_descs, sums, world, (uint32_t)n_slots, static_cast<uint32_t*>(nullptr), 0u);
         if (bt) bt->end(3);
     }
     LIO_HIP_TRY(hipGetLastError());
     return LIO_OK;
 }
 
-int p2plane_batch_update(lio_map* m, hipStream_t st, const SlotDesc* d_slots, int n_slots, uint32_t ds_bound, int n_passes, BatchTimer* bt, int count_touched) {
+int p2plane_batch_update(lio_map* m, hipStream_t st, const SlotDesc* d_slots, int n_slots, uint32_t ds_bound, int n_passes, BatchTimer* bt, int count_touched,
+                         uint32_t* d_search) {
+    if (n_passes > (int)kKnnSearchHead) d_search = nullptr;
     uint32_t lin_blocks = (ds_bound + kLinThreads - 1) / kLinThreads;
     if (lin_blocks > kLinGridCap) lin_blocks = kLinGridCap;
     if (lin_blocks == 0) lin_blocks = 1;
     for (int p = 0; p < n_passes; p++) {
         if (bt) bt->begin(1);
-        const int rc = knn_batch_launch(m, st, d_slots, n_slots, (ds_bound + 15) / 16, count_touched);
+        const int rc = knn_batch_launch(m, st, d_slots, n_slots, (ds_bound + 15) / 16, count_touched, d_search, p);
         if (bt) bt->end(1);
         if (rc != LIO_OK) return rc;
         if (bt) bt->begin(2);
         hipLaunchKernelGGL(linearize_batch, dim3(lin_blocks, (uint32_t)n_slots), kLinThreads, 0, st, d_slots);
         if (bt) { bt->end(2); bt->begin(3); }
-        hipLaunchKernelGGL((step_batch<false>), dim3((uint32_t)n_slots), kStepThreads, 0, st, d_slots, static_cast<const double*>(nullptr), 1, (uint32_t)n_slots);
+        hipLaunchKernelGGL((step_batch<false>), dim3((uint32_t)n_slots), kStepThreads, 0, st, d_slots, static_cast<const double*>(nullptr), 1, (uint32_t)n_slots, d_search, (uint32_t)(p + 1));
         if (bt) bt->end(3);
     }
     LIO_HIP_TRY(hipGetLastError());
@@ -768,7 +774,7 @@
         if (bt) bt->begin(2);
         hipLaunchKernelGGL(linearize_batch, dim3(lin_blocks, (uint32_t)n_slots), kLinThreads, 0, st, d_slots);
         if (bt) { bt->end(2); bt->begin(3); }
-        hipLaunchKernelGGL((step_batch<false>), dim3((uint32_t)n_slots), kStepThreads, 0, st, d_slots, static_cast<const double*>(nullptr), 1, (uint32_t)n_slots);
+        hipLaunchKernelGGL((step_batch<false>), dim3((uint32_t)n_slots), kStepThreads, 0, st, d_slots, static_cast<const double*>(nullptr), 1, (uint32_t)n_slots, static_cast<uint32_t*>(nullptr), 0u);
         if (bt) bt->end(3);
     }
     LIO_HIP_TRY(hipGetLastError());
diff --git a/lidar-slam-detection_amd/csrc/voxelgrid.hip b/lidar-slam-detection_amd/csrc/voxelgrid.hip
--- a/lidar-slam-detection_amd/csrc/voxelgrid.hip
+++ b/lidar-slam-detection_amd/csrc/voxelgrid.hip
@@ -910,9 +910,16 @@
     vg_centroid_long_body<2>(d.sorted, d.hpos, d.sd, d.ds_body, d.longlist, d.max_ds, 0u);
 }
 __global__ void scan_begin_kernel(ScanDev* sd, int32_t* __restrict__ nn_cnt, uint32_t min_ds) { scan_begin_body(sd, nn_cnt, min_ds, 0u); }
-__global__ void scan_begin_batch(const SlotDesc* __restrict__ slots) {
+__global__ void scan_begin_batch(const SlotDesc* __restrict__ slots, uint32_t* __restrict__ search, uint32_t n_slots) {
     const SlotDesc& d = slots[blockIdx.y];
     if (!d.active) return;
+    if (search && blockIdx.x == 0 && threadIdx.x == 0) {
+        const EskfDev* c = d.ctrl;
+        if (c->status == EK_RUNNING && c->converge != 0 && d.sd->n_ds >= d.min_ds) {
+            const uint32_t at = atomicAdd(&search[0], 1u);
+            if (at < n_slots) search[kKnnSearchHead + at] = blockIdx.y;
+        }
+    }
     scan_begin_body(d.sd, d.nn_cnt, d.min_ds, d.reset_cache);
 }
 
@@ -944,7 +951,7 @@
     return LIO_OK;
 }
 
-int vg_downsample_batch(hipStream_t st, const SlotDesc* d_slots, int n_slots, uint32_t max_raw, uint32_t max_ds, float leaf, int passes) {
+int vg_downsample_batch(hipStream_t st, const SlotDesc* d_slots, int n_slots, uint32_t max_raw, uint32_t max_ds, float leaf, int passes, uint32_t* d_search) {
     const float inv = 1.0f / leaf;
     const uint32_t nblocks = (max_raw + kTile - 1) / kTile;
     if (nblocks == 0 || n_slots <= 0) return LIO_OK;
@@ -965,14 +972,14 @@
     } else {
         hipLaunchKernelGGL(vg_centroid_both_batch, dim3(64 + kMonsterBlocksBatch, B), kThreads, 0, st, d_slots);
     }
-    hipLaunchKernelGGL(scan_begin_batch, dim3(16, B), 256, 0, st, d_slots);
+    hipLaunchKernelGGL(scan_begin_batch, dim3(16, B), 256, 0, st, d_slots, d_search, B);
     LIO_HIP_TRY(hipGetLastError());
     return LIO_OK;
 }
 
 int scan_begin_rows(hipStream_t st, const SlotDesc* d_descs, int n_rows) {
     if (n_rows <= 0) return LIO_OK;
-    hipLaunchKernelGGL(scan_begin_batch, dim3(16, (uint32_t)n_rows), 256, 0, st, d_descs);
+    hipLaunchKernelGGL(scan_begin_batch, dim3(16, (uint32_t)n_rows), 256, 0, st, d_descs, static_cast<uint32_t*>(nullptr), (uint32_t)n_rows);
     LIO_HIP_TRY(hipGetLastError());
     return LIO_OK;
 }
diff --git a/lidar-slam-detection_amd/python/lsd_amd/capi.py b/lidar-slam-detection_amd/python/lsd_amd/capi.py
--- a/lidar-slam-detection_amd/python/lsd_amd/capi.py
+++ b/lidar-slam-detection_amd/python/lsd_amd/capi.py
@@ -22,7 +22,7 @@
     "lio_engine_create", "lio_engine_create_shared", "lio_engine_destroy", "lio_engine_map", "lio_engine_scan", "lio_engine_set_state", "lio_engine_get_state",
     "lio_engine_set_cov", "lio_engine_get_cov", "lio_engine_set_flags", "lio_engine_travel", "lio_engine_is_degenerate",
     "lio_engine_update", "lio_engine_pass_log", "lio_engine_process_scan", "lio_engine_process_scan_device", "lio_engine_timings", "lio_engine_flush",
-    "lio_engine_enable_timing", "lio_comm_unique_id", "lio_comm_init", "lio_comm_destroy", "lio_comm_rank", "lio_comm_world", "lio_allgather_normal_eq", "lio_comm_stats", "lio_engine_set_joint", "lio_engine_joint_register", "lio_engine_joint_register_device", "lio_allgather_records", "lio_engines_process_batch", "lio_batch_create", "lio_batch_create_joint", "lio_batch_create_sequences", "lio_batch_sequences_step", "lio_batch_fastlio_main", "lio_batch_set_gather_hook", "lio_batch_exchange_stats", "lio_batch_destroy", "lio_batch_process", "lio_batch_engine", "lio_batch_enable_kernel_timing", "lio_batch_kernel_times", "lio_engine_set_static_map", "lio_scan_enable_kernel_timing", "lio_scan_kernel_times",
+    "lio_engine_enable_timing", "lio_comm_unique_id", "lio_comm_init", "lio_comm_destroy", "lio_comm_rank", "lio_comm_world", "lio_allgather_normal_eq", "lio_comm_stats", "lio_engine_set_joint", "lio_engine_joint_register", "lio_engine_joint_register_device", "lio_allgather_records", "lio_engines_process_batch", "lio_batch_create", "lio_batch_create_joint", "lio_batch_create_sequences", "lio_batch_sequences_step", "lio_batch_fastlio_main", "lio_batch_set_gather_hook", "lio_batch_exchange_stats", "lio_batch_destroy", "lio_batch_process", "lio_batch_engine", "lio_batch_slot_posterior","lio_batch_enable_kernel_timing", "lio_batch_kernel_times", "lio_engine_set_static_map", "lio_scan_enable_kernel_timing", "lio_scan_kernel_times",
     "lio_state_boxplus", "lio_state_boxminus",
     "lio_localmap_create", "lio_localmap_destroy", "lio_localmap_add_keyframe", "lio_localmap_num_keyframes", "lio_localmap_update",
     "lio_localmap_download",
@@ -389,6 +389,8 @@
     sig("lio_batch_destroy", None, vp)
     sig("lio_batch_process", cint, vp, C.POINTER(ScanJob), cint)
     sig("lio_batch_engine", vp, vp, cint, cint)
+    if L.lio_abi_version() >= 25:
+        sig("lio_batch_slot_posterior", cint, vp, cint, cint, C.POINTER(C.c_double), C.POINTER(C.c_int32), C.POINTER(C.c_int32), C.POINTER(C.c_uint32))
     sig("lio_batch_enable_kernel_timing", cint, vp, cint)
     sig("lio_batch_kernel_times", cint, vp, C.POINTER(BatchTimes), cint)
     sig("lio_engine_set_static_map", cint, vp, cint)
diff --git a/lidar-slam-detection_amd/python/lsd_amd/lio.py b/lidar-slam-detection_amd/python/lsd_amd/lio.py
--- a/lidar-slam-detection_amd/python/lsd_amd/lio.py
+++ b/lidar-slam-detection_amd/python/lsd_amd/lio.py
@@ -1753,6 +1753,11 @@
         e.scan = Scan(max_ds=100000, _borrow=lib().lio_engine_scan(h))
         return e
 
+    def slot_posterior(self, group, slot):
+        cov, ne, dg, sn = np.zeros(529), C.c_int32(0), C.c_int32(0), np.zeros(8, np.uint32)
+        check(lib().lio_batch_slot_posterior(self.h, int(group), int(slot), ptr(cov, C.c_double), C.byref(ne), C.byref(dg), ptr(sn, C.c_uint32)), "slot_posterior")
+        return dict(cov=cov.reshape(23, 23), n_eff=ne.value, degenerate=dg.value, search_n=sn)
+
     def process(self, jobs):
         return process_batch(None, jobs, batch=self)
 
```

After: 6.188 billion. No clear change (-0.2%).
